# fransiskusbudi/multimodal_segmentation_project

Measured on AMD Instinct MI355X. Metric: 3D volumes/sec (96^3, 4-class) fwd+bwd per node, higher is better.
Workload: dtype bf16; 1 GPU; UNet3D(1->4, features 16/32/64/128) 96^3 patch, per-GPU batch 2, fwd + Dice/CE loss + bwd + AdamW + metrics, dropout 0.0; global_batch=2, parallelism=dp1, hipgraph=False

## Files before the change

include/mi3d.h:

```cpp
#ifndef MI3D_H
#define MI3D_H
#include <stddef.h>
#include <stdint.h>

#ifdef __cplusplus
extern "C" {
#endif

#define MI3D_DTYPE_F32 0
#define MI3D_DTYPE_BF16 1
#define MI3D_MAX_LEVELS 6

const char* mi3d_last_error(void);
int mi3d_abi_version(void);

typedef struct mi3d_unet_desc {
    int32_t in_channels, out_channels;
    int32_t n_levels;
    int32_t features[MI3D_MAX_LEVELS];
    int32_t N, D, H, W;
    int32_t dtype;
    float bn_momentum, bn_eps;
} mi3d_unet_desc;

int mi3d_unet_num_params(const mi3d_unet_desc* d);
int mi3d_unet_num_buffers(const mi3d_unet_desc* d);
size_t mi3d_unet_workspace_bytes(const mi3d_unet_desc* d);
int64_t mi3d_unet_dropout_count(const mi3d_unet_desc* d);

int mi3d_unet_forward(const mi3d_unet_desc* d, const float* x, const void* const* params, void* const* buffers,
                      const float* drop_scales, int training, float* logits, float* gap_out, void* workspace,
                      size_t workspace_bytes, void* stream);

int mi3d_unet_bn_apply_deferred(const mi3d_unet_desc* d, void* const* buffers, const void* const* side, void* stream);

int mi3d_unet_infer(const mi3d_unet_desc* d, const float* x, const void* const* params, void* const* buffers, float* logits,
                    float* gap_out, void* workspace, size_t workspace_bytes, void* stream);

int mi3d_unet_num_segments(const mi3d_unet_desc* d);
int mi3d_unet_backward(const mi3d_unet_desc* d, const float* x, const void* const* params, void* const* grads,
                       const float* drop_scales, const float* dlogits, const float* dgap, float gap_scale,
                       int accumulate, int seg_begin, int seg_end, void* workspace, size_t workspace_bytes,
                       void* stream, void* aux_stream, void* const* events, int aux_join);
int mi3d_unet_backward_marks(const int* segs, void* const* events, int n);
int mi3d_stream_wait_event(void* stream, void* event);
int mi3d_event_create(void** event_out);
int mi3d_event_destroy(void* event);
int mi3d_stream_create(int priority_class, void** stream_out);
int mi3d_stream_destroy(void* stream);
int mi3d_debug_set_route(const char* name, int value);
int mi3d_debug_get_route(const char* name, int* value_out);
int mi3d_debug_route_count(void);
const char* mi3d_debug_route_name(int index);
int mi3d_debug_occupy_cus(int workgroups, int microseconds, float* buf, int64_t n, void* stream);
int mi3d_timing_event_create(void** event_out);
int mi3d_time_next_conv3_kernel(void* start_event, void* stop_event, int kind, int Cin, int Cout);
int mi3d_time_hook_fired(void);
int mi3d_event_elapsed_ms(void* start_event, void* stop_event, float* ms_out);
int mi3d_unet_segment_params(const mi3d_unet_desc* d, int seg, int* ranges);

typedef struct mi3d_loss_cfg {
    float w_ce;
    int32_t region_kind;
    float w_reg, alpha, beta, eps;
    float w_kd, temperature;
} mi3d_loss_cfg;
#define MI3D_LOSS_COEF_FLOATS 20
size_t mi3d_seg_loss_workspace_bytes(int C);
int mi3d_seg_loss_forward(const float* logits, const int64_t* labels, const float* teacher, int N, int C, int64_t V,
                          const mi3d_loss_cfg* cfg, float* loss_out, float* coef, void* workspace, void* stream);
int mi3d_seg_loss_backward(const float* logits, const int64_t* labels, const float* teacher, int N, int C, int64_t V,
                           const mi3d_loss_cfg* cfg, const float* coef, const float* grad_out, float* dlogits,
                           void* stream);
int mi3d_seg_loss_metrics_forward(const float* logits, const int64_t* labels, const float* teacher, int N, int C, int D,
                                  int64_t V, const mi3d_loss_cfg* cfg, float* loss_out, float* coef, float* metrics_out,
                                  void* loss_workspace, void* metrics_workspace, void* stream);
int mi3d_unet_head_loss_supported(const mi3d_unet_desc* d, const mi3d_loss_cfg* cfg);
int mi3d_head_loss_supported(int dtype, int Cin, int C, const mi3d_loss_cfg* cfg);
int mi3d_head_loss_forward(const void* z, int zcs, int Cin, const float* w, const float* bias, const int64_t* labels,
                           const float* teacher, int N, int C, int D, int64_t V, const mi3d_loss_cfg* cfg, float* loss_out, float* coef,
                           float* metrics_out, void* loss_workspace, void* metrics_workspace, float* logits_opt, void* stream);
int mi3d_head_loss_backward(const void* z, int zcs, int Cin, const float* w, const float* bias, const int64_t* labels,
                            const float* teacher, int N, int C, int64_t V, const mi3d_loss_cfg* cfg, const float* coef,
                            const float* grad_scale, void* dz, int dzcs, float* dW, float* db, int accumulate, void* workspace,
                            size_t workspace_bytes, void* stream);
int mi3d_unet_forward_loss(const mi3d_unet_desc* d, const float* x, const void* const* params, void* const* buffers,
                           const float* drop_scales, int training, const int64_t* labels, const float* teacher_logits,
                           const mi3d_loss_cfg* cfg, float* loss_out, float* coef, float* metrics_out, void* loss_workspace,
                           void* metrics_workspace, float* logits_opt, float* gap_out, void* workspace, size_t workspace_bytes,
                           void* stream);
int mi3d_unet_head_loss_forward(const mi3d_unet_desc* d, const void* const* params, const int64_t* labels, const float* teacher_logits,
                                const mi3d_loss_cfg* cfg, float* loss_out, float* coef, float* metrics_out, void* loss_workspace,
                                void* metrics_workspace, float* logits_opt, void* workspace, size_t workspace_bytes, void* stream);
int mi3d_unet_backward_loss(const mi3d_unet_desc* d, const float* x, const void* const* params, void* const* grads,
                            const float* drop_scales, const int64_t* labels, const float* teacher_logits, const mi3d_loss_cfg* cfg,
                            const float* coef, const float* grad_scale, const float* dgap, float gap_scale, int accumulate, int seg_begin,
                            int seg_end, void* workspace, size_t workspace_bytes, void* stream, void* aux_stream, void* const* events,
                            int aux_join);
size_t mi3d_seg_metrics_workspace_bytes(int C);
int mi3d_seg_metrics(const float* logits, const int64_t* labels, int N, int C, int D, int64_t V, float* out,
                     void* workspace, void* stream);
int mi3d_seg_class_counts(const float* logits, const int64_t* labels, int N, int C, int64_t V, int64_t* counts,
                          void* workspace, void* stream);
size_t mi3d_head_labels_workspace_bytes(int N, int Cout);
int mi3d_head_labels(int dtype, const void* z, int zcs, int Cin, const float* w, const float* bias, int Cout, int N, int64_t V,
                     uint8_t* labels_out, const int64_t* target, int64_t* counts, void* workspace, void* stream);
int mi3d_unet_head_labels(const mi3d_unet_desc* d, const void* const* params, const int64_t* target, uint8_t* labels_out,
                          int64_t* counts, void* head_workspace, void* workspace, size_t workspace_bytes, void* stream);

int mi3d_linear_forward(const float* x, const float* w, const float* b, float* y, int M, int K, int Nout, int relu,
                        const float* drop, void* stream);
int mi3d_linear_backward(const float* x, const float* w, const float* y, const float* gy, int M, int K, int Nout,
                         int relu, const float* drop, float* gx, float* gw, float* gb, int accumulate,
                         float gx_scale, float* workspace, void* stream);
int mi3d_scale(const float* x, float* y, int64_t n, float alpha, const float* alpha_dev, void* stream);
int mi3d_softmax_ce_rows(const float* logits, const int64_t* labels, int M, int C, float* loss, float* dlogits,
                         float scale, void* stream);

int mi3d_adamw_step(float* p, const float* g, float* m, float* v, int64_t n, float lr, float beta1, float beta2,
                    float eps, float weight_decay, float grad_scale, int64_t* step_dev, void* stream);
int mi3d_adamw_apply(float* p, const float* g, float* m, float* v, int64_t n, float lr, float beta1, float beta2,
                     float eps, float weight_decay, float grad_scale, int64_t* step_dev, int increment, void* stream);
int mi3d_dropout_scales(float* out, int64_t n, float p, uint64_t* state_dev, void* stream);

int mi3d_preprocess_ct(const float* in, float* out, int64_t n, float window_min, float window_max, void* stream);
size_t mi3d_preprocess_mri_workspace_bytes(void);
int mi3d_preprocess_mri(const float* in, float* out, int64_t n, float p_low, float p_high, void* workspace, void* stream);
int mi3d_remap_labels(const int64_t* in, int64_t* out, int64_t n, int kind, void* stream);

size_t mi3d_zoom3_workspace_bytes(int D, int H, int W);
int mi3d_zoom3_cubic(const float* in, float* out, int D, int H, int W, int Do, int Ho, int Wo, const void* table_d, int rows_d,
                     const void* table_h, int rows_h, const void* table_w, int rows_w, int ct_window, float window_min,
                     float window_max, void* stream);
int mi3d_zoom3_nearest_i64(const int64_t* in, int64_t* out, int D, int H, int W, int Do, int Ho, int Wo, const int32_t* index_d,
                           int rows_d, const int32_t* index_h, int rows_h, const int32_t* index_w, int rows_w, void* stream);

enum { MI3D_SRC_U8 = 0, MI3D_SRC_I16 = 1, MI3D_SRC_F32 = 2, MI3D_SRC_I64 = 3 };
int mi3d_reorient3(const void* in, int src_dtype, void* out, int out_i64, int D, int H, int W, int64_t stride_d, int64_t stride_h,
                   int64_t stride_w, int flip_mask, void* stream);
int mi3d_zoom3_cubic_src(const void* in, int src_dtype, int64_t stride_d, int64_t stride_h, int64_t stride_w, float* out, int D,
                         int H, int W, int Do, int Ho, int Wo, const void* table_d, int rows_d, const void* table_h, int rows_h,
                         const void* table_w, int rows_w, int ct_window, float window_min, float window_max, void* stream);
int mi3d_zoom3_nearest_src(const void* in, int src_dtype, int64_t stride_d, int64_t stride_h, int64_t stride_w, int64_t* out, int D,
                           int H, int W, int Do, int Ho, int Wo, const int32_t* index_d, int rows_d, const int32_t* index_h,
                           int rows_h, const int32_t* index_w, int rows_w, void* stream);
#define MI3D_MAX_MASKS 8
typedef struct {
    const void* mask[MI3D_MAX_MASKS];
    int64_t value[MI3D_MAX_MASKS];
    int32_t n;
} mi3d_mask_list;
int mi3d_merge_masks3(const mi3d_mask_list* masks, int src_dtype, int64_t stride_d, int64_t stride_h, int64_t stride_w, int64_t* out,
                      int D, int H, int W, int Do, int Ho, int Wo, const int32_t* index_d, int rows_d, const int32_t* index_h,
                      int rows_h, const int32_t* index_w, int rows_w, void* stream);
int mi3d_restore_labels3(const uint8_t* grid, int Dg, int Hg, int Wg, uint8_t* out, int D, int H, int W, int64_t stride_d,
                         int64_t stride_h, int64_t stride_w, const int32_t* index_d, const int32_t* index_h, const int32_t* index_w,
                         void* stream);

size_t mi3d_preview_workspace_bytes(int D, int H, int W);
int mi3d_foreground_profiles(const void* label, int label_dtype, int D, int H, int W, int64_t stride_d, int64_t stride_h,
                             int64_t stride_w, int64_t* counts, void* stream);
int mi3d_best_slices(const int64_t* counts, int D, int H, int W, int32_t* best, void* stream);
enum { MI3D_PREVIEW_STACK = 0, MI3D_PREVIEW_ONE = 1, MI3D_PREVIEW_THREE = 2 };
int mi3d_slice_minmax(const void* image, int image_dtype, int D, int H, int W, int64_t stride_d, int64_t stride_h, int64_t stride_w,
                      int axis, int mode, const int32_t* index, int k, uint32_t* keys, void* stream);
enum { MI3D_OVERLAY_F64 = 0, MI3D_OVERLAY_F32 = 1, MI3D_OVERLAY_U8 = 2 };
int mi3d_overlay_render(const void* image, int image_dtype, const int64_t* image_strides, const void* label, int label_dtype,
                        const int64_t* label_strides, const void* pred, int pred_dtype, const int64_t* pred_strides, int D, int H, int W,
                        int axis, int mode, const int32_t* index, int k, int rot90, const uint32_t* keys, int out_dtype,
                        void* const* outs, void* stream);

int mi3d_plane_affine(const float* img_in, float* img_out, const int64_t* lab_in, int64_t* lab_out, int C, int D, int H, int W,
                      int ax0, int ax1, const double* matrix, const double* offset, int flip_mask, void* stream);

#define MI3D_AUG_MAX_COEFF 20
#define MI3D_AUG_MAX_CP 16
#define MI3D_AUG_MAX_HOLES 8
typedef struct mi3d_aug_params {
    int32_t do_bias, bias_degree;
    double bias_coeff[MI3D_AUG_MAX_COEFF];
    int32_t do_noise;
    float noise_mean, noise_std;
    uint64_t noise_seed;
    int32_t do_contrast;
    float gamma;
    int32_t do_hist, n_cp;
    float ref_cp[MI3D_AUG_MAX_CP], flt_cp[MI3D_AUG_MAX_CP];
    int32_t n_holes;
    int32_t hole_size[3];
    int32_t hole_lo[MI3D_AUG_MAX_HOLES][3];
    float fill_value;
} mi3d_aug_params;
size_t mi3d_augment_workspace_bytes(void);
int mi3d_augment(const float* in, float* out, const float* noise, int C, int D, int H, int W, const mi3d_aug_params* params,
                 void* workspace, size_t workspace_bytes, void* stream);
int mi3d_fill_boxes_i64(int64_t* label, int C, int D, int H, int W, int n_holes, const int32_t* hole_lo,
                        const int32_t* hole_size, int64_t fill, void* stream);

size_t mi3d_conv3_workspace_bytes(int Cin, int Cout, int N, int D, int H, int W);
int mi3d_conv3_forward(int in_dtype, int out_dtype, const void* x, int xcs, int Cin, const float* w, const float* bias,
                       void* y, int ycs, int Cout, int N, int D, int H, int W, void* workspace, size_t workspace_bytes,
                       void* stream);
int mi3d_conv3_backward(int x_dtype, int dy_dtype, const void* x, int xcs, int Cin, const float* w, const void* dy,
                        int dycs, int Cout, void* dx, int dxcs, float* dW, float* db, int accumulate, int N, int D,
                        int H, int W, void* workspace, size_t workspace_bytes, void* stream);
typedef struct mi3d_conv3_bn_route { int32_t conv, ksplit, ticket, stats, rows, rows_offset; } mi3d_conv3_bn_route;
enum { MI3D_CONV3_BN_KEEP_TICKETS = 1 };
size_t mi3d_conv3_bn_workspace_bytes(int in_dtype, int dtype, int Cin, int Cout, int N, int D, int H, int W);
int mi3d_conv3_bn_forward(int in_dtype, int dtype, const void* x, int xcs, int Cin, const float* w, const float* bias,
                          const float* gamma, const float* beta, float* running_mean, float* running_var,
                          int64_t* num_batches_tracked, float momentum, float eps, const float* drop, void* y, void* z, int zcs,
                          void* pooled, int pcs, float* stat, int flags, mi3d_conv3_bn_route* route_out, int Cout, int N, int D,
                          int H, int W, void* workspace, size_t workspace_bytes, void* stream);
typedef struct mi3d_pending_sum { int64_t opaque[9]; } mi3d_pending_sum;
typedef struct mi3d_conv3_bn_bwd_route {
    int32_t bn, riders, dz_ks, conv, dgrad_ks, dx_ks, dx_offset, slabs, slab_layout, slab_ew, pending;
} mi3d_conv3_bn_bwd_route;
enum { MI3D_CONV3_BN_BWD_ALLOW_PARTIALS = 1, MI3D_CONV3_BN_BWD_DEFER = 2, MI3D_CONV3_BN_BWD_LEAVE_PENDING = 4 };
size_t mi3d_conv3_bn_bwd_workspace_bytes(int in_dtype, int dtype, int Cin, int Cout, int N, int D, int H, int W);
int mi3d_conv3_bn_backward(int in_dtype, int dtype, const void* x, int xcs, int x_split, int64_t x_delta, int Cin, const float* w,
                           const void* y, const float* stat, const float* drop, void* dz, int dzcs, const float* dz_partials,
                           int dz_ks, void* dy, void* dx, int dxcs, int dx_split, int64_t dx_delta, float* dW, float* db,
                           float* dgamma, float* dbeta, int accumulate, const mi3d_pending_sum* riders, mi3d_pending_sum* pending_out,
                           int flags, mi3d_conv3_bn_bwd_route* route_out, int Cout, int N, int D, int H, int W, void* workspace,
                           size_t workspace_bytes, void* stream);
int mi3d_pending_sum_launch(const mi3d_pending_sum* job, void* stream);
size_t mi3d_bn_workspace_bytes(int C);
int mi3d_bn_relu_drop_forward(int dtype, const void* y, int ycs, int C, int64_t M, int64_t V, const float* gamma,
                              const float* beta, float* running_mean, float* running_var, int64_t* num_batches_tracked,
                              float momentum, float eps, int training, const float* drop, void* z, int zcs, float* stat,
                              void* workspace, void* stream);
int mi3d_bn_relu_drop_backward(int dtype, const void* dz, int dzcs, const void* y, int ycs, int C, int64_t M, int64_t V,
                               const float* stat, const float* drop, void* dy, int dycs, float* dgamma, float* dbeta,
                               int accumulate, void* workspace, void* stream);
int mi3d_bn_relu_drop_pool_forward(int dtype, const void* y, int ycs, int C, int N, int D, int H, int W, const float* gamma,
                                   const float* beta, float* running_mean, float* running_var, int64_t* num_batches_tracked,
                                   float momentum, float eps, const float* drop, void* z, int zcs, void* pooled, int pcs,
                                   float* stat, void* workspace, void* stream);
int mi3d_maxpool2_forward(int dtype, const void* z, int zcs, int C, int N, int D, int H, int W, void* p, int pcs,
                          void* stream);
int mi3d_maxpool2_backward(int dtype, const void* dp, int dpcs, const void* z, int zcs, const void* dskip, int dskipcs,
                           void* dz, int dzcs, int C, int N, int D, int H, int W, void* stream);
int mi3d_maxpool2_backward_partials(int dtype, const float* dp_partials, int ks, const void* z, int zcs, const void* dskip,
                                    int dskipcs, void* dz, int dzcs, int C, int N, int D, int H, int W, void* stream);
size_t mi3d_upconv2_workspace_bytes(int Cin, int Cout, int N, int D, int H, int W);
int mi3d_upconv2_forward(int dtype, const void* x, int xcs, int Cin, const float* w, const float* bias, void* y, int ycs,
                         int Cout, int N, int D, int H, int W, void* workspace, size_t workspace_bytes, void* stream);
int mi3d_upconv2_backward(int dtype, const void* x, int xcs, int Cin, const float* w, const void* gy, int gycs, int Cout,
                          void* dx, int dxcs, float* dW, float* db, int accumulate, int N, int D, int H, int W,
                          void* workspace, size_t workspace_bytes, void* stream);
typedef struct mi3d_up_route {
    int32_t kind, gy, tap_split, wide, strided, resized, ksplit, persistent, slabs, slab_ew, wgrad_blocks, dgrad_blocks, pending;
} mi3d_up_route;
enum { MI3D_UP_BWD_LEAVE_PENDING = 1, MI3D_UP_BWD_SECOND_WORKSPACE = 2 };
size_t mi3d_up_workspace_bytes(int dtype, int Cin, int Cout, int N, int D, int H, int W);
size_t mi3d_up_workspace_region(int dtype, int Cin, int Cout, int N, int D, int H, int W, int which, size_t* bytes_out);
int mi3d_up_forward(int dtype, const void* x, int xcs, int Cin, const float* w, const float* bias, void* up, int ucs, int Cout,
                    int N, int D, int H, int W, int Do, int Ho, int Wo, mi3d_up_route* route_out, void* workspace,
                    size_t workspace_bytes, void* stream);
int mi3d_up_backward(int dtype, const void* x, int xcs, int Cin, const float* w, const void* gup, int gucs, int Cout, void* dx,
                     int dxcs, float* dW, float* db, int accumulate, int N, int D, int H, int W, int Do, int Ho, int Wo, int flags,
                     mi3d_pending_sum* pending_out, mi3d_up_route* route_out, void* workspace, size_t workspace_bytes, void* stream);
int mi3d_nearest_resize_forward(int dtype, const void* x, int xcs, int C, int N, int Di, int Hi, int Wi, void* y, int ycs, int Do,
                                int Ho, int Wo, void* stream);
int mi3d_nearest_resize_backward(int dtype, const void* gy, int gycs, int C, int N, int Do, int Ho, int Wo, void* gx, int gxcs,
                                 int Di, int Hi, int Wi, void* stream);
size_t mi3d_conv1_workspace_bytes(int Cin, int Cout);
int mi3d_conv1_forward(int dtype, const void* z, int zcs, int Cin, const float* w, const float* bias, float* logits, int Cout,
                       int N, int64_t V, void* stream);
int mi3d_conv1_backward(int dtype, const void* z, int zcs, int Cin, const float* w, const float* dlogits, int Cout, void* dz,
                        int dzcs, float* dW, float* db, int accumulate, int N, int64_t V, void* workspace,
                        size_t workspace_bytes, void* stream);
int mi3d_ncdhw_to_ndhwc(int dtype, const float* src, void* dst, int dcs, int C, int N, int64_t V, void* stream);
int mi3d_ndhwc_to_ncdhw(int dtype, const void* src, int scs, float* dst, int C, int N, int64_t V, void* stream);

int mi3d_graph_begin(void* stream);
int mi3d_graph_end(void* stream, void** graph_exec_out);
int mi3d_graph_launch(void* graph_exec, void* stream);
int mi3d_graph_destroy(void* graph_exec);
// ... 6 lines not shown
```

multimodal_segmentation_project_amd/_lib.py:

```python
import contextlib
import ctypes as C
import os

import torch

_HERE = os.path.dirname(os.path.abspath(__file__))
LIB_PATH = os.environ.get("MI3D_LIB_PATH") or os.path.join(_HERE, "libmi3d.so")
MAX_LEVELS = 6
LOSS_COEF_FLOATS = 20
DTYPE_F32, DTYPE_BF16 = 0, 1

vp, i32, i64, f32, sz = C.c_void_p, C.c_int, C.c_int64, C.c_float, C.c_size_t


class UNetDesc(C.Structure):
    _fields_ = [("in_channels", C.c_int32), ("out_channels", C.c_int32), ("n_levels", C.c_int32),
                ("features", C.c_int32 * MAX_LEVELS), ("N", C.c_int32), ("D", C.c_int32), ("H", C.c_int32),
                ("W", C.c_int32), ("dtype", C.c_int32), ("bn_momentum", C.c_float), ("bn_eps", C.c_float)]


class LossCfg(C.Structure):
    _fields_ = [("w_ce", C.c_float), ("region_kind", C.c_int32), ("w_reg", C.c_float), ("alpha", C.c_float),
                ("beta", C.c_float), ("eps", C.c_float), ("w_kd", C.c_float), ("temperature", C.c_float)]


AUG_MAX_COEFF, AUG_MAX_CP, AUG_MAX_HOLES = 20, 16, 8


class AugParams(C.Structure):
    _fields_ = [("do_bias", C.c_int32), ("bias_degree", C.c_int32), ("bias_coeff", C.c_double * AUG_MAX_COEFF),
                ("do_noise", C.c_int32), ("noise_mean", C.c_float), ("noise_std", C.c_float), ("noise_seed", C.c_uint64),
                ("do_contrast", C.c_int32), ("gamma", C.c_float), ("do_hist", C.c_int32), ("n_cp", C.c_int32),
                ("ref_cp", C.c_float * AUG_MAX_CP), ("flt_cp", C.c_float * AUG_MAX_CP), ("n_holes", C.c_int32),
                ("hole_size", C.c_int32 * 3), ("hole_lo", (C.c_int32 * 3) * AUG_MAX_HOLES), ("fill_value", C.c_float)]


MAX_MASKS = 8
SRC_U8, SRC_I16, SRC_F32, SRC_I64 = 0, 1, 2, 3
PREVIEW_STACK, PREVIEW_ONE, PREVIEW_THREE = 0, 1, 2
OVERLAY_F64, OVERLAY_F32, OVERLAY_U8 = 0, 1, 2


class MaskList(C.Structure):
    _fields_ = [("mask", C.c_void_p * MAX_MASKS), ("value", C.c_int64 * MAX_MASKS), ("n", C.c_int32)]


class Conv3BnRoute(C.Structure):
    _fields_ = [(k, C.c_int32) for k in ("conv", "ksplit", "ticket", "stats", "rows", "rows_offset")]


CONV3_BN_KEEP_TICKETS = 1


class Conv3BnBwdRoute(C.Structure):
    _fields_ = [(k, C.c_int32) for k in ("bn", "riders", "dz_ks", "conv", "dgrad_ks", "dx_ks", "dx_offset", "slabs", "slab_layout",
                                         "slab_ew", "pending")]


class PendingSum(C.Structure):
    _fields_ = [("opaque", C.c_int64 * 9)]


CONV3_BN_BWD_ALLOW_PARTIALS, CONV3_BN_BWD_DEFER, CONV3_BN_BWD_LEAVE_PENDING = 1, 2, 4


class UpRoute(C.Structure):
    _fields_ = [(k, C.c_int32) for k in ("kind", "gy", "tap_split", "wide", "strided", "resized", "ksplit", "persistent", "slabs",
                                         "slab_ew", "wgrad_blocks", "dgrad_blocks", "pending")]


UP_BWD_LEAVE_PENDING, UP_BWD_SECOND_WORKSPACE = 1, 2

_DP, _LP, _AP, _MP = C.POINTER(UNetDesc), C.POINTER(LossCfg), C.POINTER(AugParams), C.POINTER(MaskList)

_SIGS = {
    "mi3d_last_error": (C.c_char_p, []),
    "mi3d_abi_version": (i32, []),
    "mi3d_unet_num_params": (i32, [_DP]),
    "mi3d_unet_num_buffers": (i32, [_DP]),
    "mi3d_unet_num_segments": (i32, [_DP]),
    "mi3d_unet_workspace_bytes": (sz, [_DP]),
    "mi3d_unet_dropout_count": (i64, [_DP]),
    "mi3d_unet_segment_params": (i32, [_DP, i32, C.POINTER(C.c_int)]),
    "mi3d_unet_forward": (i32, [_DP, vp, vp, vp, vp, i32, vp, vp, vp, sz, vp]),
    "mi3d_unet_infer": (i32, [_DP, vp, vp, vp, vp, vp, vp, sz, vp]),
    "mi3d_unet_bn_apply_deferred": (i32, [_DP, vp, vp, vp]),
    "mi3d_unet_backward": (i32, [_DP, vp, vp, vp, vp, vp, vp, f32, i32, i32, i32, vp, sz, vp, vp, vp, i32]),
    "mi3d_unet_backward_marks": (i32, [C.POINTER(C.c_int), C.POINTER(vp), i32]),
    "mi3d_stream_wait_event": (i32, [vp, vp]),
    "mi3d_event_create": (i32, [C.POINTER(vp)]),
    "mi3d_event_destroy": (i32, [vp]),
    "mi3d_stream_create": (i32, [i32, C.POINTER(vp)]),
    "mi3d_stream_destroy": (i32, [vp]),
    "mi3d_debug_set_route": (i32, [C.c_char_p, i32]),
    "mi3d_debug_get_route": (i32, [C.c_char_p, C.POINTER(C.c_int)]),
    "mi3d_debug_route_count": (i32, []),
    "mi3d_debug_route_name": (C.c_char_p, [i32]),
    "mi3d_debug_occupy_cus": (i32, [i32, i32, vp, i64, vp]),
    "mi3d_timing_event_create": (i32, [C.POINTER(vp)]),
    "mi3d_time_next_conv3_kernel": (i32, [vp, vp, i32, i32, i32]),
    "mi3d_time_hook_fired": (i32, []),
    "mi3d_event_elapsed_ms": (i32, [vp, vp, C.POINTER(C.c_float)]),
    "mi3d_seg_loss_workspace_bytes": (sz, [i32]),
    "mi3d_seg_loss_forward": (i32, [vp, vp, vp, i32, i32, i64, _LP, vp, vp, vp, vp]),
    "mi3d_seg_loss_backward": (i32, [vp, vp, vp, i32, i32, i64, _LP, vp, vp, vp, vp]),
    "mi3d_seg_loss_metrics_forward": (i32, [vp, vp, vp, i32, i32, i32, i64, _LP, vp, vp, vp, vp, vp, vp]),
    "mi3d_unet_head_loss_supported": (i32, [_DP, _LP]),
    "mi3d_head_loss_supported": (i32, [i32, i32, i32, _LP]),
    "mi3d_head_loss_forward": (i32, [vp, i32, i32, vp, vp, vp, vp, i32, i32, i32, i64, _LP, vp, vp, vp, vp, vp, vp, vp]),
    "mi3d_head_loss_backward": (i32, [vp, i32, i32, vp, vp, vp, vp, i32, i32, i64, _LP, vp, vp, vp, i32, vp, vp, i32, vp, sz, vp]),
    "mi3d_unet_forward_loss": (i32, [_DP, vp, vp, vp, vp, i32, vp, vp, _LP, vp, vp, vp, vp, vp, vp, vp, vp, sz, vp]),
    "mi3d_unet_head_loss_forward": (i32, [_DP, vp, vp, vp, _LP, vp, vp, vp, vp, vp, vp, vp, sz, vp]),
    "mi3d_unet_backward_loss": (i32, [_DP, vp, vp, vp, vp, vp, vp, _LP, vp, vp, vp, f32, i32, i32, i32, vp, sz, vp, vp, vp, i32]),
    "mi3d_seg_metrics_workspace_bytes": (sz, [i32]),
    "mi3d_seg_metrics": (i32, [vp, vp, i32, i32, i32, i64, vp, vp, vp]),
    "mi3d_seg_class_counts": (i32, [vp, vp, i32, i32, i64, vp, vp, vp]),
    "mi3d_head_labels_workspace_bytes": (sz, [i32, i32]),
    "mi3d_head_labels": (i32, [i32, vp, i32, i32, vp, vp, i32, i32, i64, vp, vp, vp, vp, vp]),
    "mi3d_unet_head_labels": (i32, [_DP, vp, vp, vp, vp, vp, vp, sz, vp]),
    "mi3d_linear_forward": (i32, [vp, vp, vp, vp, i32, i32, i32, i32, vp, vp]),
    "mi3d_linear_backward": (i32, [vp, vp, vp, vp, i32, i32, i32, i32, vp, vp, vp, vp, i32, f32, vp, vp]),
    "mi3d_scale": (i32, [vp, vp, i64, f32, vp, vp]),
    "mi3d_softmax_ce_rows": (i32, [vp, vp, i32, i32, vp, vp, f32, vp]),
    "mi3d_adamw_step": (i32, [vp, vp, vp, vp, i64, f32, f32, f32, f32, f32, f32, vp, vp]),
    "mi3d_adamw_apply": (i32, [vp, vp, vp, vp, i64, f32, f32, f32, f32, f32, f32, vp, i32, vp]),
    "mi3d_dropout_scales": (i32, [vp, i64, f32, vp, vp]),
    "mi3d_preprocess_ct": (i32, [vp, vp, i64, f32, f32, vp]),
    "mi3d_preprocess_mri_workspace_bytes": (sz, []),
    "mi3d_preprocess_mri": (i32, [vp, vp, i64, f32, f32, vp, vp]),
    "mi3d_remap_labels": (i32, [vp, vp, i64, i32, vp]),
    "mi3d_zoom3_workspace_bytes": (sz, [i32, i32, i32]),
    "mi3d_zoom3_cubic": (i32, [vp, vp, i32, i32, i32, i32, i32, i32, vp, i32, vp, i32, vp, i32, i32, f32, f32, vp]),
    "mi3d_zoom3_nearest_i64": (i32, [vp, vp, i32, i32, i32, i32, i32, i32, vp, i32, vp, i32, vp, i32, vp]),
    "mi3d_reorient3": (i32, [vp, i32, vp, i32, i32, i32, i32, i64, i64, i64, i32, vp]),
    "mi3d_zoom3_cubic_src": (i32, [vp, i32, i64, i64, i64, vp, i32, i32, i32, i32, i32, i32, vp, i32, vp, i32, vp, i32, i32, f32, f32, vp]),
    "mi3d_zoom3_nearest_src": (i32, [vp, i32, i64, i64, i64, vp, i32, i32, i32, i32, i32, i32, vp, i32, vp, i32, vp, i32, vp]),
    "mi3d_merge_masks3": (i32, [_MP, i32, i64, i64, i64, vp, i32, i32, i32, i32, i32, i32, vp, i32, vp, i32, vp, i32, vp]),
    "mi3d_restore_labels3": (i32, [vp, i32, i32, i32, vp, i32, i32, i32, i64, i64, i64, vp, vp, vp, vp]),
    "mi3d_preview_workspace_bytes": (sz, [i32, i32, i32]),
    "mi3d_foreground_profiles": (i32, [vp, i32, i32, i32, i32, i64, i64, i64, vp, vp]),
    "mi3d_best_slices": (i32, [vp, i32, i32, i32, vp, vp]),
    "mi3d_slice_minmax": (i32, [vp, i32, i32, i32, i32, i64, i64, i64, i32, i32, vp, i32, vp, vp]),
    "mi3d_overlay_render": (i32, [vp, i32, C.POINTER(i64), vp, i32, C.POINTER(i64), vp, i32, C.POINTER(i64), i32, i32, i32, i32, i32, vp,
                                  i32, i32, vp, i32, C.POINTER(vp), vp]),
    "mi3d_plane_affine": (i32, [vp, vp, vp, vp, i32, i32, i32, i32, i32, i32, C.POINTER(C.c_double), C.POINTER(C.c_double), i32, vp]),
    "mi3d_augment_workspace_bytes": (sz, []),
    "mi3d_augment": (i32, [vp, vp, vp, i32, i32, i32, i32, _AP, vp, sz, vp]),
    "mi3d_fill_boxes_i64": (i32, [vp, i32, i32, i32, i32, i32, C.POINTER(C.c_int32), C.POINTER(C.c_int32), i64, vp]),
    "mi3d_conv3_workspace_bytes": (sz, [i32, i32, i32, i32, i32, i32]),
    "mi3d_conv3_forward": (i32, [i32, i32, vp, i32, i32, vp, vp, vp, i32, i32, i32, i32, i32, i32, vp, sz, vp]),
    "mi3d_conv3_backward": (i32, [i32, i32, vp, i32, i32, vp, vp, i32, i32, vp, i32, vp, vp, i32, i32, i32, i32, i32,
                                  vp, sz, vp]),
    "mi3d_conv3_bn_workspace_bytes": (sz, [i32, i32, i32, i32, i32, i32, i32, i32]),
    "mi3d_conv3_bn_forward": (i32, [i32, i32, vp, i32, i32, vp, vp, vp, vp, vp, vp, vp, f32, f32, vp, vp, vp, i32, vp, i32, vp, i32,
                                    C.POINTER(Conv3BnRoute), i32, i32, i32, i32, i32, vp, sz, vp]),
    "mi3d_conv3_bn_bwd_workspace_bytes": (sz, [i32, i32, i32, i32, i32, i32, i32, i32]),
    "mi3d_conv3_bn_backward": (i32, [i32, i32, vp, i32, i32, i64, i32, vp, vp, vp, vp, vp, i32, vp, i32, vp, vp, i32, i32, i64, vp, vp,
                                     vp, vp, i32, C.POINTER(PendingSum), C.POINTER(PendingSum), i32, C.POINTER(Conv3BnBwdRoute),
                                     i32, i32, i32, i32, i32, vp, sz, vp]),
    "mi3d_pending_sum_launch": (i32, [C.POINTER(PendingSum), vp]),
    "mi3d_bn_workspace_bytes": (sz, [i32]),
    "mi3d_bn_relu_drop_forward": (i32, [i32, vp, i32, i32, i64, i64, vp, vp, vp, vp, vp, f32, f32, i32, vp, vp, i32,
                                        vp, vp, vp]),
    "mi3d_bn_relu_drop_backward": (i32, [i32, vp, i32, vp, i32, i32, i64, i64, vp, vp, vp, i32, vp, vp, i32, vp, vp]),
    "mi3d_bn_relu_drop_pool_forward": (i32, [i32, vp, i32, i32, i32, i32, i32, i32, vp, vp, vp, vp, vp, f32, f32, vp, vp, i32,
                                             vp, i32, vp, vp, vp]),
    "mi3d_conv1_workspace_bytes": (sz, [i32, i32]),
    "mi3d_conv1_forward": (i32, [i32, vp, i32, i32, vp, vp, vp, i32, i32, i64, vp]),
    "mi3d_conv1_backward": (i32, [i32, vp, i32, i32, vp, vp, i32, vp, i32, vp, vp, i32, i32, i64, vp, sz, vp]),
    "mi3d_maxpool2_forward": (i32, [i32, vp, i32, i32, i32, i32, i32, i32, vp, i32, vp]),
    "mi3d_maxpool2_backward": (i32, [i32, vp, i32, vp, i32, vp, i32, vp, i32, i32, i32, i32, i32, i32, vp]),
    "mi3d_maxpool2_backward_partials": (i32, [i32, vp, i32, vp, i32, vp, i32, vp, i32, i32, i32, i32, i32, i32, vp]),
    "mi3d_upconv2_workspace_bytes": (sz, [i32, i32, i32, i32, i32, i32]),
    "mi3d_upconv2_forward": (i32, [i32, vp, i32, i32, vp, vp, vp, i32, i32, i32, i32, i32, i32, vp, sz, vp]),
    "mi3d_upconv2_backward": (i32, [i32, vp, i32, i32, vp, vp, i32, i32, vp, i32, vp, vp, i32, i32, i32, i32, i32, vp,
                                    sz, vp]),
    "mi3d_up_workspace_bytes": (sz, [i32, i32, i32, i32, i32, i32, i32]),
    "mi3d_up_workspace_region": (sz, [i32, i32, i32, i32, i32, i32, i32, i32, C.POINTER(sz)]),
# ... 107 lines not shown
```

multimodal_segmentation_project_amd/csrc/api.hip:

```cpp
#include "../../include/mi3d.h"
#include <stdlib.h>
#include <string.h>

#include "ops.h"

static_assert(MI3D_LOSS_COEF_FLOATS >= 2 * MI3D_MAX_CLASSES + 4, "coef buffer too small");

namespace {
struct RouteEntry { const char* name; int Mi3dRoutes::*field; };
const RouteEntry ROUTE_TABLE[] = {
#define MI3D_ROUTE_ENTRY(name, dflt) {#name, &Mi3dRoutes::name},
    MI3D_ROUTE_LIST(MI3D_ROUTE_ENTRY)
#undef MI3D_ROUTE_ENTRY
};
constexpr int N_ROUTES = sizeof(ROUTE_TABLE) / sizeof(ROUTE_TABLE[0]);
Mi3dRoutes load_routes() {
    Mi3dRoutes r;
    for (int i = 0; i < N_ROUTES; i++) {
        char env[64] = "MI3D_";
        size_t n = 5;
        for (const char* c = ROUTE_TABLE[i].name; *c && n + 1 < sizeof(env); c++) env[n++] = (*c >= 'a' && *c <= 'z') ? *c - 32 : *c;
        env[n] = 0;
        const char* v = getenv(env);
        if (!v) continue;
// ... 215 lines not shown
    ConvBwdCall k{x_dtype, dy_dtype, x, xcs, Halves(), Cin, w, nullptr, nullptr, nullptr, const_cast<void*>(dy), dycs, nullptr, 0, nullptr,
                  dx, dxcs, Halves(), dW, db, nullptr, nullptr, accumulate, nullptr, nullptr, 0, nullptr, Cout, g, mfma, c1, ws};
    return conv_bn_bwd_run(k, L, (hipStream_t)stream);
}

size_t mi3d_conv3_bn_bwd_workspace_bytes(int in_dtype, int dtype, int Cin, int Cout, int N, int D, int H, int W) {
    if (Cin < 1 || Cout < 1 || N < 1 || D < 1 || H < 1 || W < 1) return 0;
    bool mfma, c1;
    conv3_layer_class(dtype, Cin, Cout, mfma, c1);
    return conv_bn_bwd_ws(mfma, Cin, Cout, Geo{N, D, H, W}).total;
}
int mi3d_conv3_bn_backward(int in_dtype, int dtype, const void* x, int xcs, int x_split, int64_t x_delta, int Cin, const float* w,
                           const void* y, const float* stat, const float* drop, void* dz, int dzcs, const float* dz_partials,
                           int dz_ks, void* dy, void* dx, int dxcs, int dx_split, int64_t dx_delta, float* dW, float* db,
                           float* dgamma, float* dbeta, int accumulate, const mi3d_pending_sum* riders, mi3d_pending_sum* pending_out,
                           int flags, mi3d_conv3_bn_bwd_route* route_out, int Cout, int N, int D, int H, int W, void* workspace,
                           size_t workspace_bytes, void* stream) {
    const char* fn = "mi3d_conv3_bn_backward";
    MI3D_CHECK_ARG(x && w && dz && workspace, "%s: null pointer", fn);
    MI3D_CHECK_ARG(!stat || (y && dy), "%s: the BatchNorm backward needs y and dy", fn);
    MI3D_CHECK_ARG(stat || (!dz_partials && !riders), "%s: dz partials and riders need the BatchNorm backward", fn);
    MI3D_CHECK_ARG((dtype == MI3D_F32 || dtype == MI3D_BF16) && (in_dtype == dtype || (in_dtype == MI3D_F32 && Cin == 1 && xcs == 1)),
                   "%s: bad dtypes %d -> %d", fn, in_dtype, dtype);
    MI3D_CHECK_ARG(Cin >= 1 && Cout >= 1 && Cout <= 256 && xcs >= (x_delta ? 16 : Cin) && dzcs >= Cout && N >= 1 && D >= 1 && H >= 1 && W >= 1,
                   "%s: bad shape", fn);
    MI3D_CHECK_ARG(!dz_partials || dz_ks >= 1, "%s: dz_ks=%d", fn, dz_ks);
    MI3D_CHECK_ARG(!(flags & MI3D_CONV3_BN_BWD_LEAVE_PENDING) || pending_out, "%s: LEAVE_PENDING needs pending_out", fn);
    MI3D_CHECK_ARG(!(flags & MI3D_CONV3_BN_BWD_DEFER) || !(flags & MI3D_CONV3_BN_BWD_LEAVE_PENDING), "%s: DEFER launches its own sum", fn);
    const Geo g{N, D, H, W};
    bool mfma, c1;
    conv3_layer_class(dtype, Cin, Cout, mfma, c1);
    MI3D_CHECK_ARG(!mfma || (xcs % 8 == 0 && dzcs % 8 == 0 && (!dx || dxcs % 4 == 0)), "%s: channel strides %d / %d / %d", fn, xcs, dzcs, dxcs);
    MI3D_CHECK_ARG(!c1 || (in_dtype == MI3D_F32 && !dx), "%s: the first-layer kernel reads an fp32 image and has no input gradient", fn);
    MI3D_CHECK_ARG(!dx || dxcs >= (dx_delta ? 16 : Cin), "%s: dx stride %d", fn, dxcs);
    MI3D_CHECK_ARG(!(flags & MI3D_CONV3_BN_BWD_DEFER) || (mfma && (dW || db)), "%s: only MFMA layers with a weight gradient defer it", fn);
    MI3D_CHECK_ARG((!x_delta && !dx_delta) || (mfma && conv3_mfma_halves_ok(Cout, Cin, g)),
                   "%s: planar halves need the full-resolution kernels", fn);
    const ConvBnBwdWs L = conv_bn_bwd_ws(mfma, Cin, Cout, g);
    MI3D_CHECK_ARG(workspace_bytes >= L.total, "%s: workspace too small: %zu < %zu", fn, workspace_bytes, L.total);
    MI3D_CHECK_ARG(((uintptr_t)workspace & 255) == 0, "%s: workspace must be 256-byte aligned", fn);
    Halves xh, dxh;
    if (x_delta) { xh.split = x_split; xh.delta = x_delta; }
    if (dx_delta) { dxh.split = dx_split; dxh.delta = dx_delta; }
    ConvBwdCall k{in_dtype, dtype, x, xcs, xh, Cin, w, y, stat, drop, dz, dzcs, dz_partials, dz_ks, dy, dx, dxcs, dxh, dW, db, dgamma, dbeta,
                  accumulate, riders, pending_out, flags, route_out, Cout, g, mfma, c1, (char*)workspace};
    return conv_bn_bwd_run(k, L, (hipStream_t)stream);
}
int mi3d_pending_sum_launch(const mi3d_pending_sum* job, void* stream) {
    MI3D_CHECK_ARG(job, "mi3d_pending_sum_launch: null job");
    SlabJob q;
    memcpy(&q, job, sizeof(q));
    return slab_job_launch(q, (hipStream_t)stream);
}

}

namespace {
struct ConvBnWs {
    bool mfma, c1;
    size_t statpart, tkcount, bnws, wpf, wpd, skws, total;
};
ConvBnWs conv_bn_ws(int dtype, int Cin, int Cout, Geo g) {
    ConvBnWs L;
    conv3_layer_class(dtype, Cin, Cout, L.mfma, L.c1);
    size_t off = 0;
    auto take = [&](size_t bytes) { size_t o = off; off = (off + bytes + 255) & ~(size_t)255; return o; };
    int rows = L.mfma ? conv3_mfma_stat_blocks(Cin, Cout, g) : L.c1 ? conv3_c1_fwd_stat_blocks(g) : 1;
    L.statpart = take((size_t)rows * 2 * Cout * sizeof(float));
    L.tkcount = take((size_t)CONV3_TK_COUNTERS * sizeof(int));
    L.bnws = take(bn_ws_floats(Cout) * sizeof(float));
    L.wpf = take(L.mfma ? conv3_mfma_pack_elems(Cin, Cout) * 2 : conv3_direct_pack_floats(Cin, Cout) * sizeof(float));
    L.wpd = take(L.mfma ? conv3_mfma_pack_elems(Cin, Cout) * 2 : conv3_direct_pack_floats(Cout, Cin) * sizeof(float));
    L.skws = take((L.mfma ? conv3_mfma_splitk_floats(Cin, Cout, g) : 0) * sizeof(float) + 16);
    L.total = off;
    return L;
}
}

extern "C" {

size_t mi3d_conv3_bn_workspace_bytes(int in_dtype, int dtype, int Cin, int Cout, int N, int D, int H, int W) {
    if (Cin < 1 || Cout < 1 || N < 1 || D < 1 || H < 1 || W < 1) return 0;
    return conv_bn_ws(dtype, Cin, Cout, Geo{N, D, H, W}).total;
}
int mi3d_conv3_bn_forward(int in_dtype, int dtype, const void* x, int xcs, int Cin, const float* w, const float* bias,
                          const float* gamma, const float* beta, float* running_mean, float* running_var,
                          int64_t* num_batches_tracked, float momentum, float eps, const float* drop, void* y, void* z, int zcs,
                          void* pooled, int pcs, float* stat, int flags, mi3d_conv3_bn_route* route_out, int Cout, int N, int D,
                          int H, int W, void* workspace, size_t workspace_bytes, void* stream) {
    MI3D_CHECK_ARG(x && w && bias && gamma && beta && y && z && stat && workspace, "mi3d_conv3_bn_forward: null pointer");
    MI3D_CHECK_ARG((dtype == MI3D_F32 || dtype == MI3D_BF16) && (in_dtype == dtype || (in_dtype == MI3D_F32 && Cin == 1 && xcs == 1)),
                   "mi3d_conv3_bn_forward: bad dtypes %d -> %d", in_dtype, dtype);
    MI3D_CHECK_ARG(Cin >= 1 && Cout >= 1 && Cout <= 256 && xcs >= Cin && zcs >= Cout && N >= 1 && D >= 1 && H >= 1 && W >= 1,
                   "mi3d_conv3_bn_forward: bad shape");
    MI3D_CHECK_ARG(!pooled || (D % 2 == 0 && H % 2 == 0 && W % 2 == 0 && pcs >= Cout && (int64_t)N * D * H * W * Cout < (1ll << 31)),
                   "mi3d_conv3_bn_forward: pooled needs even sides and fewer than 2^31 elements");
    const Geo g{N, D, H, W};
    const ConvBnWs L = conv_bn_ws(dtype, Cin, Cout, g);
    MI3D_CHECK_ARG(!L.mfma || xcs % 8 == 0, "mi3d_conv3_bn_forward: input channel stride %d", xcs);
    MI3D_CHECK_ARG(!L.c1 || in_dtype == MI3D_F32, "mi3d_conv3_bn_forward: the first-layer kernel reads an fp32 image");
    MI3D_CHECK_ARG(workspace_bytes >= L.total, "mi3d_conv3_bn_forward: workspace too small: %zu < %zu", workspace_bytes, L.total);
    MI3D_CHECK_ARG(((uintptr_t)workspace & 255) == 0, "mi3d_conv3_bn_forward: workspace must be 256-byte aligned");
    char* ws = (char*)workspace;
    hipStream_t s = (hipStream_t)stream;
    bool tk_zeroed = false;
    if (L.mfma) {
// ... 330 lines not shown
```

multimodal_segmentation_project_amd/csrc/conv3_mfma.hip:

```cpp
#include <stdlib.h>

#include <type_traits>

#include <hip/hip_ext.h>

#include "mfma_tile.h"
#include "ops.h"
#include "slab_sum.h"

namespace {

constexpr int BLK = 256;

MI3D_HD constexpr int ktap(int mode, int s, int h) {
    if (mode == 0) return 2 * s + h;
    if (s < 12) {
        int dz = s / 4, k = s % 4;
        return k < 3 ? dz * 9 + k * 3 + h : dz * 9 + h * 3 + 2;
    }
    if (s == 12) return h * 9 + 8;
    return h == 0 ? 26 : 27;
}

__global__ void pack_mfma_kernel(const float* __restrict__ w, int Cin, int Cout, bf16* __restrict__ wf, bf16* __restrict__ wd,
                                 int mode_f, int mode_d) {
    int64_t n = (int64_t)Cin * Cout * 28;
    for (int64_t i = (int64_t)blockIdx.x * blockDim.x + threadIdx.x; i < 2 * n; i += (int64_t)gridDim.x * blockDim.x) {
        bool dg = i >= n;
        int64_t k = dg ? i - n : i;
        int j = k & 7; int lane = (k >> 3) & 63; int64_t r = k >> 9;
        int nob = (dg ? Cin : Cout) / 16;
        int ob = r % nob; r /= nob; int s = r % 14; int chunk = r / 14;
        int g = lane >> 4, tap = ktap(dg ? mode_d : mode_f, s, g >> 1);
        int o = ob * 16 + (lane & 15), ic = chunk * 16 + 8 * (g & 1) + j;
        float v = 0.f;
        if (tap < 27) v = dg ? w[((int64_t)ic * Cin + o) * 27 + (26 - tap)] : w[((int64_t)o * Cin + ic) * 27 + tap];
        (dg ? wd : wf)[k] = (bf16)v;
    }
}

constexpr int PK_LD = 16 * 27 + 1;
__global__ __launch_bounds__(BLK) void pack_all_kernel(PackJobs J) {
    __shared__ float wl[16 * PK_LD];
    if (blockIdx.x == 0 && J.zero)
        for (int i = threadIdx.x; i < J.nzero; i += BLK) J.zero[i] = 0;
    int b = blockIdx.x, ji = 0;
    while (ji + 1 < J.n && b >= J.j[ji + 1].blk0) ji++;
    const float* __restrict__ w = J.j[ji].w;
    int Cin = J.j[ji].Cin, Cout = J.j[ji].Cout, lb = b - J.j[ji].blk0;
    if (J.j[ji].kind == 0) {
        bf16* wf = (bf16*)J.j[ji].a; bf16* wd = (bf16*)J.j[ji].b;
        int mode_f = J.j[ji].mode_f, mode_d = J.j[ji].mode_d;
        int CIBN = Cin / 16, COBN = Cout / 16;
        int cib = lb % CIBN, cob = lb / CIBN;
        const float* __restrict__ sc = J.j[ji].scale;
        for (int idx = threadIdx.x; idx < 16 * 108; idx += BLK) {
            int row = idx / 108, k = (idx - row * 108) * 4;
            f32x4 v = *reinterpret_cast<const f32x4*>(w + ((int64_t)(cob * 16 + row) * Cin + cib * 16) * 27 + k);
            float f = sc ? sc[cob * 16 + row] : 1.f;
#pragma unroll
            for (int j = 0; j < 4; j++) wl[row * PK_LD + k + j] = v[j] * f;
        }
        __syncthreads();
        for (int q = threadIdx.x; q < 2 * 14 * 64; q += BLK) {
            int img = q / (14 * 64), r = q - img * (14 * 64);
            int s = r >> 6, lane = r & 63, g = lane >> 4, o = lane & 15;
            int tap = ktap(img ? mode_d : mode_f, s, g >> 1);
            bf16x8 v;
#pragma unroll
            for (int j = 0; j < 8; j++) {
                int ic = 8 * (g & 1) + j;
                float f = 0.f;
                if (tap < 27) f = img ? wl[ic * PK_LD + o * 27 + (26 - tap)] : wl[o * PK_LD + ic * 27 + tap];
                v[j] = (bf16)f;
            }
            bf16* dst = img ? wd + ((((int64_t)cob * 14 + s) * CIBN + cib) * 64 + lane) * 8
                            : wf + ((((int64_t)cib * 14 + s) * COBN + cob) * 64 + lane) * 8;
            *reinterpret_cast<bf16x8*>(dst) = v;
        }
    } else {
        bf16* wf = (bf16*)J.j[ji].a; bf16* wb = (bf16*)J.j[ji].b;
        int64_t n = (int64_t)Cin * Cout * 8;
        int KS = Cin / 32, COBN = Cout / 16, S = Cout / 4;
        int64_t k0 = ((int64_t)lb * BLK + threadIdx.x) * 8;
        if (k0 >= 2 * n) return;
        bool bw = k0 >= n;
        int64_t k = bw ? k0 - n : k0;
        int lane = (k >> 3) & 63, G = lane >> 4;
        int64_t r = k >> 9;
        bf16x8 v;
        if (!bw) {
            int ks = r % KS; r /= KS; int cb = r % COBN; int tap = r / COBN;
            int co = cb * 16 + (lane & 15);
#pragma unroll
            for (int j = 0; j < 8; j++) v[j] = (bf16)w[((int64_t)(32 * ks + 8 * G + j) * Cout + co) * 8 + tap];
        } else {
            int s = r % S; int cib = r / S;
            int kk0 = 32 * s + 8 * G, tap = kk0 / Cout, co0 = kk0 % Cout, ci = cib * 16 + (lane & 15);
#pragma unroll
            for (int j = 0; j < 8; j++) v[j] = (bf16)w[((int64_t)ci * Cout + co0 + j) * 8 + tap];
        }
        *reinterpret_cast<bf16x8*>((bw ? wb : wf) + k) = v;
    }
}

struct Bid { int x, y, z, gx, gy, gz; bool placed = false; };
__device__ __forceinline__ Bid real_bid() {
    return Bid{(int)blockIdx.x, (int)blockIdx.y, (int)blockIdx.z, (int)gridDim.x, (int)gridDim.y, (int)gridDim.z};
}
__device__ __forceinline__ int xcd_contig(int b, int n) {
    int q8 = n / 8, r8 = n % 8, xcd = b % 8, idx = b / 8;
    return (xcd < r8 ? xcd * (q8 + 1) : r8 * (q8 + 1) + (xcd - r8) * q8) + idx;
}

template <int TZ_, int TYB_, int TXB_, int BX_>
struct ConvTile {
    static constexpr int TZ = TZ_, TYB = TYB_, TXB = TXB_, BX = BX_;
    static constexpr int BY = 16 / BX;
    static constexpr int TY = TYB * BY, TX = TXB * BX;
    static constexpr int IZ = TZ + 2, IY = TY + 2, IX = TX + 2;
    static constexpr int IXP = BX == 4 ? 12 : IX;
    static constexpr int MB = TYB * TXB;
    static constexpr int NVT = TZ * TY * TX;
    static constexpr int NVOX = IZ * IY * IX, NVOXP = IZ * IY * IXP;
    static constexpr int pieces(int nthr) { return (NVOX * 2 + nthr - 1) / nthr; }
};
using FullTile = ConvTile<4, 8, 1, 16>;

template <class T, int COB>
struct Lds4 {
    static constexpr int xs = 0, red = T::NVOXP * 32, bytes = red + 4 * COB * 16 * 2 * 4;
};
template <class T, int COB>
struct Lds8 {
    static constexpr int xs = 0, wl = T::NVOXP * 32, red = wl + 14 * COB * 1024, bytes = red + 8 * COB * 16 * 2 * 4;
};
template <int COB, int NCH>
struct LdsP {
    static constexpr int xs = 0, wl = FullTile::NVOX * 32, red = wl + NCH * 14 * COB * 1024, bytes = red + 4 * COB * 16 * 2 * 4;
};

template <class T, int NTHR, int NIT>
__device__ __forceinline__ void staging_map(int z0, int y0, int x0, int D, int H, int W, int xcs, int (&soff)[NIT], int (&sdst)[NIT]) {
#pragma unroll
    for (int it = 0; it < NIT; it++) {
        int idx = threadIdx.x + it * NTHR;
        int vox = idx >> 1, half = idx & 1;
        int ix = vox % T::IX, t = vox / T::IX, iy = t % T::IY, iz = t / T::IY;
        sdst[it] = T::IXP == T::IX ? 0 : (t * T::IXP + ix) * 16 + half * 8;
        int gz = z0 - 1 + iz, gy = y0 - 1 + iy, gx = x0 - 1 + ix;
        bool inb = idx < T::NVOX * 2 && gz >= 0 && gz < D && gy >= 0 && gy < H && gx >= 0 && gx < W;
        soff[it] = inb ? ((gz * H + gy) * W + gx) * xcs + half * 8 : -1;
    }
}
template <class T, int NTHR, int NIT>
// ... 780 lines not shown

inline bool big_geo(Geo g) { return g.W >= 32 && g.H >= 16; }

inline int pick_ksplit(int Cin, int Cout, Geo g, int target_override = 0) {
    if (big_geo(g)) return 1;
    int64_t wgs = (int64_t)g.N * cdiv(g.D, 4) * cdiv(g.H, 8) * cdiv(g.W, 8) * (Cout / (Cout % 32 == 0 ? 32 : 16));
    int nchunk = Cin / 16, k = 1;
    constexpr int SPLITK_TARGET = 128;
    const int tgt = target_override > 0 && target_override < SPLITK_TARGET ? target_override : SPLITK_TARGET;
    while (wgs * k < tgt && k * 2 <= nchunk && nchunk % (k * 2) == 0 && k < 16) k *= 2;
    return k;
}

}

bool conv3_mfma_supported(int Cin, int Cout, int xcs, int ycs) {
    return Cin % 16 == 0 && Cout % 16 == 0 && xcs % 8 == 0 && ycs % 4 == 0 && Cin >= 16 && Cout >= 16;
}

size_t conv3_mfma_pack_elems(int Cin, int Cout) { return (size_t)Cin * Cout * 28; }

int conv3_mfma_pack(const float* w, int Cin, int Cout, void* wp_fwd, void* wp_dgrad, Geo g, hipStream_t s) {
    int64_t n = 2 * (int64_t)conv3_mfma_pack_elems(Cin, Cout);
    int mode_f = persist_ok(Cin, Cout, g) ? 1 : 0, mode_d = persist_ok(Cout, Cin, g) ? 1 : 0;
    pack_mfma_kernel<<<cdiv(n, 256) > 2048 ? 2048 : cdiv(n, 256), 256, 0, s>>>(w, Cin, Cout, (bf16*)wp_fwd, (bf16*)wp_dgrad,
                                                                             mode_f, mode_d);
    MI3D_LAUNCH_CHECK();
    return 0;
}

int pack_all_add_conv3(PackJobs& J, const float* w, int Cin, int Cout, void* wp_fwd, void* wp_dgrad, Geo g, const float* scale) {
    MI3D_CHECK_ARG(J.n < MAX_PACK_JOBS && Cin % 16 == 0 && Cout % 16 == 0, "pack_all: too many jobs / bad channels");
    MI3D_CHECK_ARG(((uintptr_t)w % 16) == 0, "pack_all: conv weight tensor must be 16-byte aligned");
    PackJob& j = J.j[J.n++];
    j = PackJob{w, wp_fwd, wp_dgrad, Cin, Cout, 0, persist_ok(Cin, Cout, g) ? 1 : 0, persist_ok(Cout, Cin, g) ? 1 : 0, J.nblocks, scale};
    J.nblocks += (Cin / 16) * (Cout / 16);
    return 0;
}
int pack_all_add_upconv(PackJobs& J, const float* w, int Cin, int Cout, void* wp) {
    MI3D_CHECK_ARG(J.n < MAX_PACK_JOBS, "pack_all: too many jobs");
    int64_t n = (int64_t)Cin * Cout * 8;
    PackJob& j = J.j[J.n++];
    j = PackJob{w, wp, (bf16*)wp + n, Cin, Cout, 1, 0, 0, J.nblocks};
    J.nblocks += (int)cdiv(2 * n, (int64_t)BLK * 8);
    return 0;
}
int pack_all_launch(const PackJobs& J, hipStream_t s) {
    if (J.n == 0) return 0;
    pack_all_kernel<<<J.nblocks, BLK, 0, s>>>(J);
    MI3D_LAUNCH_CHECK();
    return 0;
}

int conv3_mfma_stat_blocks(int Cin, int Cout, Geo g) {
    if (persist_ok(Cin, Cout, g)) return persist_grid(Cin, Cout, g);
    if (big_geo(g)) return g.N * cdiv(g.D, 4) * cdiv(g.H, 8) * cdiv(g.W, 16);
    return g.N * cdiv(g.D, 4) * cdiv(g.H, 8) * cdiv(g.W, 8);
}

size_t conv3_mfma_splitk_floats(int Cin, int Cout, Geo g) {
    int k = pick_ksplit(Cin, Cout, g);
    return k > 1 ? (size_t)k * g.M() * Cout : 0;
}
bool conv3_mfma_fuses_stats(int Cin, int Cout, Geo g) { return pick_ksplit(Cin, Cout, g) == 1; }

bool conv3_mfma_halves_ok(int Cin, int Cout, Geo g) { return persist_ok(Cin, Cout, g); }

bool conv3_mfma_ticket_ok(int Cin, int Cout, Geo g) {
    if (!mi3d_routes().splitk_ticket || mi3d_routes().conv8 == 0 || big_geo(g) || persist_ok(Cin, Cout, g)) return false;
    if (pick_ksplit(Cin, Cout, g) <= 1) return false;
    const int64_t wgs = (int64_t)g.N * cdiv(g.D, 4) * cdiv(g.H, 8) * cdiv(g.W, 8) * (Cout / (Cout % 32 == 0 ? 32 : 16));
    return wgs <= CONV3_TK_COUNTERS;
}

int conv3_mfma_fwd(const void* x, int xcs, int Cin, const void* wp, const float* bias, void* y, int ycs, int Cout, Geo g,
                   float* part, float* skws, hipStream_t s, Halves xh, Halves yh, int* ks_deferred, int relu, int split_target,
                   float* tk_rows, int* tk_count, Conv3Launch* launched) {
    if (ks_deferred) *ks_deferred = 0;
    MI3D_CHECK_ARG(!tk_rows || (conv3_mfma_ticket_ok(Cin, Cout, g) && skws && split_target == 0), "conv3_mfma_fwd: no split-K ticket for %d->%d here", Cin, Cout);
    MI3D_CHECK_ARG((!xh.on() && !yh.on()) || persist_ok(Cin, Cout, g), "conv3_mfma_fwd: planar halves need the persistent kernel");
    MI3D_CHECK_ARG(conv3_mfma_supported(Cin, Cout, xcs, ycs), "conv3_mfma_fwd: unsupported channels %d->%d", Cin, Cout);
    MI3D_CHECK_ARG(((uintptr_t)x % 16) == 0 && ((uintptr_t)y % 8) == 0, "conv3_mfma_fwd: misaligned tensors");
    const bf16* xp = (const bf16*)x; const bf16* w = (const bf16*)wp; bf16* yp = (bf16*)y;
    bool two = Cout % 32 == 0;
    if (persist_ok(Cin, Cout, g)) {
        int tz = cdiv(g.D, 4), ty = cdiv(g.H, 8), tx = cdiv(g.W, 16), nt = g.N * tz * ty * tx, grid = persist_grid(Cin, Cout, g);
        if (launched) *launched = Conv3Launch{2, 1};
        if (ycs % 8 == 0 && ((uintptr_t)y % 16) == 0 && yh.delta % 8 == 0) relu |= 2;
        auto launch = [&](auto cob, auto nch) -> int {
            constexpr int COB = decltype(cob)::value, NCH = decltype(nch)::value;
            if (part)
                return launch_hooked<conv3_mfma_persist_kernel<COB, NCH, true>>(grid, BLK, 0, s, 2, Cin, Cout, xp, xcs, w, bias, yp, ycs, g.D, g.H, g.W,
                                                                                tz, ty, tx, nt, part, xh, yh, relu);
            return launch_hooked<conv3_mfma_persist_kernel<COB, NCH, false>>(grid, BLK, 0, s, 3, Cin, Cout, xp, xcs, w, bias, yp, ycs, g.D, g.H, g.W,
                                                                             tz, ty, tx, nt, (float*)nullptr, xh, yh, relu);
        };
        constexpr std::integral_constant<int, 1> one{};
        constexpr std::integral_constant<int, 2> two{};
        return Cin == 16 && Cout == 16 ? launch(one, one) : Cin == 32 ? launch(one, two) : launch(two, one);
    }
    int ks = skws ? pick_ksplit(Cin, Cout, g, split_target) : 1;
    if (ycs % 8 == 0 && ((uintptr_t)y % 16) == 0 && Cout % 32 == 0) relu |= 2;
    if (ks > 1) MI3D_CHECK_ARG(ycs % 8 == 0 && ((uintptr_t)y % 16) == 0, "conv3_mfma_fwd: split-K needs 16-B aligned output rows");
    if (launched) *launched = Conv3Launch{big_geo(g) ? 3 : 4, big_geo(g) ? 1 : ks};
    if (big_geo(g)) {
        if (two) return launch_cfg<4, 8, 1, 16, 2>(xp, xcs, Cin, w, bias, yp, ycs, Cout, g, part, 1, nullptr, s, false, relu);
// ... 518 lines not shown
    const float* part; int ks; int64_t M; int C; bf16* y; int ycs; int nfin;
    const float* slabs; int nslab; int64_t slab_sz, nW; float* dW; float* db; int accumulate, Cin, Cout, layout, ew;
};
__global__ __launch_bounds__(BLK) void bwd_tail_kernel(TailArgs a) {
    int b = blockIdx.x;
    if (b < a.nfin) { splitk_finish_body(b, a.nfin, a.part, a.ks, a.M, a.C, nullptr, a.y, a.ycs); return; }
    b -= a.nfin;
    if (a.layout == 2) slab_reduce_tile_body(b, a.slabs, a.nslab, a.slab_sz, a.nW, a.dW, a.db, a.accumulate, a.Cin, a.Cout);
    else if (a.ew == 8) slab_reduce2_body<true, 8>(b, a.slabs, a.nslab, a.slab_sz, a.nW, a.dW, a.db, a.accumulate, a.Cin, a.Cout);
    else slab_reduce2_body<true, 32>(b, a.slabs, a.nslab, a.slab_sz, a.nW, a.dW, a.db, a.accumulate, a.Cin, a.Cout);
}

struct WgCfg { int cob, cib, nt, tg, nsb; };

inline WgCfg wgrad_cfg(int Cin, int Cout, Geo g, int target = 0) {
    WgCfg c;
    c.cob = 1;
    c.cib = 1;
    int groups = (Cout / 16) * (Cin / 16);
    int64_t ntiles = (int64_t)g.N * cdiv(g.D, WTZ) * cdiv(g.H, WTY) * cdiv(g.W, WTX);
    c.nt = 27;
    c.tg = 1;
    int64_t want = (target > 0 ? target : 2 * device_cus()) / (int64_t)groups;
    if (want < 1) want = 1;
    int64_t rounds = cdiv(ntiles, want);
    c.nsb = (int)cdiv(ntiles, rounds);
    return c;
}

template <int CO_B, int CI_B, int NT>
int launch_wgrad(const bf16* x, int xcs, int Cin, const bf16* dy, int dycs, int Cout, Geo g, float* slabs, WgCfg c,
                 hipStream_t s, Halves xh) {
    constexpr size_t lds = LdsWg<CO_B, CI_B>::bytes;
    dim3 grid((unsigned)(c.nsb * c.tg), (unsigned)(Cout / (16 * CO_B)), (unsigned)(Cin / (16 * CI_B)));
    const bool full = persist_ok(Cout, Cin, g);
    const int xcd_tiles = full ? 1 : 0;
    int pgx = 0, pgy = 0, pgz = 0;
    if (!full && c.tg == 1) {
        pgx = (int)grid.x; pgy = (int)grid.y; pgz = (int)grid.z;
        grid = dim3((unsigned)(pgx * pgy * pgz));
    }
    return launch_hooked<conv3_wgrad_mfma_kernel<CO_B, CI_B, NT>>(grid, BLK, lds, s, 1, Cin, Cout, x, xcs, Cin, dy, dycs, Cout, g.N, g.D, g.H, g.W,
                                                                  cdiv(g.D, WTZ), cdiv(g.H, WTY), cdiv(g.W, WTX), c.tg, slabs, xh, xcd_tiles,
                                                                  pgx, pgy, pgz);
}

inline int c1_nsb(Geo g) {
    int64_t ntiles = (int64_t)g.N * cdiv(g.D, WTZ) * cdiv(g.H, WTY) * cdiv(g.W, WTX);
    return (int)(ntiles < 1024 ? ntiles : 1024);
}

}

__global__ __launch_bounds__(BLK) void slab_job_kernel(SlabJob q) { slab_job_run(q, (int)blockIdx.x); }
int slab_job_launch(const SlabJob& q, hipStream_t s) {
    if (q.nblocks <= 0) return 0;
    slab_job_kernel<<<q.nblocks, BLK, 0, s>>>(q);
    MI3D_LAUNCH_CHECK();
    return 0;
}

static int wgrad_slab_sum(float* ws, int nsb, int Cin, int Cout, float* dW, float* db, int accumulate, hipStream_t s,
                          SlabJob* pend = nullptr) {
    int64_t nW = (int64_t)Cout * Cin * 27, slab_sz = nW + Cout;
    if (pend) { *pend = slab_job_make((dW && slab_sz >= (800 << 10)) ? 2 : 1, ws, nsb, slab_sz, nW, dW, db, Cin, Cout, accumulate); return 0; }
    if (dW && slab_sz >= (800 << 10))
        slab_reduce_tile_kernel<<<(Cout / 16) * (Cin / 16) * 4, BLK, 0, s>>>(ws, nsb, slab_sz, nW, dW, db, accumulate, Cin, Cout);
    else if (slab_sz < (16 << 10))
        slab_reduce2_kernel<true, 8><<<cdiv(slab_sz, 8), BLK, 0, s>>>(ws, nsb, slab_sz, nW, dW, db, accumulate, Cin, Cout);
    else
        slab_reduce2_kernel<true, 32><<<cdiv(slab_sz, 32), BLK, 0, s>>>(ws, nsb, slab_sz, nW, dW, db, accumulate, Cin, Cout);
    MI3D_LAUNCH_CHECK();
    return 0;
}

size_t conv3_mfma_wgrad_ws_floats(int Cin, int Cout, Geo g) {
    if (Cin == 1) return (size_t)c1_nsb(g) * ((size_t)Cout * 27 + Cout);
    return (size_t)wgrad_cfg(Cin, Cout, g).nsb * ((size_t)Cout * Cin * 27 + Cout);
}

bool conv3_mfma_big_geo(Geo g) { return big_geo(g); }
int conv3_mfma_wgrad_slabs(int Cin, int Cout, Geo g, int wg_target) { return wgrad_cfg(Cin, Cout, g, wg_target).nsb; }
int conv3_mfma_bwd_ksplit(int Cin, int Cout, Geo g) { return pick_ksplit(Cout, Cin, g, CONV3_BWD_SPLITK_TARGET); }

int conv3_mfma_wgrad(const void* x, int xcs, int Cin, const void* dy, int dycs, int Cout, Geo g, float* dW, float* db,
                     int accumulate, float* ws, size_t ws_floats, hipStream_t s, Halves xh, SlabJob* pend, int wg_target) {
    MI3D_CHECK_ARG(conv3_mfma_supported(Cin, Cout, xcs, dycs) && dycs % 8 == 0, "conv3_mfma_wgrad: unsupported channels");
    WgCfg c = wgrad_cfg(Cin, Cout, g, wg_target);
    int64_t nW = (int64_t)Cout * Cin * 27, slab_sz = nW + Cout;
    MI3D_CHECK_ARG(ws_floats >= (size_t)c.nsb * slab_sz, "conv3_mfma_wgrad: workspace too small");
    const bf16* xp = (const bf16*)x; const bf16* dp = (const bf16*)dy;
    int rc;
    if (c.cob == 1 && c.cib == 1) rc = launch_wgrad<1, 1, 27>(xp, xcs, Cin, dp, dycs, Cout, g, ws, c, s, xh);
    else { MI3D_CHECK_ARG(false, "conv3_mfma_wgrad: no kernel for this block config"); return -1; }
    MI3D_TRY(rc);
    return wgrad_slab_sum(ws, c.nsb, Cin, Cout, dW, db, accumulate, s, pend);
}


extern "C" int mi3d_time_next_conv3_kernel(void* start_event, void* stop_event, int kind, int Cin, int Cout) {
    g_hook = TimeHook();
    if (!start_event || !stop_event) return 0;
    g_hook.e0 = (hipEvent_t)start_event; g_hook.e1 = (hipEvent_t)stop_event;
    g_hook.kind = kind; g_hook.cin = Cin; g_hook.cout = Cout; g_hook.armed = true;
    return 0;
}
extern "C" int mi3d_time_hook_fired(void) {
    const int f = g_hook.fired ? 1 : 0;
    g_hook = TimeHook();
    return f;
// ... 134 lines not shown
```

multimodal_segmentation_project_amd/csrc/misc.hip:

```cpp
#include <stdarg.h>
#include <stdio.h>

#include "ops.h"

static thread_local char g_err[512] = "";
void mi3d_set_error(const char* fmt, ...) {
    va_list ap;
    va_start(ap, fmt);
    vsnprintf(g_err, sizeof(g_err), fmt, ap);
    va_end(ap);
}
extern "C" const char* mi3d_last_error(void) { return g_err; }

namespace {
constexpr int BLK = 256;
inline int sgrid(int64_t total, int cap = 2048) {
    int64_t w = (total + BLK - 1) / BLK;
    return (int)(w < 1 ? 1 : (w > cap ? cap : w));
}

template <int EW>
__global__ __launch_bounds__(BLK) void slab_reduce_kernel(const float* __restrict__ slabs, int nslab, int64_t slab_sz, int64_t nW,
                                                          float* __restrict__ dW, float* __restrict__ db, int accumulate) {
    constexpr int SG = BLK / EW;
    __shared__ float red[SG][EW];
    int e = threadIdx.x % EW, sg = threadIdx.x / EW;
    int64_t i = (int64_t)blockIdx.x * EW + e;
    float s = 0.f;
    if (i < slab_sz)
        for (int b = sg; b < nslab; b += SG) s += slabs[(int64_t)b * slab_sz + i];
    red[sg][e] = s;
    __syncthreads();
    if (sg == 0 && i < slab_sz) {
        float t = 0.f;
#pragma unroll
        for (int k = 0; k < SG; k += 8)
            t += ((red[k][e] + red[k + 1][e]) + (red[k + 2][e] + red[k + 3][e])) +
                 ((red[k + 4][e] + red[k + 5][e]) + (red[k + 6][e] + red[k + 7][e]));
        if (i < nW) { if (dW) dW[i] = accumulate ? dW[i] + t : t; }
        else if (db) { db[i - nW] = accumulate ? db[i - nW] + t : t; }
    }
}

template <typename T>
__global__ void ncdhw_to_ndhwc_kernel(const float* __restrict__ src, T* __restrict__ dst, int dcs, int C, int N, int64_t V) {
    int64_t total = (int64_t)N * V * C;
    for (int64_t i = (int64_t)blockIdx.x * BLK + threadIdx.x; i < total; i += (int64_t)gridDim.x * BLK) {
        int c = (int)(i % C); int64_t m = i / C; int64_t n = m / V, v = m - n * V;
        dst[m * dcs + c] = from_f<T>(src[((int64_t)n * C + c) * V + v]);
    }
}
template <typename T>
__global__ void ndhwc_to_ncdhw_kernel(const T* __restrict__ src, int scs, float* __restrict__ dst, int C, int N, int64_t V) {
    int64_t total = (int64_t)N * V * C;
    for (int64_t i = (int64_t)blockIdx.x * BLK + threadIdx.x; i < total; i += (int64_t)gridDim.x * BLK) {
// ... 47 lines not shown
__global__ void linear_bwd_pre_kernel(const float* __restrict__ y, const float* __restrict__ gy, int n, int relu,
                                      const float* __restrict__ drop, float* __restrict__ gpre) {
    int i = blockIdx.x * BLK + threadIdx.x;
    if (i >= n) return;
    float g = gy[i];
    if (drop) g *= drop[i];
    if (relu && !(y[i] > 0.f)) g = 0.f;
    gpre[i] = g;
}
__global__ __launch_bounds__(BLK) void linear_bwd_x_kernel(const float* __restrict__ gpre, const float* __restrict__ w,
                                                           float* __restrict__ gx, int M, int K, int Nout, float scale) {
    int i = blockIdx.x * BLK + threadIdx.x;
    if (i >= M * K) return;
    int m = i / K, k = i - m * K;
    float s = 0.f;
    for (int o = 0; o < Nout; o++) s = fmaf(gpre[(int64_t)m * Nout + o], w[(int64_t)o * K + k], s);
    gx[i] = s * scale;
}
__global__ __launch_bounds__(BLK) void linear_bwd_w_kernel(const float* __restrict__ gpre, const float* __restrict__ x,
                                                           float* __restrict__ gw, float* __restrict__ gb, int M, int K,
                                                           int Nout, int accumulate) {
    int i = blockIdx.x * BLK + threadIdx.x;
    if (gw && i < Nout * K) {
        int o = i / K, k = i - o * K;
        float s = 0.f;
        for (int m = 0; m < M; m++) s = fmaf(gpre[(int64_t)m * Nout + o], x[(int64_t)m * K + k], s);
        gw[i] = accumulate ? gw[i] + s : s;
    }
    if (i < Nout && gb) {
        float s = 0.f;
        for (int m = 0; m < M; m++) s += gpre[(int64_t)m * Nout + i];
        gb[i] = accumulate ? gb[i] + s : s;
    }
}

__global__ void softmax_ce_rows_kernel(const float* __restrict__ logits, const int64_t* __restrict__ labels, int M, int C,
                                       float* loss, float* dlogits, float scale) {
    int lane = threadIdx.x;
    double tot = 0.0;
    for (int m = 0; m < M; m++) {
        float z = lane < C ? logits[(int64_t)m * C + lane] : -INFINITY;
        float mx = z;
        for (int o = 32; o > 0; o >>= 1) mx = fmaxf(mx, __shfl_xor(mx, o, 64));
        float e = lane < C ? expf(z - mx) : 0.f;
        float se = wave_sum(e);
        int t = (int)labels[m];
        float zt = __shfl(z, t, 64);
        tot += (double)(mx + logf(se) - zt);
        if (dlogits && lane < C) dlogits[(int64_t)m * C + lane] = scale * (e / se - (lane == t ? 1.f : 0.f)) / (float)M;
    }
    if (lane == 0 && loss) *loss = (float)(tot / (double)M);
}

__device__ __forceinline__ void adamw_one(float& pi, float gi, float& mi, float& vi, float decay, float b1, float b2, float eps,
                                          float grad_scale, float bc2s, float step_size) {
#pragma clang fp contract(off)
    gi = gi * grad_scale;
    mi = __builtin_fmaf(b1, mi, (1.f - b1) * gi);
    vi = __builtin_fmaf(b2, vi, ((1.f - b2) * gi) * gi);
    float denom = sqrtf(vi) / bc2s + eps;
    pi = __builtin_fmaf(decay, pi, -(step_size * (mi / denom)));
}
__global__ __launch_bounds__(BLK) void adamw_kernel(float* __restrict__ p, const float* __restrict__ g, float* __restrict__ m,
                                                    float* __restrict__ v, int64_t n, float lr, float b1, float b2, float eps, float wd,
                                                    float grad_scale, const int64_t* __restrict__ step_dev) {
    const bool vec = ((reinterpret_cast<uintptr_t>(p) | reinterpret_cast<uintptr_t>(g) | reinterpret_cast<uintptr_t>(m) |
                       reinterpret_cast<uintptr_t>(v)) & 15) == 0;
    const int64_t n4 = vec ? n >> 2 : 0, stride = (int64_t)gridDim.x * BLK;
    int64_t i = (int64_t)blockIdx.x * BLK + threadIdx.x;
    float4 g4, p4, m4, v4;
    bool have = i < n4;
    if (have) {
        g4 = reinterpret_cast<const float4*>(g)[i]; p4 = reinterpret_cast<const float4*>(p)[i];
        m4 = reinterpret_cast<const float4*>(m)[i]; v4 = reinterpret_cast<const float4*>(v)[i];
    }
    double step = (double)(*step_dev + 1);
    float bc1 = (float)(1.0 - pow((double)b1, step));
    float bc2s = (float)sqrt(1.0 - pow((double)b2, step));
    float step_size = lr / bc1;
    const float decay = __builtin_fmaf(-lr, wd, 1.f);
    while (have) {
        int64_t j = i + stride;
        bool have2 = j < n4;
        float4 g5, p5, m5, v5;
        if (have2) {
            g5 = reinterpret_cast<const float4*>(g)[j]; p5 = reinterpret_cast<const float4*>(p)[j];
            m5 = reinterpret_cast<const float4*>(m)[j]; v5 = reinterpret_cast<const float4*>(v)[j];
        }
        adamw_one(p4.x, g4.x, m4.x, v4.x, decay, b1, b2, eps, grad_scale, bc2s, step_size);
        adamw_one(p4.y, g4.y, m4.y, v4.y, decay, b1, b2, eps, grad_scale, bc2s, step_size);
        adamw_one(p4.z, g4.z, m4.z, v4.z, decay, b1, b2, eps, grad_scale, bc2s, step_size);
        adamw_one(p4.w, g4.w, m4.w, v4.w, decay, b1, b2, eps, grad_scale, bc2s, step_size);
        reinterpret_cast<float4*>(m)[i] = m4;
        reinterpret_cast<float4*>(v)[i] = v4;
        reinterpret_cast<float4*>(p)[i] = p4;
        i = j; have = have2; g4 = g5; p4 = p5; m4 = m5; v4 = v5;
    }
    for (int64_t k = n4 * 4 + (int64_t)blockIdx.x * BLK + threadIdx.x; k < n; k += stride) {
        float pi = p[k], mi = m[k], vi = v[k];
        adamw_one(pi, g[k], mi, vi, decay, b1, b2, eps, grad_scale, bc2s, step_size);
        m[k] = mi; v[k] = vi; p[k] = pi;
    }
}
__global__ void step_inc_kernel(int64_t* step_dev) { *step_dev += 1; }

__device__ __forceinline__ uint64_t mix64(uint64_t x) {
    x += 0x9E3779B97F4A7C15ull;
    x = (x ^ (x >> 30)) * 0xBF58476D1CE4E5B9ull;
    x = (x ^ (x >> 27)) * 0x94D049BB133111EBull;
    return x ^ (x >> 31);
}
__global__ void dropout_scales_kernel(float* __restrict__ out, int64_t n, float p, const uint64_t* __restrict__ state) {
    uint64_t seed = state[0], ctr = state[1];
    float keep_scale = p < 1.f ? 1.f / (1.f - p) : 0.f;
    for (int64_t i = (int64_t)blockIdx.x * BLK + threadIdx.x; i < n; i += (int64_t)gridDim.x * BLK) {
// ... 137 lines not shown
```

multimodal_segmentation_project_amd/csrc/ops.h:

```cpp
#pragma once
#include "common.h"
#include "slab_sum.h"

struct Geo {
    int N, D, H, W;
    int64_t V() const { return (int64_t)D * H * W; }
    int64_t M() const { return (int64_t)N * D * H * W; }
};

size_t conv3_direct_pack_floats(int Cin, int Cout);
int conv3_direct_pack(const float* w, int Cin, int Cout, float* wp_fwd, float* wp_dgrad, hipStream_t s,
                      const float* scale = nullptr);
int conv3_direct_fwd(int in_dtype, int out_dtype, const void* x, int xcs, int Cin, const float* wp,
                     const float* bias, void* y, int ycs, int Cout, Geo g, hipStream_t s, int relu = 0);
size_t conv3_direct_wgrad_ws_floats(int Cin, int Cout, Geo g);
int conv3_direct_wgrad(int x_dtype, int dy_dtype, const void* x, int xcs, int Cin, const void* dy, int dycs,
                       int Cout, Geo g, float* dW, float* db, int accumulate, float* ws, size_t ws_floats,
                       hipStream_t s);

bool conv3_mfma_supported(int Cin, int Cout, int xcs, int ycs);
size_t conv3_mfma_pack_elems(int Cin, int Cout);
int conv3_mfma_pack(const float* w, int Cin, int Cout, void* wp_fwd, void* wp_dgrad, Geo g, hipStream_t s);
struct PackJob { const float* w; void* a; void* b; int Cin, Cout, kind, mode_f, mode_d, blk0; const float* scale; };
constexpr int MAX_PACK_JOBS = 32;
struct PackJobs { int n, nblocks; PackJob j[MAX_PACK_JOBS]; int* zero = nullptr; int nzero = 0; };
int pack_all_add_conv3(PackJobs& J, const float* w, int Cin, int Cout, void* wp_fwd, void* wp_dgrad, Geo g,
                       const float* scale = nullptr);
int pack_all_add_upconv(PackJobs& J, const float* w, int Cin, int Cout, void* wp);
int pack_all_launch(const PackJobs& J, hipStream_t s);
int conv3_mfma_stat_blocks(int Cin, int Cout, Geo g);
size_t conv3_mfma_splitk_floats(int Cin, int Cout, Geo g);
bool conv3_mfma_fuses_stats(int Cin, int Cout, Geo g);
struct Halves { int split = 1 << 30; int64_t delta = 0; bool on() const { return delta != 0; } };
bool conv3_mfma_halves_ok(int Cin, int Cout, Geo g);
bool conv3_mfma_ticket_ok(int Cin, int Cout, Geo g);
constexpr int CONV3_TK_COUNTERS = 4096;
struct Conv3Launch { int kind = 0, ks = 1; };
int conv3_mfma_fwd(const void* x, int xcs, int Cin, const void* wp, const float* bias, void* y, int ycs, int Cout,
                   Geo g, float* part, float* skws, hipStream_t s, Halves xh = Halves(), Halves yh = Halves(),
                   int* ks_deferred = nullptr, int relu = 0, int split_target = 0, float* tk_rows = nullptr,
                   int* tk_count = nullptr, Conv3Launch* launched = nullptr);
constexpr int CONV3_BWD_SPLITK_TARGET = 128;

size_t conv3_mfma_wgrad_ws_floats(int Cin, int Cout, Geo g);
int conv3_mfma_wgrad(const void* x, int xcs, int Cin, const void* dy, int dycs, int Cout, Geo g, float* dW, float* db,
                     int accumulate, float* ws, size_t ws_floats, hipStream_t s, Halves xh = Halves(), SlabJob* pend = nullptr,
                     int wg_target = 0);
int conv3_mfma_bwd_wg_target(int Cin, int Cout, int xcs, int dycs, int dxcs, Geo g);
int conv3_mfma_wgrad_slabs(int Cin, int Cout, Geo g, int wg_target);
int conv3_mfma_bwd_ksplit(int Cin, int Cout, Geo g);
bool conv3_mfma_big_geo(Geo g);

bool conv3_mfma_bwd_fused_ok(int Cin, int Cout, int xcs, int dycs, int dxcs, Geo g);
int conv3_mfma_bwd_fused(const void* x, int xcs, int Cin, const void* dy, int dycs, int Cout, const void* wp_dgrad, void* dx,
                         int dxcs, Geo g, float* dW, float* db, int accumulate, float* wgws, size_t wgws_floats, float* skws,
                         hipStream_t s, SlabJob* pend = nullptr, int* ks_deferred = nullptr);
bool conv3_mfma_bwd_fused_persist_ok(int Cin, int Cout, int xcs, int dycs, Geo g);
int conv3_mfma_bwd_fused_persist(const void* x, int xcs, int Cin, const void* dy, int dycs, int Cout, const void* wp_dgrad, void* dx,
                                 int dxcs, Geo g, float* dW, float* db, int accumulate, float* wgws, size_t wgws_floats,
                                 hipStream_t s, Halves xh = Halves(), Halves dxh = Halves(), SlabJob* pend = nullptr);
int conv3_c1_fwd_stat_blocks(Geo g);
int conv3_c1_fwd_mfma(const float* x, const float* w, const float* bias, void* y, int ycs, int Cout, Geo g, float* part,
                      hipStream_t s, const float* wscale = nullptr, int relu = 0);
int conv3_mfma_wgrad_c1(const float* x, const void* dy, int dycs, int Cout, Geo g, float* dW, float* db, int accumulate,
                        float* ws, size_t ws_floats, hipStream_t s, SlabJob* pend = nullptr);

size_t bn_ws_floats(int C);
int bn_train_stats(int dtype, const void* y, int ycs, int C, int64_t M, const float* gamma, const float* beta,
                   float* running_mean, float* running_var, int64_t* num_batches_tracked, float momentum,
                   float eps, float* stat, float* ws, hipStream_t s, int* small_rows = nullptr);
bool bn_small_ok(int C, int64_t M, int rows);
bool bn_rows_route_ok(int C, int64_t M, int rows);
struct BnSmall {
    const float* part; int nrows;
    const float* gamma; const float* beta; float* running_mean; float* running_var; int64_t* num_batches_tracked;
    float momentum, eps;
    int64_t M = 0;
};
int bn_train_finalize(const float* part, int nblk, int C, int64_t M, const float* gamma, const float* beta,
                      float* running_mean, float* running_var, int64_t* num_batches_tracked, float momentum,
                      float eps, float* stat, hipStream_t s);
int bn_eval_stats(int C, const float* gamma, const float* beta, const float* running_mean,
                  const float* running_var, float eps, float* stat, hipStream_t s);
struct BnFoldJob { const float* gamma; const float* beta; const float* rm; const float* rv; const float* conv_bias;
                   float* scale; float* fbias; int C; };
constexpr int MAX_FOLD_JOBS = 2 * (2 * 6 + 1);
struct BnFoldJobs { int n; float eps; BnFoldJob j[MAX_FOLD_JOBS]; };
int bn_fold_all(const BnFoldJobs& J, hipStream_t s);
struct BnDeferJob { float* rm; float* rv; int64_t* nbt; const double* side; int C; };
struct BnDeferJobs { int n; float momentum; BnDeferJob j[MAX_FOLD_JOBS]; };
int bn_deferred_apply(const BnDeferJobs& J, hipStream_t s);
int bn_apply_relu_drop(int dtype, const void* y, int ycs, int C, int64_t M, int64_t V, float* stat,
                       const float* drop, void* z, int zcs, hipStream_t s, const BnSmall* small = nullptr);
int bn_apply_relu_drop_pool(int dtype, const void* y, int ycs, int C, Geo g, float* stat, const float* drop, void* z, int zcs,
                            void* pooled, int pcs, hipStream_t s, const BnSmall* small = nullptr);
int bn_bwd(int dtype, const void* dz, int dzcs, const void* y, int ycs, int C, int64_t M, int64_t V,
           const float* stat, const float* drop, void* dy, int dycs, float* dgamma, float* dbeta,
           int accumulate, float* ws, hipStream_t s, const SlabJob* extra = nullptr, const float* skp = nullptr, int ks = 0,
           const SlabJob* extra2 = nullptr);
int slab_job_launch(const SlabJob& q, hipStream_t s);

int bn_train_stats_splitk(const float* skp, int ks, const float* bias, void* y, int ycs, int C, int64_t M, const float* gamma,
                          const float* beta, float* running_mean, float* running_var, int64_t* num_batches_tracked,
                          float momentum, float eps, float* stat, float* ws, hipStream_t s, int* small_rows = nullptr);

struct mi3d_conv3_bn_route;
inline void conv3_layer_class(int dt, int Cin, int Cout, bool& mfma, bool& c1) {
    mfma = dt == MI3D_BF16 && conv3_mfma_supported(Cin, Cout, 16, 16);
    c1 = dt == MI3D_BF16 && Cin == 1 && Cout % 16 == 0;
}
struct ConvBnHalf {
    int Cin, Cout; Geo g;
    int dt;
    bool mfma, c1;
    const void* in; int ics, idt; Halves ih;
    const float* w; const float* bias; const float* gamma; const float* beta;
    void* wpf; void* wpd;
    void* y; float* stat;
    float* rm; float* rv; int64_t* nbt; float mom, eps;
    int training;
    bool tk_zeroed;
    bool beside;
    float* statpart; float* skws; int* tkcount; float* bnws;
    const float* drop;
    void* out; int ocs; void* pooled; int pcs;
};
int conv3_bn_half_forward(const ConvBnHalf& a, hipStream_t s, mi3d_conv3_bn_route* route = nullptr);

struct Pending {
    SlabJob pend, pend2;
    hipEvent_t mark = nullptr;
    static bool waits(const SlabJob& j) { return j.nblocks > 0; }
    int flush(hipStream_t s) {
        int rc = 0;
        if (waits(pend)) { rc = slab_job_launch(pend, s); pend.nblocks = 0; }
        if (waits(pend2)) { int r2 = slab_job_launch(pend2, s); pend2.nblocks = 0; if (!rc) rc = r2; }
        return rc;
    }
    SlabJob* first(hipStream_t s) {
        flush(s);
        pend = SlabJob();
        return &pend;
    }
    SlabJob* carry() {
        if (!waits(pend) || waits(pend2)) return nullptr;
        pend2 = SlabJob();
        return &pend2;
    }
    void riders(const SlabJob*& extra, const SlabJob*& extra2) const {
        extra = waits(pend) ? &pend : (waits(pend2) ? &pend2 : nullptr);
        extra2 = (waits(pend) && waits(pend2)) ? &pend2 : nullptr;
    }
    int rode(hipStream_t s) {
        pend.nblocks = pend2.nblocks = 0;
        if (mark) { MI3D_HIP(hipEventRecord(mark, s)); mark = nullptr; }
        return 0;
    }
    int finish(hipStream_t s) {
        MI3D_TRY(flush(s));
        return rode(s);
    }
    int set_mark(hipEvent_t ev, hipStream_t s) {
        if (mark) MI3D_TRY(finish(s));
        mark = ev;
        return 0;
    }
};

struct mi3d_conv3_bn_bwd_route;
struct ConvBnHalfBwd {
    int Cin, Cout; Geo g;
    int dt;
    bool mfma, c1;
    const void* in; int ics, idt; Halves ih;
    const void* wpd;
    const void* y; const float* stat; const float* drop;
    const void* dz; int dzcs;
    const float* dz_skp; int dz_ks;
    void* dy; int dycs;
    void* dx; int dxcs; Halves dxh;
    float* dW; float* db; float* dgamma; float* dbeta; int accumulate;
    float* bnws; float* wgws; size_t wgws_floats; float* skws;
    bool allow_partials;
    bool deferred;
    int (*after_bn)(void*); void* after_bn_arg;
};
int conv3_bn_half_backward(const ConvBnHalfBwd& a, Pending& pending, hipStream_t s, int* dx_ks = nullptr,
                           mi3d_conv3_bn_bwd_route* route = nullptr);
int conv3_deferred_wgrad(const void* in, int ics, int Cin, Halves ih, const void* dy, int dycs, int Cout, Geo g, int dxcs, float* dW,
                         float* db, int accumulate, float* ws, size_t ws_floats, hipStream_t s);

int maxpool2_fwd(int dtype, const void* z, int zcs, int C, Geo g, void* p, int pcs, hipStream_t s);
int maxpool2_bwd(int dtype, const void* dp, int dpcs, const void* z, int zcs, const void* dskip, int dskipcs,
                 void* dz, int dzcs, int C, Geo g, hipStream_t s, const float* skp = nullptr, int ks = 0);

int nearest_resize_fwd(int dtype, const void* x, int xcs, int C, Geo gi, void* y, int ycs, Geo go, hipStream_t s);
int nearest_resize_bwd(int dtype, const void* gy, int gycs, int C, Geo go, void* gx, int gxcs, Geo gi, hipStream_t s);

struct UpLaunch { int kind = 0, gy = 1, tap_split = 0, wide = 0, strided = 0; };
struct UpBwdLaunch { int kind = 0, ksplit = 0, persistent = 0, slabs = 0, slab_ew = 0, wgrad_blocks = 0, dgrad_blocks = 0; };
size_t upconv2_pack_floats(int Cin, int Cout);
int upconv2_pack(const float* w, int Cin, int Cout, float* wp_fwd, float* wp_bwd, hipStream_t s);
int upconv2_fwd(int dtype, const void* x, int xcs, int Cin, const float* wp_fwd, const float* bias, void* y,
                int ycs, int Cout, Geo g, hipStream_t s, UpLaunch* launched = nullptr);
size_t upconv2_bwd_ws_floats(int Cin, int Cout, Geo g);
int upconv2_bwd(int dtype, const void* x, int xcs, int Cin, const void* gy, int gycs, int Cout,
                const float* wp_bwd, void* dx, int dxcs, float* dW, float* db, int accumulate, float* ws,
                size_t ws_floats, Geo g, hipStream_t s, UpBwdLaunch* launched = nullptr);

bool upconv2_mfma_supported(int Cin, int Cout, int xcs, int ycs);
size_t upconv2_mfma_pack_elems(int Cin, int Cout);
int upconv2_mfma_pack(const float* w, int Cin, int Cout, void* wp, hipStream_t s);
// ... 92 lines not shown
```

multimodal_segmentation_project_amd/csrc/plan.hip:

```cpp
#include "../../include/mi3d.h"
#include <stdlib.h>

#include "ops.h"

int conv3_bn_half_forward(const ConvBnHalf& a, hipStream_t s, mi3d_conv3_bn_route* route) {
    const Geo g = a.g;
    const int training = a.training;
    bool fused_stats = false;
    int ksd = 0, c1_blocks = 0;
    Conv3Launch ln;
    bool tk = false;
    if (a.mfma) {
        tk = training && a.tk_zeroed && conv3_mfma_ticket_ok(a.Cin, a.Cout, g);
        MI3D_TRY(conv3_mfma_fwd(a.in, a.ics, a.Cin, a.wpf, a.bias, a.y, a.Cout, a.Cout, g,
                                training ? a.statpart : nullptr, a.skws, s, a.ih, Halves(),
                                training ? &ksd : nullptr, 0, 0, tk ? a.statpart : nullptr,
                                tk ? a.tkcount : nullptr, &ln));
        fused_stats = training && (tk || conv3_mfma_fuses_stats(a.Cin, a.Cout, g));
    } else if (a.c1) {
        MI3D_TRY(conv3_c1_fwd_mfma((const float*)a.in, a.w, a.bias, a.y, a.Cout, a.Cout, g,
                                   training ? a.statpart : nullptr, s));
        if (training) { fused_stats = true; c1_blocks = conv3_c1_fwd_stat_blocks(g); }
        ln.kind = 1;
    } else {
// ... 590 lines not shown
int mi3d_unet_num_buffers(const mi3d_unet_desc* d) { return d ? 6 * (2 * d->n_levels + 1) : -1; }
int mi3d_unet_num_segments(const mi3d_unet_desc* d) { return d ? 2 * d->n_levels + 2 : -1; }

size_t mi3d_unet_workspace_bytes(const mi3d_unet_desc* d) {
    Plan p;
    if (build_plan(d, p) != 0) return 0;
    return p.total;
}

int64_t mi3d_unet_dropout_count(const mi3d_unet_desc* d) {
    Plan p;
    if (build_plan(d, p) != 0) return -1;
    const HalfP& last = p.blk[p.nblk - 1].h[1];
    return last.drop_off + (int64_t)d->N * last.Cout;
}

int mi3d_unet_segment_params(const mi3d_unet_desc* d, int seg, int* r) {
    Plan p;
    MI3D_TRY(build_plan(d, p));
    int L = p.L;
    MI3D_CHECK_ARG(seg >= 0 && seg < 2 * L + 2 && r, "bad segment %d", seg);
    r[2] = r[3] = -1;
    if (seg == 0) { r[0] = p.final_pidx(); r[1] = r[0] + 2; }
    else if (seg <= L) {
        int i = L - seg;
        r[0] = p.blk[L + 1 + i].h[0].pidx; r[1] = r[0] + 8;
        r[2] = p.up_pidx(i); r[3] = r[2] + 2;
    } else if (seg == L + 1) { r[0] = p.blk[L].h[0].pidx; r[1] = r[0] + 8; }
    else { int l = 2 * L + 1 - seg; r[0] = p.blk[l].h[0].pidx; r[1] = r[0] + 8; }
    return 0;
}

}

struct HeadLoss {
    const int64_t* labels; LossCfg cfg; float* loss_out; float* coef; float* metrics_out; void* loss_ws; void* met_ws;
    const float* grad_scale;
    const float* teacher;
};
static LossCfg cfg_of(const mi3d_loss_cfg* c) {
    LossCfg k;
    k.w_ce = c->w_ce; k.region_kind = c->region_kind; k.w_reg = c->w_reg; k.alpha = c->alpha; k.beta = c->beta; k.eps = c->eps;
    k.w_kd = c->w_kd; k.temp = c->temperature > 0.f ? c->temperature : 1.f;
    return k;
}

static int unet_forward_impl(const mi3d_unet_desc* d, const float* x, const void* const* params, void* const* buffers,
                      const float* drop_scales, int training, float* logits, float* gap_out, void* workspace,
                      size_t workspace_bytes, void* stream, const HeadLoss* hl) {
    Plan p;
    Ctx c{p};
    MI3D_TRY(enter(c, p, d, "mi3d_unet_forward", x != nullptr, params, workspace, workspace_bytes, stream));
    c.beside = (training & 4) != 0;
    training &= 3;
    int L = p.L;
    if (d->in_channels > 1)
        MI3D_TRY(ncdhw_to_ndhwc(p.dt, x, c.at(p.xcl), d->in_channels, d->in_channels, d->N, p.geo[0].V(), c.s));
    {
        PackJobs J;
        J.n = 0; J.nblocks = 0;
        if (training) { J.zero = c.at<int>(p.tkcount); J.nzero = CONV3_TK_COUNTERS; }
        MI3D_TRY(add_pack_jobs(c, J, false));
        if (training && J.n > 0) c.tk_zeroed = true;
        MI3D_TRY(pack_all_launch(J, c.s));
    }
    for (int l = 0; l < L; l++) {
        const bool even = p.geo[l].D % 2 == 0 && p.geo[l].H % 2 == 0 && p.geo[l].W % 2 == 0 &&
                          p.geo[l].M() * p.C[l] < (1ll << 31) && !mi3d_routes().no_pool_fuse;
        MI3D_TRY(block_forward(c, l, x, buffers, drop_scales, training, even ? c.at(p.pool[l]) : nullptr, p.C[l]));
        if (!even) MI3D_TRY(maxpool2_fwd(p.dt, c.at(p.cat[l]), p.catcs(l), p.C[l], p.geo[l], c.at(p.pool[l]), p.C[l], c.s));
    }
    MI3D_TRY(block_forward(c, L, x, buffers, drop_scales, training));
    if (gap_out) MI3D_TRY(gap_fwd(p.dt, c.at(p.zb), p.C[L], p.C[L], d->N, p.geo[L].V(), gap_out, c.s));
    for (int i = 0; i < L; i++) {
        MI3D_TRY(up_forward(c, i));
        MI3D_TRY(block_forward(c, L + 1 + i, x, buffers, drop_scales, training));
    }
    if (hl) {
        MI3D_CHECK_ARG(head_loss_ok(p.dt, c.at(p.zd[L - 1]), p.C[0], p.C[0], d->out_channels, hl->cfg),
                       "mi3d_unet_forward_loss: no fused head + loss for this configuration (see mi3d_unet_head_loss_supported)");
        return head_loss_fwd(c.at(p.zd[L - 1]), p.C[0], p.C[0], c.P(p.final_pidx()), c.P(p.final_pidx() + 1), hl->labels, hl->teacher,
                             d->N, d->out_channels, p.geo[0].V(), hl->cfg, hl->loss_out, hl->coef, hl->loss_ws, c.s, d->D,
                             hl->metrics_out, hl->met_ws, logits);
    }
    if (logits)
        MI3D_TRY(conv1_fwd(p.dt, c.at(p.zd[L - 1]), p.C[0], p.C[0], c.P(p.final_pidx()), c.P(p.final_pidx() + 1), logits,
                           d->out_channels, d->N, p.geo[0].V(), c.s));
    return 0;
}

extern "C" {

int mi3d_unet_head_loss_forward(const mi3d_unet_desc* d, const void* const* params, const int64_t* labels, const float* teacher_logits,
                                const mi3d_loss_cfg* cfg, float* loss_out, float* coef, float* metrics_out, void* loss_workspace,
                                void* metrics_workspace, float* logits_opt, void* workspace, size_t workspace_bytes, void* stream) {
    Plan p;
    Ctx c{p};
    MI3D_TRY(enter(c, p, d, "mi3d_unet_head_loss_forward", labels && cfg && loss_out && coef && loss_workspace, params, workspace,
                   workspace_bytes, stream));
    LossCfg k = cfg_of(cfg);
    MI3D_CHECK_ARG(head_loss_ok(p.dt, c.at(p.zd[p.L - 1]), p.C[0], p.C[0], d->out_channels, k),
                   "mi3d_unet_head_loss_forward: no fused head + loss for this configuration (see mi3d_unet_head_loss_supported)");
    return head_loss_fwd(c.at(p.zd[p.L - 1]), p.C[0], p.C[0], c.P(p.final_pidx()), c.P(p.final_pidx() + 1), labels, teacher_logits, d->N,
                         d->out_channels, p.geo[0].V(), k, loss_out, coef, loss_workspace, c.s, d->D, metrics_out, metrics_workspace,
                         logits_opt);
}

int mi3d_unet_head_labels(const mi3d_unet_desc* d, const void* const* params, const int64_t* target, uint8_t* labels_out,
                          int64_t* counts, void* head_workspace, void* workspace, size_t workspace_bytes, void* stream) {
    Plan p;
    Ctx c{p};
    MI3D_TRY(enter(c, p, d, "mi3d_unet_head_labels", labels_out != nullptr, params, workspace, workspace_bytes, stream));
    return head_labels(p.dt, c.at(p.zd[p.L - 1]), p.C[0], p.C[0], c.P(p.final_pidx()), c.P(p.final_pidx() + 1), d->out_channels, d->N,
                       p.geo[0].V(), labels_out, target, counts, head_workspace, c.s);
}

int mi3d_unet_forward(const mi3d_unet_desc* d, const float* x, const void* const* params, void* const* buffers,
// ... 26 lines not shown
    BnDeferJobs J;
    J.n = 0; J.momentum = d->bn_momentum;
    for (int b = 0; b < p.nblk; b++)
        for (int h = 0; h < 2; h++) {
            const HalfP& H = p.blk[b].h[h];
            MI3D_CHECK_ARG(buffers[H.bidx] && buffers[H.bidx + 1] && side[H.bidx], "mi3d_unet_bn_apply_deferred: missing buffer %d", H.bidx);
            J.j[J.n++] = BnDeferJob{(float*)buffers[H.bidx], (float*)buffers[H.bidx + 1], (int64_t*)buffers[H.bidx + 2],
                                    (const double*)side[H.bidx], H.Cout};
        }
    return bn_deferred_apply(J, (hipStream_t)stream);
}

int mi3d_unet_infer(const mi3d_unet_desc* d, const float* x, const void* const* params, void* const* buffers,
                    float* logits, float* gap_out, void* workspace, size_t workspace_bytes, void* stream) {
    Plan p;
    Ctx c{p};
    MI3D_TRY(enter(c, p, d, "mi3d_unet_infer", x && buffers, params, workspace, workspace_bytes, stream));
    int L = p.L;
    if (d->in_channels > 1)
        MI3D_TRY(ncdhw_to_ndhwc(p.dt, x, c.at(p.xcl), d->in_channels, d->in_channels, d->N, p.geo[0].V(), c.s));
    {
        BnFoldJobs F;
        F.n = 0; F.eps = d->bn_eps;
        for (int b = 0; b < p.nblk; b++)
            for (int h = 0; h < 2; h++) {
                const HalfP& H = p.blk[b].h[h];
                MI3D_CHECK_ARG(buffers[H.bidx] && buffers[H.bidx + 1], "mi3d_unet_infer needs running statistics");
                float* scale = c.at<float>(H.stat);
                F.j[F.n++] = BnFoldJob{c.P(H.pidx + 2), c.P(H.pidx + 3), (const float*)buffers[H.bidx], (const float*)buffers[H.bidx + 1],
                                       c.P(H.pidx + 1), scale, scale + H.Cout, H.Cout};
            }
        PackJobs J;
        J.n = 0; J.nblocks = 0;
        MI3D_TRY(add_pack_jobs(c, J, true));
        MI3D_TRY(bn_fold_all(F, c.s));
        MI3D_TRY(pack_all_launch(J, c.s));
    }
    for (int l = 0; l < L; l++) {
        MI3D_TRY(block_infer(c, l, x));
        MI3D_TRY(maxpool2_fwd(p.dt, c.at(p.cat[l]), p.catcs(l), p.C[l], p.geo[l], c.at(p.pool[l]), p.C[l], c.s));
    }
    MI3D_TRY(block_infer(c, L, x));
    if (gap_out) MI3D_TRY(gap_fwd(p.dt, c.at(p.zb), p.C[L], p.C[L], d->N, p.geo[L].V(), gap_out, c.s));
    for (int i = 0; i < L; i++) {
        MI3D_TRY(up_forward(c, i));
        MI3D_TRY(block_infer(c, L + 1 + i, x));
    }
    if (logits)
        MI3D_TRY(conv1_fwd(p.dt, c.at(p.zd[L - 1]), p.C[0], p.C[0], c.P(p.final_pidx()), c.P(p.final_pidx() + 1), logits,
                           d->out_channels, d->N, p.geo[0].V(), c.s));
    return 0;
}

}

struct BwdMarks { int n = 0; int seg[4]; hipEvent_t ev[4]; };
static thread_local BwdMarks g_marks;
extern "C" int mi3d_unet_backward_marks(const int* segs, void* const* events, int n) {
    MI3D_CHECK_ARG(n >= 0 && n <= 4 && (n == 0 || (segs && events)), "mi3d_unet_backward_marks: at most 4 marks");
    g_marks.n = n;
    for (int i = 0; i < n; i++) { g_marks.seg[i] = segs[i]; g_marks.ev[i] = (hipEvent_t)events[i]; }
    return 0;
}
extern "C" int mi3d_stream_wait_event(void* stream, void* event) {
    MI3D_CHECK_ARG(event, "mi3d_stream_wait_event: null event");
    MI3D_HIP(hipStreamWaitEvent((hipStream_t)stream, (hipEvent_t)event, 0));
    return 0;
}

static int unet_backward_impl(const mi3d_unet_desc* d, const float* x, const void* const* params, void* const* grads,
                       const float* drop_scales, const float* dlogits_in, const float* dgap, float gap_scale, int accumulate,
                       int seg_begin, int seg_end, void* workspace, size_t workspace_bytes, void* stream, void* aux_stream,
                       void* const* events, int aux_join, const HeadLoss* hl) {
    Plan p;
    Ctx c{p};
    MI3D_TRY(enter(c, p, d, "mi3d_unet_backward", x && grads, params, workspace, workspace_bytes, stream));
    const float* dlogits = hl ? reinterpret_cast<const float*>(hl->coef) : dlogits_in;
    MI3D_CHECK_ARG(dlogits || dgap, "mi3d_unet_backward: neither dlogits nor dgap given");
    int L = p.L, nseg = 2 * L + 2;
    MI3D_CHECK_ARG(seg_begin >= 0 && seg_end <= nseg && seg_begin <= seg_end, "bad segment range [%d,%d)", seg_begin, seg_end);
    if (aux_stream && events) { c.s2 = (hipStream_t)aux_stream; c.ev = (hipEvent_t*)events; }
    float* wgws = c.at<float>(p.wgws);
    auto G = [&](int i) { return (float*)grads[i]; };
    BwdMarks marks = g_marks;
    g_marks.n = 0;
    for (int seg = seg_begin; seg < seg_end; seg++) {
        if (seg > seg_begin)
            for (int i = 0; i < marks.n; i++)
                if (marks.seg[i] == seg - 1) MI3D_TRY(c.pending.set_mark(marks.ev[i], c.s));
        if (seg == 0) {
            if (!dlogits) continue;
            SlabJob* ps = c.pending.first(c.s);
            if (hl) {
                MI3D_CHECK_ARG(head_loss_bwd_ok(p.dt, c.at(p.zd[L - 1]), p.C[0], p.C[0], d->out_channels, hl->cfg, c.at(p.gz[0]), p.C[0]),
                               "mi3d_unet_backward_loss: no fused head + loss for this configuration (see mi3d_unet_head_loss_supported)");
                MI3D_TRY(head_loss_bwd(c.at(p.zd[L - 1]), p.C[0], p.C[0], c.P(p.final_pidx()), c.P(p.final_pidx() + 1), hl->labels,
                                       hl->teacher, d->out_channels, hl->cfg, hl->coef, hl->grad_scale, c.at(p.gz[0]), p.C[0], G(p.final_pidx()),
                                       G(p.final_pidx() + 1), accumulate, wgws, d->N, p.geo[0].V(), c.s, ps));
            } else
                MI3D_TRY(conv1_bwd(p.dt, c.at(p.zd[L - 1]), p.C[0], p.C[0], c.P(p.final_pidx()), dlogits, d->out_channels,
                                   c.at(p.gz[0]), p.C[0], G(p.final_pidx()), G(p.final_pidx() + 1), accumulate, wgws, d->N,
                                   p.geo[0].V(), c.s, ps));
        } else if (seg <= L) {
            if (!dlogits) continue;
            int l = seg - 1, i = L - 1 - l;
            MI3D_TRY(block_backward(c, L + 1 + i, x, grads, drop_scales, c.at(p.gz[l]), p.C[l], c.at(p.gcat[l]), p.catcs(l), accumulate));
            const UpIO u = up_io(c, i);
            UpHalfBwd a{u.Cin, u.Cout, u.g, p.dt, p.up_mfma[i], u.in, u.Cin, u.w, u.wb, c.at<char>(p.gcat[l]) + u.half, u.cs, p.geo[l],
                        p.resize[l] ? c.at(p.uptmp) : nullptr, c.at(p.gz[l + 1]), u.Cin, G(p.up_pidx(i)), G(p.up_pidx(i) + 1), accumulate,
                        wgws, c.at<float>(p.wgws2), p.wgws_floats, true};
            MI3D_TRY(up_half_backward(a, c.pending, c.s));
        } else if (seg == L + 1) {
            if (dgap)
                MI3D_TRY(gap_bwd(p.dt, dgap, gap_scale, c.at(p.gz[L]), p.C[L], p.C[L], d->N, p.geo[L].V(), dlogits ? 1 : 0, c.s));
            c.pool_defer = seg + 1 < seg_end && !mi3d_routes().no_pool_splitk;
            MI3D_TRY(block_backward(c, L, x, grads, drop_scales, c.at(p.gz[L]), p.C[L], c.at(p.gp[L - 1]), p.C[L - 1], accumulate));
            c.pool_defer = false;
        } else {
            int l = 2 * L + 1 - seg;
            MI3D_TRY(maxpool2_bwd(p.dt, c.at(p.gp[l]), p.C[l], c.at(p.cat[l]), p.catcs(l), dlogits ? c.at(p.gcat[l]) : nullptr,
                                  p.catcs(l), c.at(p.gz[l]), p.C[l], p.C[l], p.geo[l], c.s,
                                  c.pool_ks > 0 ? c.at<float>(p.skws) : nullptr, c.pool_ks));
            c.pool_ks = 0;
            void* dx = l > 0 ? c.at(p.gp[l - 1]) : nullptr;
            c.pool_defer = l > 0 && seg + 1 < seg_end && !mi3d_routes().no_pool_splitk;
            MI3D_TRY(block_backward(c, l, x, grads, drop_scales, c.at(p.gz[l]), p.C[l], dx, l > 0 ? p.C[l - 1] : 0, accumulate));
            c.pool_defer = false;
        }
    }
    MI3D_TRY(c.pending.finish(c.s));
    for (int i = 0; i < marks.n; i++)
        if (marks.seg[i] == seg_end - 1) MI3D_HIP(hipEventRecord(marks.ev[i], c.s));
    if (c.s2 && c.ev) {
        MI3D_TRY(flush_deferred(c, x, grads, accumulate));
        MI3D_TRY(drain_aux(c, x, grads, accumulate, -1));
    }
    if (c.aux_used) {
        MI3D_HIP(hipEventRecord(c.ev[3], c.s2));
        if (aux_join) MI3D_HIP(hipStreamWaitEvent(c.s, c.ev[3], 0));
    }
    return 0;
}

extern "C" {

int mi3d_unet_backward(const mi3d_unet_desc* d, const float* x, const void* const* params, void* const* grads,
                       const float* drop_scales, const float* dlogits, const float* dgap, float gap_scale, int accumulate,
                       int seg_begin, int seg_end, void* workspace, size_t workspace_bytes, void* stream, void* aux_stream,
                       void* const* events, int aux_join) {
    return unet_backward_impl(d, x, params, grads, drop_scales, dlogits, dgap, gap_scale, accumulate, seg_begin, seg_end, workspace,
                              workspace_bytes, stream, aux_stream, events, aux_join, nullptr);
}

int mi3d_unet_backward_loss(const mi3d_unet_desc* d, const float* x, const void* const* params, void* const* grads,
                            const float* drop_scales, const int64_t* labels, const float* teacher_logits, const mi3d_loss_cfg* cfg,
                            const float* coef, const float* grad_scale, const float* dgap, float gap_scale, int accumulate, int seg_begin,
                            int seg_end, void* workspace, size_t workspace_bytes, void* stream, void* aux_stream, void* const* events,
                            int aux_join) {
    MI3D_CHECK_ARG(labels && cfg && coef, "mi3d_unet_backward_loss: null pointer");
    HeadLoss hl{labels, cfg_of(cfg), nullptr, const_cast<float*>(coef), nullptr, nullptr, nullptr, grad_scale, teacher_logits};
    return unet_backward_impl(d, x, params, grads, drop_scales, nullptr, dgap, gap_scale, accumulate, seg_begin, seg_end, workspace,
                              workspace_bytes, stream, aux_stream, events, aux_join, &hl);
}

}
```

multimodal_segmentation_project_amd/engine.py:

```python
import copy
import ctypes as C

import torch

from . import _lib
from ._lib import UNetDesc, call, ptr, ptr_table, stream_ptr

_default_compute_dtype = None


def set_compute_dtype(dtype):
    global _default_compute_dtype
    if dtype not in (None, torch.float32, torch.bfloat16):
        raise _lib.Mi3dError(f"unsupported compute dtype {dtype}")
    _default_compute_dtype = dtype


def resolve_compute_dtype(model):
    dt = getattr(model, "compute_dtype", None)
    if dt is None:
        dt = _default_compute_dtype
    if dt is None:
        if torch.is_autocast_enabled():
            dt = torch.bfloat16
# ... 6 lines not shown
    shape = tuple(getattr(x, "shape", x))
    if len(shape) != 5:
        raise _lib.Mi3dError(f"expected a (N,C,D,H,W) input, got shape {shape}")
    feats = [blk.double_conv[0].out_channels for blk in model.encoder]
    if len(feats) > _lib.MAX_LEVELS:
        raise _lib.Mi3dError(f"{len(feats)} levels > {_lib.MAX_LEVELS}")
    d = UNetDesc()
    d.in_channels = model.encoder[0].double_conv[0].in_channels
    d.out_channels = model.final_conv.out_channels
    d.n_levels = len(feats)
    for i, f in enumerate(feats):
        d.features[i] = f
    d.N, d.D, d.H, d.W = shape[0], shape[2], shape[3], shape[4]
    if shape[1] != d.in_channels:
        raise _lib.Mi3dError(f"input has {shape[1]} channels, model expects {d.in_channels}")
    d.dtype = _lib.dtype_code(dtype)
    bn = model.encoder[0].double_conv[1]
    if bn.momentum is None:
        raise _lib.Mi3dError("BatchNorm3d(momentum=None) (cumulative moving average) is not supported; the reference "
                             "uses the default momentum 0.1 (models/unet.py:12,16)")
    d.bn_momentum = bn.momentum
    d.bn_eps = bn.eps
    return d


def _rng_state(model, device):
    st = getattr(model, "_mi3d_rng_state", None)
    if st is None or st.device != device:
        st = torch.tensor([torch.initial_seed() & 0x7FFFFFFFFFFFFFFF, 0], dtype=torch.int64, device=device)
        model._mi3d_rng_state = st
    return st


def fill_drop_scales(buf, p, rng, injected=None, stream=None):
    if injected is not None:
        if injected.numel() != buf.numel():
            raise _lib.Mi3dError(f"injected dropout scales have {injected.numel()} entries, plan needs {buf.numel()}")
        buf.copy_(injected.reshape(buf.shape))
        return buf
    if p > 0.0:
        call("mi3d_dropout_scales", ptr(buf), buf.numel(), p, ptr(rng()), stream_ptr() if stream is None else stream)
        return buf
    return None


def make_drop_scales(model, desc, p, device, injected=None):
    out = torch.empty(_lib.lib().mi3d_unet_dropout_count(C.byref(desc)), dtype=torch.float32, device=device)
    return fill_drop_scales(out, float(p), lambda: _rng_state(model, device), injected)


TRAIN = 1
BN_PUBLISH = 2
THIN_CONSUMERS = 4


class LossGroup:

    def __init__(self, cfg, classes, device, n_metrics=4):
        lib = _lib.lib()
        self.cfg = cfg
        self.metrics = torch.empty(n_metrics, dtype=torch.float32, device=device)
        self.coef = torch.empty(_lib.LOSS_COEF_FLOATS, dtype=torch.float32, device=device)
        self.loss_ws = torch.empty(lib.mi3d_seg_loss_workspace_bytes(classes), dtype=torch.uint8, device=device)
        self.met_ws = torch.empty(lib.mi3d_seg_metrics_workspace_bytes(classes), dtype=torch.uint8, device=device)
        m = self.metrics.data_ptr()
        self.cfg_ref = C.byref(cfg)
        self.fwd = (self.cfg_ref, m, ptr(self.coef), m + 4, ptr(self.loss_ws), ptr(self.met_ws))

    def metrics_forward(self, logits, labels, *, teacher=None, stream):
        n, c, d = logits.shape[:3]
        call("mi3d_seg_loss_metrics_forward", ptr(logits), ptr(labels), ptr(teacher), n, c, d, logits.numel() // (n * c), *self.fwd, stream)

    def backward(self, logits, labels, dlogits, *, teacher=None, grad_scale, stream):
        n, c = logits.shape[:2]
        call("mi3d_seg_loss_backward", ptr(logits), ptr(labels), ptr(teacher), n, c, logits.numel() // (n * c), self.cfg_ref, ptr(self.coef),
             ptr(grad_scale), ptr(dlogits), stream)


class Plan:

    def __init__(self, model, shape, dtype, params=None, buffers=None, grads=None):
        self.desc = build_desc(model, shape, dtype)
        self.d = C.byref(self.desc)
        self.ws_bytes = _lib.lib().mi3d_unet_workspace_bytes(self.d)
        if self.ws_bytes == 0:
            _lib.check(-1, "mi3d_unet_workspace_bytes")
        self.ws = self.ws_ptr = self.gtab = None
        self.set_tables(list(model.parameters()) if params is None else params,
                        list(model.buffers()) if buffers is None else buffers, grads)

    def set_tables(self, params=None, buffers=None, grads=None):
        if params is not None:
            self.params, self.ptab = list(params), ptr_table([p.data_ptr() for p in params])
        if buffers is not None:
            self.buffers, self.btab = list(buffers), ptr_table([ptr(b) for b in buffers])
        if grads is not None:
            self.gtab = ptr_table(list(grads))

    def own_workspace(self, device):
        self.ws = torch.empty(self.ws_bytes, dtype=torch.uint8, device=device)
        self.ws_ptr = self.ws.data_ptr()
        return self

    def release_workspace(self):
        self.ws = self.ws_ptr = None

    def sibling(self, device, **tables):
        p = copy.copy(self)
        p.set_tables(**tables)
        return p.own_workspace(device)

    def forward(self, x, *, drop=None, training=TRAIN, logits=None, gap=None, stream):
        call("mi3d_unet_forward", self.d, ptr(x), self.ptab, self.btab, ptr(drop), training, ptr(logits), ptr(gap),
             self.ws_ptr, self.ws_bytes, stream)

    def infer(self, x, *, logits=None, gap=None, stream):
        call("mi3d_unet_infer", self.d, ptr(x), self.ptab, self.btab, ptr(logits), ptr(gap), self.ws_ptr, self.ws_bytes, stream)

    def forward_loss(self, x, loss, *, drop=None, training=TRAIN, labels, teacher=None, logits=None, gap=None, stream):
        call("mi3d_unet_forward_loss", self.d, ptr(x), self.ptab, self.btab, ptr(drop), training, ptr(labels), ptr(teacher),
             *loss.fwd, ptr(logits), ptr(gap), self.ws_ptr, self.ws_bytes, stream)

    def head_loss_forward(self, loss, *, labels, teacher=None, logits=None, stream):
        call("mi3d_unet_head_loss_forward", self.d, self.ptab, ptr(labels), ptr(teacher), *loss.fwd, ptr(logits),
             self.ws_ptr, self.ws_bytes, stream)

    def backward(self, x, *, drop=None, dlogits=None, dgap=None, gap_scale=1.0, accumulate=0, start, end, stream, aux=None,
                 events=None, join=1):
        call("mi3d_unet_backward", self.d, ptr(x), self.ptab, self.gtab, ptr(drop), ptr(dlogits), ptr(dgap), gap_scale,
             accumulate, start, end, self.ws_ptr, self.ws_bytes, stream, aux, events, join)

    def backward_loss(self, x, loss, *, drop=None, labels, teacher=None, grad_scale, dgap=None, gap_scale=1.0, accumulate=0,
                      start, end, stream, aux=None, events=None, join=1):
        call("mi3d_unet_backward_loss", self.d, ptr(x), self.ptab, self.gtab, ptr(drop), ptr(labels), ptr(teacher), loss.cfg_ref,
             ptr(loss.coef), ptr(grad_scale), ptr(dgap), gap_scale, accumulate, start, end, self.ws_ptr, self.ws_bytes, stream,
             aux, events, join)

    def head_labels(self, *, labels=None, out, counts=None, head_ws=None, stream):
        call("mi3d_unet_head_labels", self.d, self.ptab, ptr(labels), ptr(out), ptr(counts), ptr(head_ws), self.ws_ptr,
             self.ws_bytes, stream)

    def bn_apply_deferred(self, side, *, stream):
        call("mi3d_unet_bn_apply_deferred", self.d, self.btab, side.btab, stream)


def _outputs(desc, want_gap, device):
    logits = torch.empty((desc.N, desc.out_channels, desc.D, desc.H, desc.W), dtype=torch.float32, device=device)
    gap = None
    if want_gap:
        gap = torch.empty((desc.N, 2 * desc.features[desc.n_levels - 1]), dtype=torch.float32, device=device)
    return logits, gap


class _Hold:
    __slots__ = ("plan", "training", "want_gap", "segment_hook")


class _UNetFn(torch.autograd.Function):
    @staticmethod
    def forward(ctx, hold, x, drop, *params):
        plan = hold.plan.own_workspace(x.device)
        logits, gap = _outputs(plan.desc, hold.want_gap, x.device)
        plan.forward(x, drop=drop, training=int(hold.training), logits=logits, gap=gap, stream=stream_ptr())
        ctx.hold, ctx.drop = hold, drop
        ctx.save_for_backward(x, *params)
        ctx.set_materialize_grads(False)
        if gap is None:
            return logits
        return logits, gap

    @staticmethod
    def backward(ctx, dlogits, dgap=None):
        hold = ctx.hold
        plan = hold.plan
        x, *params = ctx.saved_tensors
        if dlogits is None and dgap is None:
            return (None, None, None) + (None,) * len(params)
        if not hold.training:
            raise _lib.Mi3dError("backward through a UNet3D forward that ran in eval mode is not supported: call "
                                 "model.train() (train_unet.py:208) or wrap evaluation in torch.no_grad()")
        if dlogits is not None:
            dlogits = dlogits.contiguous().float()
        if dgap is not None:
            dgap = dgap.contiguous().float()
        n_live = len(params) if dlogits is not None else 8 * (plan.desc.n_levels + 1)
        grads = [torch.empty_like(p) if (i < n_live and ctx.needs_input_grad[3 + i]) else None
                 for i, p in enumerate(params)]
        plan.set_tables(grads=[ptr(g) for g in grads])
        for seg in range(2 * plan.desc.n_levels + 2):
            plan.backward(x, drop=ctx.drop, dlogits=dlogits, dgap=dgap, start=seg, end=seg + 1, stream=stream_ptr())
            if hold.segment_hook is not None:
                hold.segment_hook(seg, grads)
        plan.release_workspace()
# ... 37 lines not shown
```

multimodal_segmentation_project_amd/trainer.py:

```python
import ctypes as C
import os

import torch
import torch.distributed as dist

from . import _lib, engine
from ._lib import Mi3dError, call, ptr, ptr_table, stream_ptr
from .engine import BN_PUBLISH, THIN_CONSUMERS, TRAIN
from . import metrics as M
from .dp import DataParallelComm, ParamArena

_LOSS_TABLE = {
    "combined": (1.0, 1, 1.0, 0.0, 0.0, 1e-5), "dice": (0.0, 1, 1.0, 0.0, 0.0, 1e-5),
    "tversky": (0.0, 2, 1.0, 0.5, 0.5, 1e-6), "ce_tversky": (0.3, 2, 0.7, 0.5, 0.5, 1e-6),
    "ce": (1.0, 0, 0.0, 0.0, 0.0, 1e-6),
}


def _loss_cfg(kind, kd_alpha=None, temperature=2.0):
    if kd_alpha is not None:
        return M._cfg(0.3 * kd_alpha, 2, 0.7 * kd_alpha, 0.7, 0.3, 1e-6, 1.0 - kd_alpha, temperature)
    if kind not in _LOSS_TABLE:
        raise Mi3dError(f"unknown loss {kind!r}: one of {sorted(_LOSS_TABLE)} (train_unet.py:538 --loss choices)")
    return M._cfg(*_LOSS_TABLE[kind])


def _priority_stream(device, cls):
    h = C.c_void_p()
    call("mi3d_stream_create", int(cls), C.byref(h))
    st = torch.cuda.ExternalStream(h.value, device=device)
    st.mi3d_handle = h
    return st


_STREAM_CACHE = {}
_CAPTURE_STREAMS = {}


def _capture_stream(device):
    dev = torch.device(device)
    key = dev.index if dev.index is not None else torch.cuda.current_device()
    if key not in _CAPTURE_STREAMS:
        _CAPTURE_STREAMS[key] = _priority_stream(dev, 0)
    return _CAPTURE_STREAMS[key]


def concurrent_stream(device, candidates=6, hold_us=300, role="aux"):
    import warnings
    dev = torch.device(device)
    key = (dev.index if dev.index is not None else torch.cuda.current_device(), role)
    if key in _STREAM_CACHE:
        return _STREAM_CACHE[key]
    main = torch.cuda.current_stream(device)
    buf = torch.zeros(1024, dtype=torch.float32, device=device)
    best = None
    for i in range(candidates):
        c = torch.cuda.Stream(device=device, priority=-1 if i == 0 else 0)
        times = []
        for rep in range(4):
            e0, e1 = torch.cuda.Event(enable_timing=True), torch.cuda.Event(enable_timing=True)
            torch.cuda.synchronize(device)
# ... 41 lines not shown
                    _lib.lib().mi3d_graph_destroy(g)
        self.by_variant = {}


class _State:

    def __getitem__(self, name):
        try:
            return getattr(self, name)
        except AttributeError:
            raise KeyError(name) from None


def _segment_runs(nseg, due):
    start = 0
    for seg in range(nseg):
        buckets = tuple(due.get(seg) or ())
        if buckets or seg == nseg - 1:
            yield start, seg + 1, buckets, seg == nseg - 1
            start = seg + 1


class _StepBase:
    _n_metrics = 4

    def _init_common(self, model, lr, weight_decay, betas, eps, grad_accum, process_group, compute_dtype, use_graph,
                     force_comm):
        self.model = model
        self.accum = int(grad_accum)
        if self.accum < 1:
            raise Mi3dError("grad_accum must be >= 1")
        self.micro = 0
        self.dtype = compute_dtype
        self.pg = process_group
        self.world = dist.get_world_size(process_group) if (dist.is_available() and dist.is_initialized()) else 1
        p0 = next(model.parameters())
        _lib.require_cuda(p0, type(self).__name__)
        self.device = p0.device
        self.arena = ParamArena(model.parameters(), self.device)
        self.optimizer = ArenaAdamW(model.parameters(), lr, betas, eps, weight_decay)
        n_levels = len(model.encoder)
        self.force_comm = bool(force_comm) or os.environ.get("MI3D_FORCE_COMM", "0") == "1"
        self.do_comm = self.world > 1 or (self.force_comm and dist.is_available() and dist.is_initialized())
        self.comm = DataParallelComm(self.arena, n_levels, process_group, force=self.do_comm)
        self.comm_stream = concurrent_stream(self.device, role="comm") if self.do_comm else None
        self.no_marks = bool(os.environ.get("MI3D_NO_MARKS"))
        self.comm_serial = bool(os.environ.get("MI3D_COMM_SERIAL"))
        self._mark_handles = []
        self.use_graph = bool(use_graph)
        self.keep_logits = False
        self._statics = {}
        self._static = None
        self.inv_accum = torch.full((), 1.0 / self.accum, dtype=torch.float32, device=self.device)
        self._closed = False

    def _prepare(self, x, mode="train"):
        dt = self.dtype or engine.resolve_compute_dtype(self.model)
        trainable = tuple(bool(p.requires_grad) for p in self.arena.params)
        key = (tuple(x.shape), dt, trainable, mode)
        st = self._statics.get(key)
        if st is None:
            st = self._new_state(key, self.cfg if mode == "train" else self.eval_cfg)
            self._extend(st)
            self._statics[key] = st
        if mode == "train":
            self._static = st
        return st

    def _new_state(self, key, cfg):
        shape, dt, trainable, mode = key
        dev = self.device
        st = _State()
        st.mode, st.trainable, st.graphs = mode, trainable, _Graphs()
        st.plan = engine.Plan(self.model, shape, dt, params=self.arena.params,
                              grads=[g if t else None for g, t in zip(self.arena.grad_ptrs(), trainable)]).own_workspace(dev)
        desc = st.desc = st.plan.desc
        st.L = desc.n_levels
        st.x = torch.empty(shape, dtype=torch.float32, device=dev)
        st.y = torch.empty((desc.N, desc.D * desc.H * desc.W), dtype=torch.int64, device=dev)
        st.loss = engine.LossGroup(cfg, desc.out_channels, dev, self._n_metrics)
        st.metrics = st.loss.metrics
        st.logits_shape = (desc.N, desc.out_channels, desc.D, desc.H, desc.W)
        keep = True
        if mode == "train":
            st.fused_head = (not _lib.get_route("no_head_loss") and
                             _lib.lib().mi3d_unet_head_loss_supported(st.plan.d, st.loss.cfg_ref) == 1)
            st.drop = torch.empty(_lib.lib().mi3d_unet_dropout_count(st.plan.d), dtype=torch.float32, device=dev)
            keep = not st.fused_head or self.keep_logits
            st.dlogits = torch.empty(st.logits_shape, dtype=torch.float32, device=dev) if keep else None
        st.logits = torch.empty(st.logits_shape, dtype=torch.float32, device=dev) if keep else None
        return st

    def _extend(self, st):
        pass

    def _load(self, st, non_blocking, **tensors):
        for name, t in tensors.items():
            st[name].copy_(t.reshape(st[name].shape), non_blocking=non_blocking)

    def step_static(self, last_batch=False):
        st = self._static
        if st is None:
            raise Mi3dError("step_static() before any step()/load_batch()")
        self._run(st, last_batch=last_batch)
        return st.metrics

# ... 31 lines not shown
        pass

    def __del__(self):
        self.close()

    def broadcast_parameters(self):
        self.comm.broadcast_parameters(self.model.buffers())

    def sync_buffers(self):
        self.comm.sync_buffers(self.model.buffers())

    def _on_comm_stream(self, fn):
        cs = self.comm_stream
        cs.wait_stream(torch.cuda.current_stream())
        aux = getattr(self, "aux_stream", None)
        if aux is not None:
            cs.wait_stream(aux)
        with torch.cuda.stream(cs):
            fn()

    def _join_comm(self):
        torch.cuda.current_stream().wait_stream(self.comm_stream)

    def _adamw(self, arena, ranges, hyper, s):
        lr, b1, b2, eps, wd = hyper
        for k, (lo, hi) in enumerate(ranges):
            call("mi3d_adamw_apply", arena.p.data_ptr() + 4 * lo, arena.g.data_ptr() + 4 * lo,
                 arena.m.data_ptr() + 4 * lo, arena.v.data_ptr() + 4 * lo, hi - lo, lr, b1, b2, eps, wd, 1.0,
                 ptr(arena.step), int(k == len(ranges) - 1), s)

    @staticmethod
    def _trainable_ranges(arena, trainable):
        ranges = []
        for i, t in enumerate(trainable):
            if not t:
                continue
            lo, hi = arena.range_of(i, i + 1)
            if ranges and ranges[-1][1] == lo:
                ranges[-1] = (ranges[-1][0], hi)
            else:
                ranges.append((lo, hi))
        return ranges

    def _variant(self):
        return (self.micro % self.accum == 0, (self.micro + 1) % self.accum == 0)

    def _run(self, st, last_batch=False):
        self._check_mode()
        variant = self._variant()
        bump = 1
        if last_batch and not variant[1]:
            variant = (variant[0], True)
            bump = self.accum - (self.micro % self.accum)
        if not self.use_graph:
            self._enqueue(st, variant, lambda fn: fn())
            self.micro += bump
            return
        gr = st.graphs
        hyper = self._hyper()
        if gr.hyper != hyper:
            gr.drop()
            gr.hyper = hyper
        segs = gr.by_variant.get(variant)
        if segs is None:
            segs = gr.by_variant[variant] = self._capture(st, variant)
        for g, fn in segs:
            call("mi3d_graph_launch", g, stream_ptr())
            if fn is not None:
                fn()
        self.micro += bump

    def _mutable_state(self):
        a = self.arena
        return [a.p, a.g, a.m, a.v, a.step] + list(self.model.buffers()) + [engine._rng_state(self.model, self.device)]

    def _capture(self, st, variant):
        s = torch.cuda.Stream(device=self.device)
        s.wait_stream(torch.cuda.current_stream())
        segs = []
        with torch.cuda.stream(s):
            state = self._mutable_state()
            snap = [t.clone() for t in state]
            self._enqueue(st, variant, lambda fn: fn())
            if self.do_comm:
                self._join_comm()
                self.comm_stream.synchronize()
            s.synchronize()
            for t, c in zip(state, snap):
                t.copy_(c)
            s.synchronize()
        cs = _capture_stream(self.device)
        cs.wait_stream(s)
        with torch.cuda.stream(cs):
            def cut(fn):
                g = C.c_void_p()
                call("mi3d_graph_end", cs.cuda_stream, C.byref(g))
                segs.append((g, fn))
                call("mi3d_graph_begin", cs.cuda_stream)

            call("mi3d_graph_begin", cs.cuda_stream)
            try:
                self._enqueue(st, variant, cut)
            finally:
                g = C.c_void_p()
                call("mi3d_graph_end", cs.cuda_stream, C.byref(g))
                segs.append((g, None))
        torch.cuda.current_stream().wait_stream(s)
        torch.cuda.current_stream().wait_stream(cs)
        return segs


class TrainStep(_StepBase):
    def __init__(self, model, loss="combined", lr=1e-3, weight_decay=0.01, betas=(0.9, 0.999), eps=1e-8,
                 grad_accum=1, kd_teacher=None, kd_alpha=0.7, kd_temperature=2.0, process_group=None,
                 compute_dtype=None, use_graph=False, aux_wgrad=None, reference_zero_grad_quirk=False,
                 force_comm=False, overlap_teacher=True, keep_logits=False):
        cfg = _loss_cfg(loss, kd_alpha if kd_teacher is not None else None, kd_temperature)
        self._init_common(model, lr, weight_decay, betas, eps, grad_accum, process_group, compute_dtype, use_graph,
                          force_comm)
        self.teacher = kd_teacher
        self.loss_kind = loss
        self.cfg = cfg
        self.keep_logits = bool(keep_logits)
        self.eval_cfg = _loss_cfg("combined" if kd_teacher is not None else loss)
        self.quirk = bool(reference_zero_grad_quirk) and kd_teacher is None
        if kd_teacher is not None:
            self._check_teacher(kd_teacher)
        self.kd_stream = concurrent_stream(self.device, role="kd") if (kd_teacher is not None and overlap_teacher) else None
        if aux_wgrad is None:
            aux_wgrad = not use_graph and not self.do_comm
        self.aux_stream = concurrent_stream(self.device) if aux_wgrad else None
        self._event_handles = [_lib.new_event() for _ in range(4)] if aux_wgrad else []
        self._events = ptr_table(self._event_handles) if aux_wgrad else None
        if self.world > 1:
            self.broadcast_parameters()

    def _close_extra(self):
        for e in self._event_handles:
            _lib.lib().mi3d_event_destroy(e)
        self._event_handles = []

    def _check_teacher(self, teacher):
        sp, tp = list(self.model.parameters()), list(teacher.parameters())
        sb, tb = list(self.model.buffers()), list(teacher.buffers())
        if len(sp) != len(tp) or len(sb) != len(tb):
            raise Mi3dError(f"kd_teacher has {len(tp)} parameters / {len(tb)} buffers, the student {len(sp)} / {len(sb)}: "
                            "teacher and student must be the same UNet3D architecture (distill_unet.py:214-215)")
        for kind, mine, theirs in (("parameter", sp, tp), ("buffer", sb, tb)):
            for i, (a, b) in enumerate(zip(mine, theirs)):
                if b.device != self.device:
                    raise Mi3dError(f"kd_teacher {kind} {i} is on {b.device}, the student on {self.device}: move the "
                                    "teacher with .to(device) first (no CPU fallback)")
                if tuple(a.shape) != tuple(b.shape) or a.dtype != b.dtype:
                    raise Mi3dError(f"kd_teacher {kind} {i}: shape/dtype {tuple(b.shape)}/{b.dtype} != student's "
                                    f"{tuple(a.shape)}/{a.dtype}")
                if not b.is_contiguous():
                    raise Mi3dError(f"kd_teacher {kind} {i} is not contiguous")

    def reset_optimizer(self):
        self.arena.m.zero_()
        self.arena.v.zero_()
        self.arena.step.zero_()
        self._drop_graphs()
        self._statics = {}
        self._static = None

    def _extend(self, st):
        if st.mode != "train":
            return
        desc, trainable, dev = st.desc, st.trainable, self.device
        st.opt_ranges = self._trainable_ranges(self.arena, trainable)
        last = -1
        r = (C.c_int * 4)()
        for seg in range(2 * st.L + 2):
            _lib.check(_lib.lib().mi3d_unet_segment_params(st.plan.d, seg, r), "mi3d_unet_segment_params")
            idx = list(range(r[0], r[1])) + (list(range(r[2], r[3])) if r[2] >= 0 else [])
            if any(trainable[i] for i in idx):
                last = seg
        st.nseg_run = last + 1
        sched = {}
        for seg, (lo, hi) in self.comm.buckets.items():
            live = any(t and lo <= o < hi for o, t in zip(self.arena.offsets, trainable))
            if live and last >= 0:
                sched.setdefault(min(seg, last), []).append(seg)
        if self.comm_serial and sched and last >= 0:
            sched = {last: [b for sg in sorted(sched) for b in sched[sg]]}
        st.comm_after = sched
        if self.teacher is not None:
            st.teacher = st.plan.sibling(dev, params=list(self.teacher.parameters()), buffers=list(self.teacher.buffers()))
            st.t_logits = torch.empty(st.logits_shape, dtype=torch.float32, device=dev)

    def _check_mode(self):
        if not self.model.training:
            raise Mi3dError("TrainStep.step() on a model in eval mode: the backward kernels use batch statistics "
                            "(train_unet.py:208 calls model.train() first); use evaluate() for eval-mode passes")

    def _enqueue(self, st, variant, comm):
        first, boundary = variant
        s = stream_ptr()
        if self.quirk:
            accumulate, run_backward = 0, boundary
        else:
            accumulate, run_backward = (0 if first else 1), True
        drop, t_logits = self._forward_loss(st, s)
        self._backward_exchange(st, s, comm, drop, t_logits, accumulate, boundary, run_backward)
        if boundary:
            self._adamw(self.arena, st.opt_ranges, self._hyper(), s)

    def _forward_loss(self, st, s):
        model, plan, loss = self.model, st.plan, st.loss
        drop = engine.fill_drop_scales(st.drop, float(getattr(model, "dropout_rate", 0.0)),
                                       lambda: engine._rng_state(model, self.device),
                                       getattr(model, "_mi3d_injected_drop_scales", None), s)
        teacher, ks = (st.teacher if self.teacher is not None else None), self.kd_stream
        if teacher is not None and ks is not None:
            ks.wait_stream(torch.cuda.current_stream())
            with torch.cuda.stream(ks):
                teacher.infer(st.x, logits=st.t_logits, stream=ks.cuda_stream)
        fused = st.fused_head
        keep = st.logits if self.keep_logits else None
        if fused and teacher is None:
            plan.forward_loss(st.x, loss, drop=drop, labels=st.y, logits=keep, stream=s)
        else:
            plan.forward(st.x, drop=drop, logits=None if fused else st.logits, stream=s)
        t_logits = None
        if teacher is not None:
            if ks is not None:
                torch.cuda.current_stream().wait_stream(ks)
            else:
                teacher.infer(st.x, logits=st.t_logits, stream=s)
            t_logits = st.t_logits
            if fused:
                plan.head_loss_forward(loss, labels=st.y, teacher=t_logits, logits=keep, stream=s)
        if not fused:
            loss.metrics_forward(st.logits, st.y, teacher=t_logits, stream=s)
        return drop, t_logits

    def _backward_exchange(self, st, s, comm, drop, t_logits, accumulate, boundary, run_backward):
        met = st.metrics
        met_pending = self.do_comm
        joined = False

        def exchange(buckets):
            nonlocal met_pending
            with_met, met_pending = met_pending, False

            def fn():
                if with_met:
                    self.comm.average_(met)
                for k in buckets:
                    self.comm.reduce_bucket(k)
            return fn

        if run_backward:
            if not st.fused_head:
                st.loss.backward(st.logits, st.y, st.dlogits, teacher=t_logits, grad_scale=self.inv_accum, stream=s)
            nseg = st.nseg_run
            due = st.comm_after if (self.do_comm and boundary) else {}
            aux = self.aux_stream.cuda_stream if self.aux_stream is not None else None
            aux_open = False
            mid = [(sg, tuple(due[sg])) for sg in range(nseg - 1) if due.get(sg)]
            use_marks = bool(mid) and not self.use_graph and aux is None and len(mid) <= 4 and not self.no_marks
            if use_marks:
                while len(self._mark_handles) < len(mid):
                    self._mark_handles.append(_lib.new_event())
                call("mi3d_unet_backward_marks", (C.c_int * len(mid))(*[sg for sg, _ in mid]),
                     ptr_table(self._mark_handles[:len(mid)]), len(mid))
                due = {sg: b for sg, b in due.items() if sg >= nseg - 1}
            for start, end, buckets, last in _segment_runs(nseg, due):
                join = 1 if (last or self.use_graph or aux is None) else 0
                aux_open = aux_open or (aux is not None and not join)
                kw = dict(drop=drop, accumulate=accumulate, start=start, end=end, stream=s, aux=aux, events=self._events, join=join)
                if st.fused_head:
                    st.plan.backward_loss(st.x, st.loss, labels=st.y, teacher=t_logits, grad_scale=self.inv_accum, **kw)
                else:
                    st.plan.backward(st.x, dlogits=st.dlogits, **kw)
                if use_marks:
                    cs = self.comm_stream
                    for i, (sg, b) in enumerate(mid):
                        fn = exchange(b)
                        call("mi3d_stream_wait_event", cs.cuda_stream, self._mark_handles[i])
                        with torch.cuda.stream(cs):
                            fn()
                if buckets and not last:
                    comm(lambda fn=exchange(buckets): self._on_comm_stream(fn))
                elif buckets:
                    joined = True
                    comm(self._join_comm)
                    comm(exchange(buckets))
            if aux_open:
                torch.cuda.current_stream().wait_stream(self.aux_stream)
        if met_pending:
            comm(lambda: self._on_comm_stream(lambda: self.comm.average_(met)))
        if self.do_comm and not joined:
            comm(self._join_comm)

    def load_batch(self, images, labels):
        self._load(self._prepare(images), False, x=images, y=labels)

    def step(self, images, labels, last_batch=False):
        self._load(self._prepare(images), True, x=images, y=labels)
        return self.step_static(last_batch=last_batch)

    @torch.no_grad()
    def evaluate(self, images, labels):
        if self.do_comm:
            self.sync_buffers()
        st = self._prepare(images, mode="eval")
        st.x.copy_(images)
        st.y.copy_(labels.reshape(st.y.shape))
        plan, loss, s = st.plan, st.loss, stream_ptr()
        fused = (not _lib.get_route("no_head_loss") and not self.keep_logits and
                 _lib.lib().mi3d_unet_head_loss_supported(plan.d, loss.cfg_ref) == 1)
        if fused:
            plan.infer(st.x, stream=s)
            plan.head_loss_forward(loss, labels=st.y, stream=s)
        else:
            plan.infer(st.x, logits=st.logits, stream=s)
            loss.metrics_forward(st.logits, st.y, stream=s)
        out = st.metrics.clone()
        self.comm.average_(out)
        return out


class DannStep(_StepBase):
    _n_metrics = 5

    def __init__(self, seg_model, disc_model, loss="ce_tversky", lambda_domain=0.1, lr=1e-3, weight_decay=0.01,
                 betas=(0.9, 0.999), eps=1e-8, grad_accum=1, process_group=None, compute_dtype=None, use_graph=False,
                 force_comm=False, overlap_forwards=True):
        self._init_common(seg_model, lr, weight_decay, betas, eps, grad_accum, process_group, compute_dtype, use_graph,
                          force_comm)
        self.fwd_stream = concurrent_stream(self.device, role="fwd") if overlap_forwards else None
        self.disc = disc_model
        self.lam = float(lambda_domain)
        self.cfg = _loss_cfg(loss)
        self.eval_cfg = self.cfg
        self.lins = [disc_model.net[0], disc_model.net[3], disc_model.net[6], disc_model.net[8]]
        self.disc_p = [float(disc_model.net[2].p), float(disc_model.net[5].p)]
        for p in disc_model.parameters():
            _lib.require_cuda(p, "DannStep discriminator")
        self.disc_arena = ParamArena(disc_model.parameters(), self.device)
        self.disc_optimizer = ArenaAdamW(disc_model.parameters(), lr, betas, eps, weight_decay)
        if self.world > 1:
            self.broadcast_parameters()
            dist.broadcast(self.disc_arena.p, src=0, group=process_group)

    def _hyper(self):
        g = self.disc_optimizer.param_groups[0]
        return super()._hyper() + (float(g["lr"]), float(g["betas"][0]), float(g["betas"][1]), float(g["eps"]),
                                   float(g["weight_decay"]))

    def _mutable_state(self):
        d = self.disc_arena
        return super()._mutable_state() + [d.p, d.g, d.m, d.v, d.step, self._disc_rng()]

    def _disc_rng(self):
        st = getattr(self.disc, "_mi3d_rng_state", None)
        if st is None or st.device != self.device:
            st = torch.tensor([(torch.initial_seed() + 0x5DEECE66D) & 0x7FFFFFFFFFFFFFFF, 0], dtype=torch.int64,
# ... 143 lines not shown
```

Before: 978.8 volumes/s.

## Fuse AdamW update with bf16 weight repacking and ride step increment on backward

Adds a fused optimizer tail. The AdamW update writes the packed bf16 MFMA weight images for conv and upconv layers directly, so the next forward can skip its own weight-packing pass (PREPACKED flag). The step-counter increment rides on the last backward pending-sum launch instead of a separate launch. A version and serial token tracks whether the packs are still current, and evaluation or broadcasting parameters invalidates them. This removes separate pack_all and optimizer launches and repeated weight reads, in exchange for more complex state tracking and a risk of stale packs if parameters are changed outside the tracked paths.

```diff
diff --git a/include/mi3d.h b/include/mi3d.h
--- a/include/mi3d.h
+++ b/include/mi3d.h
@@ -43,6 +43,8 @@
                        int accumulate, int seg_begin, int seg_end, void* workspace, size_t workspace_bytes,
                        void* stream, void* aux_stream, void* const* events, int aux_join);
 int mi3d_unet_backward_marks(const int* segs, void* const* events, int n);
+int mi3d_backward_step_rider(int64_t* step_dev);
+int mi3d_backward_step_rode(void);
 int mi3d_stream_wait_event(void* stream, void* event);
 int mi3d_event_create(void** event_out);
 int mi3d_event_destroy(void* event);
@@ -121,6 +123,25 @@
                     float eps, float weight_decay, float grad_scale, int64_t* step_dev, void* stream);
 int mi3d_adamw_apply(float* p, const float* g, float* m, float* v, int64_t n, float lr, float beta1, float beta2,
                      float eps, float weight_decay, float grad_scale, int64_t* step_dev, int increment, void* stream);
+typedef struct mi3d_pack_tensor {
+    int32_t kind;
+    int32_t Cin, Cout;
+    int32_t N, D, H, W;
+    int32_t reserved;
+    int64_t offset;
+    void* image_a;
+    void* image_b;
+} mi3d_pack_tensor;
+int mi3d_adamw_pack(float* p, const float* g, float* m, float* v, int64_t n, const mi3d_pack_tensor* tensors, int n_tensors,
+                    const int64_t* ranges, int n_ranges, float lr, float beta1, float beta2, float eps, float weight_decay,
+                    float grad_scale, int64_t* step_dev, int step_incremented, int32_t* zero, int n_zero, void* stream);
+int mi3d_adamw_pack_check(const void* p, const void* g, const void* m, const void* v, int64_t n, const mi3d_pack_tensor* tensors,
+                          int n_tensors, const int64_t* ranges, int n_ranges, int* pack_blocks_out, int* flat_jobs_out);
+int mi3d_pack_all(const float* p, int64_t n, const mi3d_pack_tensor* tensors, int n_tensors, int32_t* zero, int n_zero, void* stream);
+int mi3d_adamw_pack_unet(const mi3d_unet_desc* d, const void* const* params, float* p, const float* g, float* m, float* v, int64_t n,
+                         const int64_t* ranges, int n_ranges, float lr, float beta1, float beta2, float eps, float weight_decay,
+                         float grad_scale, int64_t* step_dev, int step_incremented, void* workspace, size_t workspace_bytes,
+                         void* stream);
 int mi3d_dropout_scales(float* out, int64_t n, float p, uint64_t* state_dev, void* stream);
 
 int mi3d_preprocess_ct(const float* in, float* out, int64_t n, float window_min, float window_max, void* stream);
@@ -225,6 +246,7 @@
                            int flags, mi3d_conv3_bn_bwd_route* route_out, int Cout, int N, int D, int H, int W, void* workspace,
                            size_t workspace_bytes, void* stream);
 int mi3d_pending_sum_launch(const mi3d_pending_sum* job, void* stream);
+int mi3d_pending_sum_launch_step(const mi3d_pending_sum* job, int64_t* step_dev, void* stream);
 size_t mi3d_bn_workspace_bytes(int C);
 int mi3d_bn_relu_drop_forward(int dtype, const void* y, int ycs, int C, int64_t M, int64_t V, const float* gamma,
                               const float* beta, float* running_mean, float* running_var, int64_t* num_batches_tracked,
diff --git a/multimodal_segmentation_project_amd/_lib.py b/multimodal_segmentation_project_amd/_lib.py
--- a/multimodal_segmentation_project_amd/_lib.py
+++ b/multimodal_segmentation_project_amd/_lib.py
@@ -71,6 +71,12 @@
 
 UP_BWD_LEAVE_PENDING, UP_BWD_SECOND_WORKSPACE = 1, 2
 
+class PackTensor(C.Structure):
+    _fields_ = [(k, C.c_int32) for k in ("kind", "Cin", "Cout", "N", "D", "H", "W", "reserved")] + \
+               [("offset", C.c_int64), ("image_a", C.c_void_p), ("image_b", C.c_void_p)]
+
+
+_TP = C.POINTER(PackTensor)
 _DP, _LP, _AP, _MP = C.POINTER(UNetDesc), C.POINTER(LossCfg), C.POINTER(AugParams), C.POINTER(MaskList)
 
 _SIGS = {
@@ -124,6 +130,13 @@
     "mi3d_softmax_ce_rows": (i32, [vp, vp, i32, i32, vp, vp, f32, vp]),
     "mi3d_adamw_step": (i32, [vp, vp, vp, vp, i64, f32, f32, f32, f32, f32, f32, vp, vp]),
     "mi3d_adamw_apply": (i32, [vp, vp, vp, vp, i64, f32, f32, f32, f32, f32, f32, vp, i32, vp]),
+    "mi3d_adamw_pack": (i32, [vp, vp, vp, vp, i64, _TP, i32, C.POINTER(i64), i32, f32, f32, f32, f32, f32, f32, vp, i32, vp, i32, vp]),
+    "mi3d_adamw_pack_check": (i32, [vp, vp, vp, vp, i64, _TP, i32, C.POINTER(i64), i32, C.POINTER(C.c_int), C.POINTER(C.c_int)]),
+    "mi3d_pack_all": (i32, [vp, i64, _TP, i32, vp, i32, vp]),
+    "mi3d_adamw_pack_unet": (i32, [_DP, vp, vp, vp, vp, vp, i64, C.POINTER(i64), i32, f32, f32, f32, f32, f32, f32, vp, i32, vp, sz, vp]),
+    "mi3d_backward_step_rider": (i32, [vp]),
+    "mi3d_backward_step_rode": (i32, []),
+    "mi3d_pending_sum_launch_step": (i32, [C.POINTER(PendingSum), vp, vp]),
     "mi3d_dropout_scales": (i32, [vp, i64, f32, vp, vp]),
     "mi3d_preprocess_ct": (i32, [vp, vp, i64, f32, f32, vp]),
     "mi3d_preprocess_mri_workspace_bytes": (sz, []),
diff --git a/multimodal_segmentation_project_amd/csrc/adamw.h b/multimodal_segmentation_project_amd/csrc/adamw.h
--- /dev/null
+++ b/multimodal_segmentation_project_amd/csrc/adamw.h
@@ -0,0 +1,14 @@
+#pragma once
+#include "common.h"
+
+#ifdef __HIPCC__
+__device__ __forceinline__ void adamw_one(float& pi, float gi, float& mi, float& vi, float decay, float b1, float b2, float eps,
+                                          float grad_scale, float bc2s, float step_size) {
+#pragma clang fp contract(off)
+    gi = gi * grad_scale;
+    mi = __builtin_fmaf(b1, mi, (1.f - b1) * gi);
+    vi = __builtin_fmaf(b2, vi, ((1.f - b2) * gi) * gi);
+    float denom = sqrtf(vi) / bc2s + eps;
+    pi = __builtin_fmaf(decay, pi, -(step_size * (mi / denom)));
+}
+#endif
diff --git a/multimodal_segmentation_project_amd/csrc/api.hip b/multimodal_segmentation_project_amd/csrc/api.hip
--- a/multimodal_segmentation_project_amd/csrc/api.hip
+++ b/multimodal_segmentation_project_amd/csrc/api.hip
@@ -291,6 +291,52 @@
     memcpy(&q, job, sizeof(q));
     return slab_job_launch(q, (hipStream_t)stream);
 }
+int mi3d_pending_sum_launch_step(const mi3d_pending_sum* job, int64_t* step_dev, void* stream) {
+    MI3D_CHECK_ARG(job && step_dev, "mi3d_pending_sum_launch_step: null job / step counter");
+    SlabJob q;
+    memcpy(&q, job, sizeof(q));
+    MI3D_CHECK_ARG(q.nblocks > 0, "mi3d_pending_sum_launch_step: an empty job launches nothing, the counter would not move");
+    return slab_job_launch(q, (hipStream_t)stream, step_dev);
+}
+
+static int pack_tensor_list(const mi3d_pack_tensor* t, int nt, OptPackTensor* out, const char* fn) {
+    MI3D_CHECK_ARG(nt >= 0 && nt <= MAX_PACK_JOBS && (nt == 0 || t), "%s: bad tensor list (at most %d tensors)", fn, MAX_PACK_JOBS);
+    for (int i = 0; i < nt; i++)
+        out[i] = OptPackTensor{t[i].kind, t[i].Cin, t[i].Cout, Geo{t[i].N, t[i].D, t[i].H, t[i].W}, t[i].offset, t[i].image_a, t[i].image_b, nullptr};
+    return 0;
+}
+int mi3d_adamw_pack(float* p, const float* g, float* m, float* v, int64_t n, const mi3d_pack_tensor* tensors, int n_tensors,
+                    const int64_t* ranges, int n_ranges, float lr, float beta1, float beta2, float eps, float weight_decay,
+                    float grad_scale, int64_t* step_dev, int step_incremented, int32_t* zero, int n_zero, void* stream) {
+    OptPackTensor t[MAX_PACK_JOBS];
+    MI3D_TRY(pack_tensor_list(tensors, n_tensors, t, "mi3d_adamw_pack"));
+    return adamw_pack(p, g, m, v, n, t, n_tensors, ranges, n_ranges, AdamwHyper{lr, beta1, beta2, eps, weight_decay, grad_scale}, step_dev,
+                      step_incremented, zero, n_zero, (hipStream_t)stream);
+}
+int mi3d_adamw_pack_check(const void* p, const void* g, const void* m, const void* v, int64_t n, const mi3d_pack_tensor* tensors,
+                          int n_tensors, const int64_t* ranges, int n_ranges, int* pack_blocks_out, int* flat_jobs_out) {
+    OptPackTensor t[MAX_PACK_JOBS];
+    MI3D_TRY(pack_tensor_list(tensors, n_tensors, t, "mi3d_adamw_pack_check"));
+    OptPackJobs J;
+    MI3D_TRY(adamw_pack_plan(J, p, g, m, v, n, t, n_tensors, ranges, n_ranges));
+    if (pack_blocks_out) *pack_blocks_out = J.nblocks_pack;
+    if (flat_jobs_out) *flat_jobs_out = J.nflat;
+    return 0;
+}
+int mi3d_pack_all(const float* p, int64_t n, const mi3d_pack_tensor* tensors, int n_tensors, int32_t* zero, int n_zero, void* stream) {
+    OptPackTensor t[MAX_PACK_JOBS];
+    MI3D_TRY(pack_tensor_list(tensors, n_tensors, t, "mi3d_pack_all"));
+    OptPackJobs chk;
+    MI3D_TRY(adamw_pack_plan(chk, p, p, p, p, n, t, n_tensors, nullptr, 0));
+    PackJobs J;
+    J.n = 0; J.nblocks = 0;
+    if (n_zero > 0) { MI3D_CHECK_ARG(zero, "mi3d_pack_all: null counter space"); J.zero = zero; J.nzero = n_zero; }
+    for (int i = 0; i < n_tensors; i++) {
+        if (t[i].kind == 0) MI3D_TRY(pack_all_add_conv3(J, p + t[i].off, t[i].Cin, t[i].Cout, t[i].a, t[i].b, t[i].g));
+        else MI3D_TRY(pack_all_add_upconv(J, p + t[i].off, t[i].Cin, t[i].Cout, t[i].a));
+    }
+    return pack_all_launch(J, (hipStream_t)stream);
+}
 
 }
 
diff --git a/multimodal_segmentation_project_amd/csrc/conv3_mfma.hip b/multimodal_segmentation_project_amd/csrc/conv3_mfma.hip
--- a/multimodal_segmentation_project_amd/csrc/conv3_mfma.hip
+++ b/multimodal_segmentation_project_amd/csrc/conv3_mfma.hip
@@ -4,6 +4,7 @@
 
 #include <hip/hip_ext.h>
 
+#include "adamw.h"
 #include "mfma_tile.h"
 #include "ops.h"
 #include "slab_sum.h"
@@ -40,6 +41,26 @@
 }
 
 constexpr int PK_LD = 16 * 27 + 1;
+template <int TPB>
+__device__ __forceinline__ void pack_pair_images(const float* wl, bf16* __restrict__ wf, bf16* __restrict__ wd, int mode_f, int mode_d,
+                                                 int CIBN, int COBN, int cib, int cob) {
+    for (int q = threadIdx.x; q < 2 * 14 * 64; q += TPB) {
+        int img = q / (14 * 64), r = q - img * (14 * 64);
+        int s = r >> 6, lane = r & 63, g = lane >> 4, o = lane & 15;
+        int tap = ktap(img ? mode_d : mode_f, s, g >> 1);
+        bf16x8 v;
+#pragma unroll
+        for (int j = 0; j < 8; j++) {
+            int ic = 8 * (g & 1) + j;
+            float f = 0.f;
+            if (tap < 27) f = img ? wl[ic * PK_LD + o * 27 + (26 - tap)] : wl[o * PK_LD + ic * 27 + tap];
+            v[j] = (bf16)f;
+        }
+        bf16* dst = img ? wd + ((((int64_t)cob * 14 + s) * CIBN + cib) * 64 + lane) * 8
+                        : wf + ((((int64_t)cib * 14 + s) * COBN + cob) * 64 + lane) * 8;
+        *reinterpret_cast<bf16x8*>(dst) = v;
+    }
+}
 __global__ __launch_bounds__(BLK) void pack_all_kernel(PackJobs J) {
     __shared__ float wl[16 * PK_LD];
     if (blockIdx.x == 0 && J.zero)
@@ -62,22 +83,7 @@
             for (int j = 0; j < 4; j++) wl[row * PK_LD + k + j] = v[j] * f;
         }
         __syncthreads();
-        for (int q = threadIdx.x; q < 2 * 14 * 64; q += BLK) {
-            int img = q / (14 * 64), r = q - img * (14 * 64);
-            int s = r >> 6, lane = r & 63, g = lane >> 4, o = lane & 15;
-            int tap = ktap(img ? mode_d : mode_f, s, g >> 1);
-            bf16x8 v;
-#pragma unroll
-            for (int j = 0; j < 8; j++) {
-                int ic = 8 * (g & 1) + j;
-                float f = 0.f;
-                if (tap < 27) f = img ? wl[ic * PK_LD + o * 27 + (26 - tap)] : wl[o * PK_LD + ic * 27 + tap];
-                v[j] = (bf16)f;
-            }
-            bf16* dst = img ? wd + ((((int64_t)cob * 14 + s) * CIBN + cib) * 64 + lane) * 8
-                            : wf + ((((int64_t)cib * 14 + s) * COBN + cob) * 64 + lane) * 8;
-            *reinterpret_cast<bf16x8*>(dst) = v;
-        }
+        pack_pair_images<BLK>(wl, wf, wd, mode_f, mode_d, CIBN, COBN, cib, cob);
     } else {
         bf16* wf = (bf16*)J.j[ji].a; bf16* wb = (bf16*)J.j[ji].b;
         int64_t n = (int64_t)Cin * Cout * 8;
@@ -101,6 +107,156 @@
             for (int j = 0; j < 8; j++) v[j] = (bf16)w[((int64_t)ci * Cout + co0 + j) * 8 + tap];
         }
         *reinterpret_cast<bf16x8*>((bw ? wb : wf) + k) = v;
+    }
+}
+
+constexpr int OPT_BLK = 256;
+constexpr int OPT_FLAT_EW = 1024;
+constexpr int UP_LD = 16 * 8 + 1;
+struct AdamwCoef { float decay, b1, b2, eps, grad_scale, bc2s, step_size; };
+__device__ __forceinline__ AdamwCoef adamw_coef(const AdamwHyper& h, const int64_t* step_dev) {
+    double step = (double)(*step_dev);
+    float bc1 = (float)(1.0 - pow((double)h.b1, step));
+    AdamwCoef c;
+    c.bc2s = (float)sqrt(1.0 - pow((double)h.b2, step));
+    c.step_size = h.lr / bc1;
+    c.decay = __builtin_fmaf(-h.lr, h.wd, 1.f);
+    c.b1 = h.b1; c.b2 = h.b2; c.eps = h.eps; c.grad_scale = h.grad_scale;
+    return c;
+}
+__device__ __forceinline__ void adamw_four(f32x4& p, const f32x4& g, f32x4& m, f32x4& v, const AdamwCoef& c) {
+#pragma unroll
+    for (int j = 0; j < 4; j++) {
+        float pj = p[j], mj = m[j], vj = v[j];
+        adamw_one(pj, g[j], mj, vj, c.decay, c.b1, c.b2, c.eps, c.grad_scale, c.bc2s, c.step_size);
+        p[j] = pj; m[j] = mj; v[j] = vj;
+    }
+}
+template <int NQ, typename EOff, typename Put>
+__device__ __forceinline__ void adamw_piece(const OptPackJobs& J, int64_t off, bool train, EOff eoff, Put put) {
+    float* __restrict__ p = J.p + off;
+    const float* __restrict__ g = J.g + off;
+    float* __restrict__ m = J.m + off;
+    float* __restrict__ v = J.v + off;
+    int idx = threadIdx.x;
+    bool have = idx < NQ;
+    int64_t e = 0;
+    f32x4 p4 = {0.f, 0.f, 0.f, 0.f}, g4 = p4, m4 = p4, v4 = p4;
+    if (have) {
+        e = eoff(idx);
+        p4 = *reinterpret_cast<const f32x4*>(p + e);
+        if (train) {
+            g4 = *reinterpret_cast<const f32x4*>(g + e); m4 = *reinterpret_cast<const f32x4*>(m + e);
+            v4 = *reinterpret_cast<const f32x4*>(v + e);
+        }
+    }
+    AdamwCoef c{};
+    if (train) c = adamw_coef(J.h, J.step);
+    while (have) {
+        const int nidx = idx + OPT_BLK;
+        const bool have2 = nidx < NQ;
+        int64_t e2 = 0;
+        f32x4 p5 = p4, g5 = g4, m5 = m4, v5 = v4;
+        if (have2) {
+            e2 = eoff(nidx);
+            p5 = *reinterpret_cast<const f32x4*>(p + e2);
+            if (train) {
+                g5 = *reinterpret_cast<const f32x4*>(g + e2); m5 = *reinterpret_cast<const f32x4*>(m + e2);
+                v5 = *reinterpret_cast<const f32x4*>(v + e2);
+            }
+        }
+        if (train) {
+            adamw_four(p4, g4, m4, v4, c);
+            *reinterpret_cast<f32x4*>(m + e) = m4;
+            *reinterpret_cast<f32x4*>(v + e) = v4;
+            *reinterpret_cast<f32x4*>(p + e) = p4;
+        }
+        put(idx, p4);
+        idx = nidx; have = have2; e = e2; p4 = p5; g4 = g5; m4 = m5; v4 = v5;
+    }
+}
+__global__ __launch_bounds__(OPT_BLK) void adamw_pack_kernel(OptPackJobs J) {
+    __shared__ float wl[16 * PK_LD];
+    static_assert(32 * UP_LD <= 16 * PK_LD, "the transposed conv piece fits the conv piece's LDS");
+    if (blockIdx.x == 0 && J.zero)
+        for (int i = threadIdx.x; i < J.nzero; i += OPT_BLK) J.zero[i] = 0;
+    const int b = blockIdx.x;
+    if (b >= J.nblocks_pack) {
+        int fb = b - J.nblocks_pack, fi = 0;
+        while (fi + 1 < J.nflat && fb >= J.f[fi + 1].blk0) fi++;
+        const int64_t lo = J.f[fi].lo + (int64_t)(fb - J.f[fi].blk0) * OPT_FLAT_EW, left = J.f[fi].lo + J.f[fi].n - lo;
+        const int cnt = (int)(left < OPT_FLAT_EW ? left : OPT_FLAT_EW);
+        float* __restrict__ p = J.p + lo;
+        const float* __restrict__ g = J.g + lo;
+        float* __restrict__ m = J.m + lo;
+        float* __restrict__ v = J.v + lo;
+        const bool vec = ((reinterpret_cast<uintptr_t>(p) | reinterpret_cast<uintptr_t>(g) | reinterpret_cast<uintptr_t>(m) |
+                           reinterpret_cast<uintptr_t>(v)) & 15) == 0;
+        const int n4 = vec ? cnt >> 2 : 0, i = threadIdx.x;
+        static_assert(OPT_FLAT_EW <= 4 * OPT_BLK, "at most one 16-byte quad per thread");
+        f32x4 p4, g4, m4, v4;
+        if (i < n4) {
+            g4 = reinterpret_cast<const f32x4*>(g)[i]; p4 = reinterpret_cast<const f32x4*>(p)[i];
+            m4 = reinterpret_cast<const f32x4*>(m)[i]; v4 = reinterpret_cast<const f32x4*>(v)[i];
+        }
+        const AdamwCoef c = adamw_coef(J.h, J.step);
+        if (i < n4) {
+            adamw_four(p4, g4, m4, v4, c);
+            reinterpret_cast<f32x4*>(m)[i] = m4; reinterpret_cast<f32x4*>(v)[i] = v4; reinterpret_cast<f32x4*>(p)[i] = p4;
+        }
+        for (int k = n4 * 4 + i; k < cnt; k += OPT_BLK) {
+            float pi = p[k], mi = m[k], vi = v[k];
+            adamw_one(pi, g[k], mi, vi, c.decay, c.b1, c.b2, c.eps, c.grad_scale, c.bc2s, c.step_size);
+            m[k] = mi; v[k] = vi; p[k] = pi;
+        }
+        return;
+    }
+    int ji = 0;
+    while (ji + 1 < J.n && b >= J.j[ji + 1].blk0) ji++;
+    const int Cin = J.j[ji].Cin, Cout = J.j[ji].Cout, lb = b - J.j[ji].blk0;
+    const bool train = J.j[ji].train != 0;
+    const int64_t off = J.j[ji].off;
+    if (J.j[ji].kind == 0) {
+        const int CIBN = Cin / 16, COBN = Cout / 16;
+        const int cib = lb % CIBN, cob = lb / CIBN;
+        const float* __restrict__ sc = J.j[ji].scale;
+        adamw_piece<16 * 108>(J, off, train,
+            [&](int idx) { int row = idx / 108, k = (idx - row * 108) * 4; return ((int64_t)(cob * 16 + row) * Cin + cib * 16) * 27 + k; },
+            [&](int idx, const f32x4& p4) {
+                int row = idx / 108, k = (idx - row * 108) * 4;
+                float f = sc ? sc[cob * 16 + row] : 1.f;
+#pragma unroll
+                for (int j = 0; j < 4; j++) wl[row * PK_LD + k + j] = p4[j] * f;
+            });
+        __syncthreads();
+        pack_pair_images<OPT_BLK>(wl, (bf16*)J.j[ji].a, (bf16*)J.j[ji].b, J.j[ji].mode_f, J.j[ji].mode_d, CIBN, COBN, cib, cob);
+    } else {
+        const int KS = Cin / 32, COBN = Cout / 16, S = Cout / 4;
+        const int ks = lb % KS, cb = lb / KS;
+        adamw_piece<32 * 32>(J, off, train,
+            [&](int idx) { return ((int64_t)(32 * ks + (idx >> 5)) * Cout + cb * 16) * 8 + (idx & 31) * 4; },
+            [&](int idx, const f32x4& p4) {
+#pragma unroll
+                for (int j = 0; j < 4; j++) wl[(idx >> 5) * UP_LD + (idx & 31) * 4 + j] = p4[j];
+            });
+        __syncthreads();
+        bf16* wf = (bf16*)J.j[ji].a; bf16* wb = (bf16*)J.j[ji].b;
+        for (int q = threadIdx.x; q < 2 * 512; q += OPT_BLK) {
+            const int r = q & 511;
+            bf16x8 v;
+            if (q < 512) {
+                int tap = r >> 6, lane = r & 63, G = lane >> 4, col = lane & 15;
+#pragma unroll
+                for (int j = 0; j < 8; j++) v[j] = (bf16)wl[(8 * G + j) * UP_LD + col * 8 + tap];
+                *reinterpret_cast<bf16x8*>(wf + ((((int64_t)tap * COBN + cb) * KS + ks) * 64 + lane) * 8) = v;
+            } else {
+                int cl = r >> 8, tap = (r >> 5) & 7, h = (r >> 4) & 1, cil = r & 15;
+                int kk0 = tap * Cout + cb * 16 + 8 * h, s = kk0 >> 5, G = (kk0 & 31) >> 3;
+#pragma unroll
+                for (int j = 0; j < 8; j++) v[j] = (bf16)wl[(cl * 16 + cil) * UP_LD + (8 * h + j) * 8 + tap];
+                *reinterpret_cast<bf16x8*>(wb + ((((int64_t)(2 * ks + cl)) * S + s) * 64 + G * 16 + cil) * 8) = v;
+            }
+        }
     }
 }
 
@@ -987,6 +1143,89 @@
     return 0;
 }
 
+int adamw_pack_plan(OptPackJobs& J, const void* p, const void* g, const void* m, const void* v, int64_t n, const OptPackTensor* t, int nt,
+                    const int64_t* ranges, int nranges) {
+    MI3D_CHECK_ARG(p && g && m && v && n >= 0, "adamw_pack: null arena pointer");
+    MI3D_CHECK_ARG(nt >= 0 && nt <= MAX_PACK_JOBS && (nt == 0 || t), "adamw_pack: bad tensor list (at most %d tensors)", MAX_PACK_JOBS);
+    MI3D_CHECK_ARG(nranges >= 0 && (nranges == 0 || ranges), "adamw_pack: bad range list");
+    MI3D_CHECK_ARG(nt == 0 || (((uintptr_t)p | (uintptr_t)g | (uintptr_t)m | (uintptr_t)v) & 15) == 0,
+                   "adamw_pack: the arenas of packed tensors must be 16-byte aligned");
+    int64_t prev = 0;
+    for (int r = 0; r < nranges; r++) {
+        const int64_t lo = ranges[2 * r], hi = ranges[2 * r + 1];
+        MI3D_CHECK_ARG(lo >= prev && hi > lo && hi <= n, "adamw_pack: range %d [%lld, %lld) is off the arena (%lld floats) or out of order",
+                       r, (long long)lo, (long long)hi, (long long)n);
+        prev = hi;
+    }
+    J.n = 0; J.nflat = 0;
+    int nblocks = 0, ord[MAX_PACK_JOBS];
+    int64_t numel[MAX_PACK_JOBS];
+    for (int i = 0; i < nt; i++) {
+        const OptPackTensor& q = t[i];
+        MI3D_CHECK_ARG(q.kind == 0 || q.kind == 1, "adamw_pack: tensor %d: bad kind %d", i, q.kind);
+        if (q.kind == 0) MI3D_CHECK_ARG(q.Cin >= 16 && q.Cout >= 16 && q.Cin % 16 == 0 && q.Cout % 16 == 0 && q.a && q.b,
+                                        "adamw_pack: tensor %d: conv %d -> %d has no MFMA image / null image pointer", i, q.Cin, q.Cout);
+        else MI3D_CHECK_ARG(q.Cin >= 32 && q.Cout >= 16 && q.Cin % 32 == 0 && q.Cout % 16 == 0 && q.a,
+                            "adamw_pack: tensor %d: transposed conv %d -> %d has no MFMA image / null image pointer", i, q.Cin, q.Cout);
+        numel[i] = (int64_t)q.Cin * q.Cout * (q.kind == 0 ? 27 : 8);
+        MI3D_CHECK_ARG(q.off >= 0 && q.off % 4 == 0 && q.off + numel[i] <= n, "adamw_pack: tensor %d at %lld (+%lld) is off the arena or not 16-byte aligned",
+                       i, (long long)q.off, (long long)numel[i]);
+        int train = 0;
+        for (int r = 0; r < nranges; r++) {
+            const int64_t lo = ranges[2 * r], hi = ranges[2 * r + 1];
+            if (q.off >= lo && q.off + numel[i] <= hi) train = 1;
+            else MI3D_CHECK_ARG(q.off + numel[i] <= lo || q.off >= hi, "adamw_pack: tensor %d straddles the end of range %d", i, r);
+        }
+        OptPackJob& j = J.j[J.n++];
+        j = OptPackJob{q.off, q.a, q.kind == 0 ? q.b : (void*)((bf16*)q.a + numel[i]), q.scale, q.Cin, q.Cout, q.kind,
+                       q.kind == 0 && persist_ok(q.Cin, q.Cout, q.g) ? 1 : 0, q.kind == 0 && persist_ok(q.Cout, q.Cin, q.g) ? 1 : 0, nblocks, train};
+        nblocks += q.kind == 0 ? (q.Cin / 16) * (q.Cout / 16) : (q.Cin / 32) * (q.Cout / 16);
+        int k = i;
+        for (; k > 0 && t[ord[k - 1]].off > q.off; k--) ord[k] = ord[k - 1];
+        ord[k] = i;
+    }
+    for (int i = 0; i + 1 < nt; i++)
+        MI3D_CHECK_ARG(t[ord[i]].off + numel[ord[i]] <= t[ord[i + 1]].off, "adamw_pack: tensors %d and %d overlap", ord[i], ord[i + 1]);
+    J.nblocks_pack = nblocks;
+    int fblocks = 0;
+    auto flat = [&](int64_t lo, int64_t hi) {
+        if (hi <= lo) return 0;
+        MI3D_CHECK_ARG(J.nflat < MAX_FLAT_JOBS, "adamw_pack: more than %d flat ranges", MAX_FLAT_JOBS);
+        MI3D_CHECK_ARG(fblocks + (hi - lo + OPT_FLAT_EW - 1) / OPT_FLAT_EW < (1 << 30), "adamw_pack: flat range too long");
+        J.f[J.nflat++] = OptFlatJob{lo, hi - lo, fblocks};
+        fblocks += cdiv(hi - lo, OPT_FLAT_EW);
+        return 0;
+    };
+    for (int r = 0; r < nranges; r++) {
+        int64_t cur = ranges[2 * r];
+        const int64_t hi = ranges[2 * r + 1];
+        for (int i = 0; i < nt; i++) {
+            const OptPackTensor& q = t[ord[i]];
+            if (q.off < cur || q.off >= hi) continue;
+            MI3D_TRY(flat(cur, q.off));
+            cur = q.off + numel[ord[i]];
+        }
+        MI3D_TRY(flat(cur, hi));
+    }
+    J.nblocks = nblocks + fblocks;
+    return 0;
+}
+int adamw_pack(float* p, const float* g, float* m, float* v, int64_t n, const OptPackTensor* t, int nt, const int64_t* ranges,
+               int nranges, AdamwHyper h, int64_t* step_dev, int step_incremented, int* zero, int nzero, hipStream_t s) {
+    OptPackJobs L;
+    MI3D_TRY(adamw_pack_plan(L, p, g, m, v, n, t, nt, ranges, nranges));
+    MI3D_CHECK_ARG(step_dev != nullptr && (nzero == 0 || zero) && nzero >= 0, "adamw_pack: null step counter / counter space");
+    L.p = p; L.g = g; L.m = m; L.v = v; L.step = step_dev; L.zero = nzero ? zero : nullptr; L.nzero = nzero; L.h = h;
+    if (!step_incremented) MI3D_TRY(adamw_step(nullptr, nullptr, nullptr, nullptr, 0, 0.f, 0.f, 0.f, 0.f, 0.f, 0.f, step_dev, s, 1));
+    if (L.nblocks == 0) {
+        if (L.zero) MI3D_HIP(hipMemsetAsync(L.zero, 0, (size_t)nzero * sizeof(int), s));
+        return 0;
+    }
+    adamw_pack_kernel<<<L.nblocks, OPT_BLK, 0, s>>>(L);
+    MI3D_LAUNCH_CHECK();
+    return 0;
+}
+
 int conv3_mfma_stat_blocks(int Cin, int Cout, Geo g) {
     if (persist_ok(Cin, Cout, g)) return persist_grid(Cin, Cout, g);
     if (big_geo(g)) return g.N * cdiv(g.D, 4) * cdiv(g.H, 8) * cdiv(g.W, 16);
@@ -1611,10 +1850,16 @@
 
 }
 
-__global__ __launch_bounds__(BLK) void slab_job_kernel(SlabJob q) { slab_job_run(q, (int)blockIdx.x); }
-int slab_job_launch(const SlabJob& q, hipStream_t s) {
+__global__ __launch_bounds__(BLK) void slab_job_kernel(SlabJob q, int64_t* step_inc) {
+    if ((int)blockIdx.x >= q.nblocks) {
+        if (threadIdx.x == 0) *step_inc += 1;
+        return;
+    }
+    slab_job_run(q, (int)blockIdx.x);
+}
+int slab_job_launch(const SlabJob& q, hipStream_t s, int64_t* step_inc) {
     if (q.nblocks <= 0) return 0;
-    slab_job_kernel<<<q.nblocks, BLK, 0, s>>>(q);
+    slab_job_kernel<<<q.nblocks + (step_inc ? 1 : 0), BLK, 0, s>>>(q, step_inc);
     MI3D_LAUNCH_CHECK();
     return 0;
 }
diff --git a/multimodal_segmentation_project_amd/csrc/misc.hip b/multimodal_segmentation_project_amd/csrc/misc.hip
--- a/multimodal_segmentation_project_amd/csrc/misc.hip
+++ b/multimodal_segmentation_project_amd/csrc/misc.hip
@@ -1,6 +1,7 @@
 #include <stdarg.h>
 #include <stdio.h>
 
+#include "adamw.h"
 #include "ops.h"
 
 static thread_local char g_err[512] = "";
@@ -154,15 +155,6 @@
     if (lane == 0 && loss) *loss = (float)(tot / (double)M);
 }
 
-__device__ __forceinline__ void adamw_one(float& pi, float gi, float& mi, float& vi, float decay, float b1, float b2, float eps,
-                                          float grad_scale, float bc2s, float step_size) {
-#pragma clang fp contract(off)
-    gi = gi * grad_scale;
-    mi = __builtin_fmaf(b1, mi, (1.f - b1) * gi);
-    vi = __builtin_fmaf(b2, vi, ((1.f - b2) * gi) * gi);
-    float denom = sqrtf(vi) / bc2s + eps;
-    pi = __builtin_fmaf(decay, pi, -(step_size * (mi / denom)));
-}
 __global__ __launch_bounds__(BLK) void adamw_kernel(float* __restrict__ p, const float* __restrict__ g, float* __restrict__ m,
                                                     float* __restrict__ v, int64_t n, float lr, float b1, float b2, float eps, float wd,
                                                     float grad_scale, const int64_t* __restrict__ step_dev) {
diff --git a/multimodal_segmentation_project_amd/csrc/ops.h b/multimodal_segmentation_project_amd/csrc/ops.h
--- a/multimodal_segmentation_project_amd/csrc/ops.h
+++ b/multimodal_segmentation_project_amd/csrc/ops.h
@@ -28,6 +28,22 @@
                        const float* scale = nullptr);
 int pack_all_add_upconv(PackJobs& J, const float* w, int Cin, int Cout, void* wp);
 int pack_all_launch(const PackJobs& J, hipStream_t s);
+struct OptPackTensor { int kind, Cin, Cout; Geo g; int64_t off; void* a; void* b; const float* scale; };
+struct AdamwHyper { float lr, b1, b2, eps, wd, grad_scale; };
+struct OptPackJob { int64_t off; void* a; void* b; const float* scale; int Cin, Cout, kind, mode_f, mode_d, blk0, train; };
+struct OptFlatJob { int64_t lo, n; int blk0; };
+constexpr int MAX_FLAT_JOBS = 40;
+struct OptPackJobs {
+    float* p; const float* g; float* m; float* v; const int64_t* step; int* zero; int nzero;
+    int n, nflat, nblocks_pack, nblocks;
+    AdamwHyper h;
+    OptPackJob j[MAX_PACK_JOBS]; OptFlatJob f[MAX_FLAT_JOBS];
+};
+static_assert(sizeof(OptPackJobs) <= 4096, "the job table travels as a kernel argument");
+int adamw_pack(float* p, const float* g, float* m, float* v, int64_t n, const OptPackTensor* t, int nt, const int64_t* ranges,
+               int nranges, AdamwHyper h, int64_t* step_dev, int step_incremented, int* zero, int nzero, hipStream_t s);
+int adamw_pack_plan(OptPackJobs& J, const void* p, const void* g, const void* m, const void* v, int64_t n, const OptPackTensor* t, int nt,
+                    const int64_t* ranges, int nranges);
 int conv3_mfma_stat_blocks(int Cin, int Cout, Geo g);
 size_t conv3_mfma_splitk_floats(int Cin, int Cout, Geo g);
 bool conv3_mfma_fuses_stats(int Cin, int Cout, Geo g);
@@ -98,7 +114,7 @@
            const float* stat, const float* drop, void* dy, int dycs, float* dgamma, float* dbeta,
            int accumulate, float* ws, hipStream_t s, const SlabJob* extra = nullptr, const float* skp = nullptr, int ks = 0,
            const SlabJob* extra2 = nullptr);
-int slab_job_launch(const SlabJob& q, hipStream_t s);
+int slab_job_launch(const SlabJob& q, hipStream_t s, int64_t* step_inc = nullptr);
 
 int bn_train_stats_splitk(const float* skp, int ks, const float* bias, void* y, int ycs, int C, int64_t M, const float* gamma,
                           const float* beta, float* running_mean, float* running_var, int64_t* num_batches_tracked,
@@ -130,11 +146,14 @@
 struct Pending {
     SlabJob pend, pend2;
     hipEvent_t mark = nullptr;
+    int64_t* step_inc = nullptr;
+    bool step_rode = false;
     static bool waits(const SlabJob& j) { return j.nblocks > 0; }
-    int flush(hipStream_t s) {
+    int flush(hipStream_t s, int64_t* inc = nullptr) {
         int rc = 0;
-        if (waits(pend)) { rc = slab_job_launch(pend, s); pend.nblocks = 0; }
-        if (waits(pend2)) { int r2 = slab_job_launch(pend2, s); pend2.nblocks = 0; if (!rc) rc = r2; }
+        const bool two = waits(pend) && waits(pend2);
+        if (waits(pend)) { rc = slab_job_launch(pend, s, two ? nullptr : inc); pend.nblocks = 0; }
+        if (waits(pend2)) { int r2 = slab_job_launch(pend2, s, inc); pend2.nblocks = 0; if (!rc) rc = r2; }
         return rc;
     }
     SlabJob* first(hipStream_t s) {
@@ -157,7 +176,9 @@
         return 0;
     }
     int finish(hipStream_t s) {
-        MI3D_TRY(flush(s));
+        int64_t* inc = (waits(pend) || waits(pend2)) ? step_inc : nullptr;
+        if (inc) { step_rode = true; step_inc = nullptr; }
+        MI3D_TRY(flush(s, inc));
         return rode(s);
     }
     int set_mark(hipEvent_t ev, hipStream_t s) {
diff --git a/multimodal_segmentation_project_amd/csrc/plan.hip b/multimodal_segmentation_project_amd/csrc/plan.hip
--- a/multimodal_segmentation_project_amd/csrc/plan.hip
+++ b/multimodal_segmentation_project_amd/csrc/plan.hip
@@ -666,7 +666,9 @@
     Ctx c{p};
     MI3D_TRY(enter(c, p, d, "mi3d_unet_forward", x != nullptr, params, workspace, workspace_bytes, stream));
     c.beside = (training & 4) != 0;
+    const bool prepacked = (training & 8) != 0;
     training &= 3;
+    MI3D_CHECK_ARG(!prepacked || training, "mi3d_unet_forward: training | 8 (prepacked) needs a training forward");
     int L = p.L;
     if (d->in_channels > 1)
         MI3D_TRY(ncdhw_to_ndhwc(p.dt, x, c.at(p.xcl), d->in_channels, d->in_channels, d->N, p.geo[0].V(), c.s));
@@ -676,7 +678,7 @@
         if (training) { J.zero = c.at<int>(p.tkcount); J.nzero = CONV3_TK_COUNTERS; }
         MI3D_TRY(add_pack_jobs(c, J, false));
         if (training && J.n > 0) c.tk_zeroed = true;
-        MI3D_TRY(pack_all_launch(J, c.s));
+        if (!prepacked) MI3D_TRY(pack_all_launch(J, c.s));
     }
     for (int l = 0; l < L; l++) {
         const bool even = p.geo[l].D % 2 == 0 && p.geo[l].H % 2 == 0 && p.geo[l].W % 2 == 0 &&
@@ -809,6 +811,34 @@
     return 0;
 }
 
+int mi3d_adamw_pack_unet(const mi3d_unet_desc* d, const void* const* params, float* p, const float* g, float* m, float* v, int64_t n,
+                         const int64_t* ranges, int n_ranges, float lr, float beta1, float beta2, float eps, float weight_decay,
+                         float grad_scale, int64_t* step_dev, int step_incremented, void* workspace, size_t workspace_bytes,
+                         void* stream) {
+    Plan pl;
+    Ctx c{pl};
+    MI3D_TRY(enter(c, pl, d, "mi3d_adamw_pack_unet", p && g && m && v && step_dev, params, workspace, workspace_bytes, stream));
+    OptPackTensor t[MAX_PACK_JOBS];
+    int nt = 0;
+    auto add = [&](int kind, int pidx, int Cin, int Cout, Geo geo, void* a, void* b) {
+        MI3D_CHECK_ARG(nt < MAX_PACK_JOBS, "mi3d_adamw_pack_unet: too many packed tensors");
+        MI3D_CHECK_ARG(c.P(pidx) != nullptr, "mi3d_adamw_pack_unet: parameter %d is NULL", pidx);
+        t[nt++] = OptPackTensor{kind, Cin, Cout, geo, (int64_t)(c.P(pidx) - p), a, b, nullptr};
+        return 0;
+    };
+    for (int b = 0; b < pl.nblk; b++)
+        for (int h = 0; h < 2; h++) {
+            const HalfP& H = pl.blk[b].h[h];
+            if (H.mfma) MI3D_TRY(add(0, H.pidx, H.Cin, H.Cout, pl.geo[pl.blk[b].level], c.at(H.wpf), c.at(H.wpd)));
+        }
+    for (int i = 0; i < pl.L; i++) {
+        const int l = pl.L - 1 - i;
+        if (pl.up_mfma[i]) MI3D_TRY(add(1, pl.up_pidx(i), 2 * pl.C[l], pl.C[l], pl.geo[l + 1], c.at(pl.upw[i]), nullptr));
+    }
+    return adamw_pack(p, g, m, v, n, t, nt, ranges, n_ranges, AdamwHyper{lr, beta1, beta2, eps, weight_decay, grad_scale}, step_dev,
+                      step_incremented, c.at<int>(pl.tkcount), CONV3_TK_COUNTERS, c.s);
+}
+
 }
 
 struct BwdMarks { int n = 0; int seg[4]; hipEvent_t ev[4]; };
@@ -819,6 +849,13 @@
     for (int i = 0; i < n; i++) { g_marks.seg[i] = segs[i]; g_marks.ev[i] = (hipEvent_t)events[i]; }
     return 0;
 }
+static thread_local int64_t* g_step_rider = nullptr;
+static thread_local int g_step_rode = 0;
+extern "C" int mi3d_backward_step_rider(int64_t* step_dev) {
+    g_step_rider = step_dev;
+    return 0;
+}
+extern "C" int mi3d_backward_step_rode(void) { return g_step_rode; }
 extern "C" int mi3d_stream_wait_event(void* stream, void* event) {
     MI3D_CHECK_ARG(event, "mi3d_stream_wait_event: null event");
     MI3D_HIP(hipStreamWaitEvent((hipStream_t)stream, (hipEvent_t)event, 0));
@@ -841,6 +878,9 @@
     auto G = [&](int i) { return (float*)grads[i]; };
     BwdMarks marks = g_marks;
     g_marks.n = 0;
+    int64_t* const step_rider = g_step_rider;
+    g_step_rider = nullptr;
+    g_step_rode = 0;
     for (int seg = seg_begin; seg < seg_end; seg++) {
         if (seg > seg_begin)
             for (int i = 0; i < marks.n; i++)
@@ -885,7 +925,9 @@
             c.pool_defer = false;
         }
     }
+    c.pending.step_inc = step_rider;
     MI3D_TRY(c.pending.finish(c.s));
+    g_step_rode = c.pending.step_rode ? 1 : 0;
     for (int i = 0; i < marks.n; i++)
         if (marks.seg[i] == seg_end - 1) MI3D_HIP(hipEventRecord(marks.ev[i], c.s));
     if (c.s2 && c.ev) {
diff --git a/multimodal_segmentation_project_amd/engine.py b/multimodal_segmentation_project_amd/engine.py
--- a/multimodal_segmentation_project_amd/engine.py
+++ b/multimodal_segmentation_project_amd/engine.py
@@ -82,6 +82,7 @@
 TRAIN = 1
 BN_PUBLISH = 2
 THIN_CONSUMERS = 4
+PREPACKED = 8
 
 
 class LossGroup:
@@ -169,6 +170,14 @@
     def head_labels(self, *, labels=None, out, counts=None, head_ws=None, stream):
         call("mi3d_unet_head_labels", self.d, self.ptab, ptr(labels), ptr(out), ptr(counts), ptr(head_ws), self.ws_ptr,
              self.ws_bytes, stream)
+
+    def step_rider(self, step):
+        call("mi3d_backward_step_rider", ptr(step))
+
+    def adamw_pack(self, arena, ranges, n_ranges, hyper, *, rode, stream):
+        lr, b1, b2, eps, wd = hyper
+        call("mi3d_adamw_pack_unet", self.d, self.ptab, ptr(arena.p), ptr(arena.g), ptr(arena.m), ptr(arena.v), arena.numel, ranges,
+             n_ranges, lr, b1, b2, eps, wd, 1.0, ptr(arena.step), int(rode), self.ws_ptr, self.ws_bytes, stream)
 
     def bn_apply_deferred(self, side, *, stream):
         call("mi3d_unet_bn_apply_deferred", self.d, self.btab, side.btab, stream)
diff --git a/multimodal_segmentation_project_amd/trainer.py b/multimodal_segmentation_project_amd/trainer.py
--- a/multimodal_segmentation_project_amd/trainer.py
+++ b/multimodal_segmentation_project_amd/trainer.py
@@ -6,7 +6,7 @@
 
 from . import _lib, engine
 from ._lib import Mi3dError, call, ptr, ptr_table, stream_ptr
-from .engine import BN_PUBLISH, THIN_CONSUMERS, TRAIN
+from .engine import BN_PUBLISH, PREPACKED, THIN_CONSUMERS, TRAIN
 from . import metrics as M
 from .dp import DataParallelComm, ParamArena
 
@@ -154,6 +154,7 @@
         self._statics = {}
         self._static = None
         self.inv_accum = torch.full((), 1.0 / self.accum, dtype=torch.float32, device=self.device)
+        self._opt_serial = 0
         self._closed = False
 
     def _prepare(self, x, mode="train"):
@@ -291,8 +292,10 @@
         if last_batch and not variant[1]:
             variant = (variant[0], True)
             bump = self.accum - (self.micro % self.accum)
+        variant = self._last_variant = self._tail_variant(st, variant)
         if not self.use_graph:
             self._enqueue(st, variant, lambda fn: fn())
+            self._ran(st, variant)
             self.micro += bump
             return
         gr = st.graphs
@@ -307,7 +310,18 @@
             call("mi3d_graph_launch", g, stream_ptr())
             if fn is not None:
                 fn()
+        self._ran(st, variant)
         self.micro += bump
+
+    def _tail_variant(self, st, variant):
+        return variant
+
+    def _ran(self, st, variant):
+        if variant[1]:
+            self._opt_serial += 1
+
+    def _after_warmup(self, st, variant):
+        pass
 
     def _mutable_state(self):
         a = self.arena
@@ -327,6 +341,7 @@
             s.synchronize()
             for t, c in zip(state, snap):
                 t.copy_(c)
+            self._after_warmup(st, variant)
             s.synchronize()
         cs = _capture_stream(self.device)
         cs.wait_stream(s)
@@ -353,7 +368,7 @@
     def __init__(self, model, loss="combined", lr=1e-3, weight_decay=0.01, betas=(0.9, 0.999), eps=1e-8,
                  grad_accum=1, kd_teacher=None, kd_alpha=0.7, kd_temperature=2.0, process_group=None,
                  compute_dtype=None, use_graph=False, aux_wgrad=None, reference_zero_grad_quirk=False,
-                 force_comm=False, overlap_teacher=True, keep_logits=False):
+                 force_comm=False, overlap_teacher=True, keep_logits=False, fused_tail=None):
         cfg = _loss_cfg(loss, kd_alpha if kd_teacher is not None else None, kd_temperature)
         self._init_common(model, lr, weight_decay, betas, eps, grad_accum, process_group, compute_dtype, use_graph,
                           force_comm)
@@ -361,6 +376,7 @@
         self.loss_kind = loss
         self.cfg = cfg
         self.keep_logits = bool(keep_logits)
+        self.fused_tail = (not os.environ.get("MI3D_NO_FUSED_TAIL")) if fused_tail is None else bool(fused_tail)
         self.eval_cfg = _loss_cfg("combined" if kd_teacher is not None else loss)
         self.quirk = bool(reference_zero_grad_quirk) and kd_teacher is None
         if kd_teacher is not None:
@@ -404,11 +420,43 @@
         self._statics = {}
         self._static = None
 
+    def invalidate_packs(self):
+        self._opt_serial += 1
+
+    def broadcast_parameters(self):
+        super().broadcast_parameters()
+        self.invalidate_packs()
+
+    def _tail_fused(self, st):
+        return st.mode == "train" and st.tail_ok and not self.do_comm and self.fused_tail
+
+    def _pack_token(self):
+        return (self.arena.p._version,) + tuple(p._version for p in self._packed_params)
+
+    def _tail_variant(self, st, variant):
+        if not self._tail_fused(st):
+            return variant
+        current = st.pack_serial == self._opt_serial and st.pack_token == self._pack_token()
+        return variant + (True, current)
+
+    def _ran(self, st, variant):
+        super()._ran(st, variant)
+        if variant[1] and len(variant) > 2:
+            st.pack_serial, st.pack_token = self._opt_serial, self._pack_token()
+
+    def _after_warmup(self, st, variant):
+        if len(variant) > 2:
+            st.plan.adamw_pack(self.arena, None, 0, self._hyper(), rode=True, stream=stream_ptr())
+
     def _extend(self, st):
         if st.mode != "train":
             return
         desc, trainable, dev = st.desc, st.trainable, self.device
         st.opt_ranges = self._trainable_ranges(self.arena, trainable)
+        st.tail_ranges = (C.c_int64 * (2 * len(st.opt_ranges)))(*[v for r in st.opt_ranges for v in r])
+        st.tail_ok = desc.dtype == _lib.DTYPE_BF16
+        st.pack_serial = st.pack_token = None
+        self._packed_params = [p for p in self.arena.params if p.dim() == 5]
         last = -1
         r = (C.c_int * 4)()
         for seg in range(2 * st.L + 2):
@@ -435,18 +483,21 @@
                             "(train_unet.py:208 calls model.train() first); use evaluate() for eval-mode passes")
 
     def _enqueue(self, st, variant, comm):
-        first, boundary = variant
+        first, boundary = variant[:2]
+        fused, prepacked = variant[2:] if len(variant) > 2 else (False, False)
         s = stream_ptr()
         if self.quirk:
             accumulate, run_backward = 0, boundary
         else:
             accumulate, run_backward = (0 if first else 1), True
-        drop, t_logits = self._forward_loss(st, s)
-        self._backward_exchange(st, s, comm, drop, t_logits, accumulate, boundary, run_backward)
-        if boundary:
+        drop, t_logits = self._forward_loss(st, s, TRAIN | (PREPACKED if prepacked else 0))
+        rode = self._backward_exchange(st, s, comm, drop, t_logits, accumulate, boundary, run_backward, rider=fused and boundary)
+        if boundary and fused:
+            st.plan.adamw_pack(self.arena, st.tail_ranges, len(st.opt_ranges), self._hyper(), rode=rode, stream=s)
+        elif boundary:
             self._adamw(self.arena, st.opt_ranges, self._hyper(), s)
 
-    def _forward_loss(self, st, s):
+    def _forward_loss(self, st, s, training=TRAIN):
         model, plan, loss = self.model, st.plan, st.loss
         drop = engine.fill_drop_scales(st.drop, float(getattr(model, "dropout_rate", 0.0)),
                                        lambda: engine._rng_state(model, self.device),
@@ -459,9 +510,9 @@
         fused = st.fused_head
         keep = st.logits if self.keep_logits else None
         if fused and teacher is None:
-            plan.forward_loss(st.x, loss, drop=drop, labels=st.y, logits=keep, stream=s)
+            plan.forward_loss(st.x, loss, drop=drop, training=training, labels=st.y, logits=keep, stream=s)
         else:
-            plan.forward(st.x, drop=drop, logits=None if fused else st.logits, stream=s)
+            plan.forward(st.x, drop=drop, training=training, logits=None if fused else st.logits, stream=s)
         t_logits = None
         if teacher is not None:
             if ks is not None:
@@ -475,7 +526,8 @@
             loss.metrics_forward(st.logits, st.y, teacher=t_logits, stream=s)
         return drop, t_logits
 
-    def _backward_exchange(self, st, s, comm, drop, t_logits, accumulate, boundary, run_backward):
+    def _backward_exchange(self, st, s, comm, drop, t_logits, accumulate, boundary, run_backward, rider=False):
+        rode = False
         met = st.metrics
         met_pending = self.do_comm
         joined = False
@@ -510,10 +562,14 @@
                 join = 1 if (last or self.use_graph or aux is None) else 0
                 aux_open = aux_open or (aux is not None and not join)
                 kw = dict(drop=drop, accumulate=accumulate, start=start, end=end, stream=s, aux=aux, events=self._events, join=join)
+                if rider and last:
+                    st.plan.step_rider(self.arena.step)
                 if st.fused_head:
                     st.plan.backward_loss(st.x, st.loss, labels=st.y, teacher=t_logits, grad_scale=self.inv_accum, **kw)
                 else:
                     st.plan.backward(st.x, dlogits=st.dlogits, **kw)
+                if rider and last:
+                    rode = _lib.lib().mi3d_backward_step_rode() == 1
                 if use_marks:
                     cs = self.comm_stream
                     for i, (sg, b) in enumerate(mid):
@@ -533,6 +589,7 @@
             comm(lambda: self._on_comm_stream(lambda: self.comm.average_(met)))
         if self.do_comm and not joined:
             comm(self._join_comm)
+        return rode
 
     def load_batch(self, images, labels):
         self._load(self._prepare(images), False, x=images, y=labels)
@@ -545,6 +602,7 @@
     def evaluate(self, images, labels):
         if self.do_comm:
             self.sync_buffers()
+        self.invalidate_packs()
         st = self._prepare(images, mode="eval")
         st.x.copy_(images)
         st.y.copy_(labels.reshape(st.y.shape))
```

Measured after the change: 984.9 volumes/s, median of 6. About the same (+0.6%).
